# NVlabs/bayes-sim-ig

Hardware: AMD Instinct MI355X
Metric: summary_vectors_per_sec_in_fit (higher is better)
Workload: dtype f32; 1 GPU; cfg5: ShadowHand MDRFF-4096 K=4 D=32, summary_start (I=2310), 100000 pairs/GPU, reference chunk protocol: <=1000-pair chunks, summarizer + 100 Adam updates x minibatch 100 + 6 held-out evals per chunk; pairs_per_gpu=100000, parallelism=dp1, gradient_exchange=none, hip_graph=True

## Files before the change

### bayes_sim_ig_amd/_lib.py

```python
import ctypes as C
import os

import torch

_HERE = os.path.dirname(os.path.abspath(__file__))
LIB_PATH = os.environ.get('BSIG_LIB_PATH') or os.path.join(_HERE, 'lib', 'libbsig_hip.so')

BSIG_OK, BSIG_EINVAL, BSIG_ELAUNCH, BSIG_EUNSUPPORTED, BSIG_ENONFINITE = 0, -1, -2, -3, -4
EPI_NONE, EPI_BIAS, EPI_BIAS_ACT, EPI_COS_SIN, EPI_COS_OFF, EPI_MUL_DACT = range(6)
ACT_TANH, ACT_RELU, ACT_LEAKY_RELU, ACT_SIGMOID, ACT_IDENTITY = range(5)
MAX_HIDDEN = 8
FIT_GRAPH, FIT_SPLIT_ADAM = 1, 2
PLAN_NO_PERSISTENT = 1
X_ROWS, X_CROSSCORR_FACTORS = 0, 1

i64, i32, u64, f32, vp, sz = (C.c_int64, C.c_int32, C.c_uint64, C.c_float,
                              C.c_void_p, C.c_size_t)


class HeadDims(C.Structure):
    _fields_ = [('out_dim', i32), ('n_comp', i32), ('full_cov', i32),
                ('eps_noise', f32), ('min_weight', f32), ('ll_limit', f32)]


class MdnCfg(C.Structure):
    _fields_ = [('input_dim', i32), ('n_hidden', i32),
                ('hidden', i32 * MAX_HIDDEN), ('activation', i32),
                ('rff_feats', i32), ('rff_cos_only', i32),
                ('rff_scale', f32), ('head', HeadDims),
                ('lr', f32), ('beta1', f32), ('beta2', f32), ('adam_eps', f32)]


class FitBuffers(C.Structure):
    _fields_ = [('params', vp), ('grads', vp), ('exp_avg', vp),
                ('exp_avg_sq', vp),
                ('rff_coeff', vp), ('ld_coeff', i64), ('rff_offset', vp),
                ('x_train', vp), ('ldx_train', i64), ('n_train', i64),
                ('y_train', vp), ('ldy_train', i64),
                ('x_test', vp), ('ldx_test', i64), ('n_test', i64),
                ('y_test', vp), ('ldy_test', i64),
                ('ids_table', vp), ('train_loss', vp), ('test_loss', vp),
                ('state', vp), ('workspace', vp), ('workspace_bytes', sz),
                ('x_kind', i32), ('x_s', i32), ('x_a', i32),
                ('x_test_factors', vp), ('ldx_test_factors', i64)]


_PROTOS = {
    'bsig_last_error': (C.c_char_p, []),
    'bsig_version': (C.c_int, []),
    'bsig_abi_info': (u64, [C.c_int]),
    'bsig_device_count': (C.c_int, []),
    'bsig_summary_dim': (i64, [C.c_int] * 5),
    'bsig_summary_start': (C.c_int, [vp, vp, vp, i64] + [C.c_int] * 5 + [i64, vp]),
    'bsig_crosscorr': (C.c_int, [vp, vp, vp, i64] + [C.c_int] * 5 + [i64, vp, vp]),
    'bsig_crosscorr_factor_dims': (C.c_int, [C.c_int] * 3 + [C.POINTER(i32)] * 2),
    'bsig_crosscorr_factors': (C.c_int, [vp, vp, vp, i64] + [C.c_int] * 5 + [i64, vp, vp]),
    'bsig_crosscorr_expand': (C.c_int, [vp, i64, i64, C.c_int, C.c_int, vp, i64, vp]),
    'bsig_signature': (C.c_int, [vp, vp, vp, i64] + [C.c_int] * 4 + [i64, vp]),
    'bsig_gemm_workspace_bytes': (sz, [i64, i64, i64]),
    'bsig_gemm_f32': (C.c_int, [vp, i64, C.c_int, vp, vp, i64, C.c_int, vp, vp,
                                i64, i64, i64, i64, C.c_int, C.c_int, vp, vp,
                                i64, f32, vp, sz, vp]),
    'bsig_rff_coeff': (C.c_int, [vp, vp, vp, i64, i64, i64, vp]),
    'bsig_rff_project': (C.c_int, [vp, i64, vp, vp, i64, vp, vp, i64, i64, i64,
                                   i64, f32, C.c_int, vp, sz, vp]),
    'bsig_head_width': (i64, [C.POINTER(HeadDims)]),
    'bsig_head_workspace_bytes': (sz, [C.POINTER(HeadDims), i64]),
    'bsig_mdn_head_outputs': (C.c_int, [C.POINTER(HeadDims), vp, i64, i64, vp,
                                        u64, u64, vp, vp, vp, vp, vp, vp, sz, vp]),
    'bsig_mdn_nll_from_tuple': (C.c_int, [C.POINTER(HeadDims), vp, vp, vp, vp,
                                          vp, i64, i64, vp, vp, vp, sz, vp]),
    'bsig_mdn_head_nll': (C.c_int, [C.POINTER(HeadDims), vp, i64, vp, i64, vp,
                                    i64, i64, vp, u64, u64, vp, vp, vp, vp, sz,
                                    vp]),
    'bsig_adam_flat': (C.c_int, [vp, vp, vp, vp, i64, f32, f32, f32, f32, i64, vp]),
    'bsig_colsum': (C.c_int, [vp, i64, i64, i64, vp, vp, sz, vp]),
    'bsig_normalize_rows': (C.c_int, [vp, i64, vp, vp, vp, i64, i64, i64, vp]),
    'bsig_copy_rows': (C.c_int, [vp, i64, vp, vp, i64, i64, i64, vp]),
    'bsig_mdn_param_count': (i64, [C.POINTER(MdnCfg)]),
    'bsig_mdn_param_offsets': (C.c_int, [C.POINTER(MdnCfg), C.POINTER(i64), C.c_int]),
    'bsig_mdn_workspace_bytes': (sz, [C.POINTER(MdnCfg), i64]),
    'bsig_mdn_head_forward': (C.c_int, [C.POINTER(MdnCfg), vp, vp, i64, vp, vp,
                                        i64, vp, i64, vp, i64, vp, sz, vp]),
    'bsig_mdn_loss_grad': (C.c_int, [C.POINTER(MdnCfg), vp, vp, i64, vp, vp, i64,
                                     vp, i64, vp, i64, i64, vp, u64, u64, vp, vp,
                                     vp, vp, sz, vp]),
    'bsig_fit_create': (C.c_int, [C.POINTER(MdnCfg), i64, i64, i64, C.POINTER(vp)]),
    'bsig_fit_create_sized': (C.c_int, [C.POINTER(MdnCfg), i64, i64, i64, i64, C.POINTER(vp)]),
    'bsig_fit_create_ex': (C.c_int, [C.POINTER(MdnCfg), i64, i64, i64, i64, C.c_int, C.POINTER(vp)]),
    'bsig_fit_destroy': (None, [vp]),
    'bsig_fit_workspace_bytes': (sz, [vp]),
    'bsig_fit_bind': (C.c_int, [vp, C.POINTER(FitBuffers), C.c_int]),
    'bsig_fit_begin': (C.c_int, [vp, u64, i64, vp]),
    'bsig_fit_set_features': (C.c_int, [vp, vp, i64, i64, vp]),
    'bsig_fit_run': (C.c_int, [vp, i64, vp]),
    'bsig_fit_grad': (C.c_int, [vp, vp]),
    'bsig_fit_apply': (C.c_int, [vp, vp]),
    'bsig_fit_flush': (C.c_int, [vp, vp]),
    'bsig_fit_is_persistent': (C.c_int, [vp]),
    'bsig_fit_accepts_factors': (C.c_int, [vp]),
    'bsig_fit_accepts_factor_rows': (C.c_int, [vp, C.c_int, C.c_int]),
    'bsig_fit_evaluates_from_factors': (C.c_int, [vp, C.c_int, C.c_int, C.c_int]),
    'bsig_fit_takes_features': (C.c_int, [vp, i64]),
    'bsig_fit_eval': (C.c_int, [vp, vp]),
    'bsig_fit_updates': (C.c_int, [vp, i64, vp]),
    'bsig_debug_persist_profile': (None, [vp]),
    'bsig_debug_spin': (C.c_int, [C.c_int, sz, C.c_int, vp]),
    'bsig_debug_persist_geometry': (C.c_int, [C.c_int, C.c_int, C.c_int, C.c_int, C.c_int, C.POINTER(C.c_int32)]),
    'bsig_debug_head_geometry': (C.c_int, [C.POINTER(HeadDims), i64, C.POINTER(C.c_int32)]),
    'bsig_debug_summary_path': (C.c_int, [C.c_int, i64] + [C.c_int] * 6 + [i64, C.c_int, C.c_int,
                                                                         C.POINTER(C.c_int32)]),
    'bsig_debug_mfma_vs_fma': (C.c_int, [vp, vp, C.c_int, vp, vp]),
    'bsig_debug_persist_mdnn_geometry': (C.c_int, [C.c_int, C.c_int, C.c_int, C.c_int, C.c_int, C.c_int, C.POINTER(C.c_int32)]),
    'bsig_comm_unique_id': (C.c_int, [vp]),
    'bsig_comm_init': (C.c_int, [vp, C.c_int, C.c_int, C.c_int, C.POINTER(vp)]),
    'bsig_comm_init_external': (C.c_int, [C.c_int, C.c_int, vp, vp, C.POINTER(vp)]),
    'bsig_comm_transport': (C.c_int, [vp]),
    'bsig_comm_world': (C.c_int, [vp]),
    'bsig_fit_dp_graph_status': (C.c_int, [vp, C.c_char_p, sz]),
    'bsig_comm_rank': (C.c_int, [vp]),
    'bsig_comm_resident_calls': (i64, [vp]),
    'bsig_comm_set_resident': (None, [vp, C.c_int]),
    'bsig_comm_resident_mode': (C.c_int, [vp]),
    'bsig_comm_allreduce': (C.c_int, [vp, vp, i64, vp]),
    'bsig_comm_broadcast': (C.c_int, [vp, vp, i64, C.c_int, vp]),
    'bsig_comm_destroy': (None, [vp]),
    'bsig_fit_pack_logs': (C.c_int, [vp, i64, vp, vp]),
    'bsig_fit_run_dp': (C.c_int, [vp, vp, i64, vp, vp]),
}
COMM_ID_BYTES = 128
EXCHANGE_SUM, EXCHANGE_BROADCAST = 0, 1
EXCHANGE_FN = C.CFUNCTYPE(C.c_int, vp, C.c_int, vp, i64, C.c_int, vp)

_lib = None


def exported_symbols():
    return sorted(_PROTOS)


def load():
    global _lib
    if _lib is None:
        if not os.path.exists(LIB_PATH):
            raise RuntimeError(
                'libbsig_hip.so not built (%s): run ./build.sh or '
                '__graft_entry__.build(); there is no CPU fallback' % LIB_PATH)
        lib = C.CDLL(LIB_PATH)
        for name, (res, args) in _PROTOS.items():
            fn = getattr(lib, name)
            fn.restype, fn.argtypes = res, args
        _check_abi(lib)
        _lib = lib
    return _lib


HEADER_PATH = os.path.join(os.path.dirname(_HERE), 'include', 'bsig.h')


def header_hash(path=HEADER_PATH):
    h = 0xcbf29ce484222325
    with open(path, 'rb') as f:
        for b in f.read():
            h = ((h ^ b) * 0x100000001b3) & 0xFFFFFFFFFFFFFFFF
    return h


def _check_abi(lib):
    want = {1: C.sizeof(HeadDims), 2: C.sizeof(MdnCfg), 3: C.sizeof(FitBuffers),
            4: FitBuffers.x_kind.offset}
    for which, size in want.items():
        got = int(lib.bsig_abi_info(which))
        if got != size:
            raise RuntimeError('libbsig_hip.so was built against another include/bsig.h (layout %d: '
                               'library %d, binding %d): rebuild with ./build.sh' % (which, got, size))
    built = int(lib.bsig_abi_info(0))
    if built and os.path.exists(HEADER_PATH) and built != header_hash():
        raise RuntimeError('libbsig_hip.so was built from another revision of include/bsig.h '
                           '(hash %016x, header %016x): rebuild with ./build.sh'
                           % (built, header_hash()))


def require_gpu():
    lib = load()
    if not torch.cuda.is_available():
        raise RuntimeError('bayes_sim_ig_amd needs a ROCm GPU (MI355X): '
                           'torch.cuda.is_available() is False and there is '
                           'no CPU fallback')
    return lib


def check(rc):
    if rc == BSIG_OK:
        return
    msg = load().bsig_last_error().decode('utf-8', 'replace')
    if rc == BSIG_EINVAL:
        raise AssertionError(msg)
    if rc == BSIG_EUNSUPPORTED:
        raise NotImplementedError(msg)
    raise RuntimeError('libbsig_hip: %s (code %d)' % (msg, rc))


def ptr(t):
    return None if t is None else C.c_void_p(t.data_ptr())


def stream(device=None):
    return C.c_void_p(torch.cuda.current_stream(device).cuda_stream)


# ... 24 lines not shown
```

### bayes_sim_ig_amd/bayes_sim.py

```python
import os

import numpy as np
import torch

from . import pdf
from . import summarizers as _summ
from .mdnn import MDNN
from .mdrff import MDRFF
from .summarizers import (pad_states_actions, summary_start, summary_waypts,
                          summary_corr, summary_corrdiff, summary_signatory,
                          signature_depth, cross_correlation)

_SUMMARIZERS = {
    'summary_start': summary_start, 'summary_waypts': summary_waypts,
    'summary_corr': summary_corr, 'summary_corrdiff': summary_corrdiff,
    'summary_signatory': summary_signatory,
}
_MODELS = {'MDNN': MDNN, 'MDRFF': MDRFF}


class BayesSim(object):
    NUM_TRAIN_TRAJ_PER_BATCH = 1000
    NUM_TRAIN_EPOCHS = 10
    MINIBATCH_SIZE = 100
# ... 2 lines not shown
    FIT_BLOCK_CHUNKS = 32
    REFIT_SAMPLES = int(1e4)
    REFIT_MINIBATCH = 100
    REFIT_EPOCHS = 5

    def __init__(self, model_cfg, obs_dim, act_dim, params_dim, params_lows,
                 params_highs, prior, proposal=None, device='cpu'):
        self.prior = prior
        self.proposal = proposal
        model_class = model_cfg['modelClass']
        name = model_cfg['summarizerFxn']
        if name not in _SUMMARIZERS:
            raise NameError("name '%s' is not defined" % name)
        self.summarizer_name = name
        self.summarizer_fxn = _SUMMARIZERS[name]
        self._sig_depth = model_cfg.get('sigDepth', None)
        traj_summaries_dim = _summ.summary_dim(
            name, model_cfg['trainTrajLen'], obs_dim, act_dim,
            self._sig_depth or 0)
        full_covariance = bool(model_cfg.get('fullCovariance', False))
        kwargs = {'input_dim': traj_summaries_dim, 'output_dim': params_dim,
                  'output_lows': params_lows, 'output_highs': params_highs,
                  'n_gaussians': model_cfg['components'],
                  'hidden_layers': model_cfg['hiddenLayers'],
                  'lr': model_cfg['lr'],
                  'activation': torch.nn.Tanh,
                  'full_covariance': full_covariance,
                  'device': device}
        if model_class.startswith('MDRFF'):
            kernel, sigma = 'RBF', 4.0
            if '_' in model_class:
                parts = model_class.split('_')
                model_class, kernel = parts[0], parts[1]
                if len(parts) > 2:
                    sigma = float(parts[2])
            kwargs.update({'n_feat': int(model_cfg.get('nFeat', 200)),
                           'sigma': sigma, 'kernel': kernel})
        if model_class not in _MODELS:
            raise NameError("name '%s' is not defined" % model_class)
        self.model = _MODELS[model_class](**kwargs)

    @staticmethod
    def get_n_trajs_per_batch(n_train_trajs, n_train_trajs_done):
        n = BayesSim.NUM_TRAIN_TRAJ_PER_BATCH
        if n_train_trajs_done + n > n_train_trajs:
            n = n_train_trajs - n_train_trajs_done
        return n

    def _summarize(self, states, actions, finite_flag=None, lazy=False):
        if self.summarizer_name == 'summary_signatory' and self._sig_depth:
            return self.summarizer_fxn(states, actions, depth=self._sig_depth)
        if self.summarizer_name in ('summary_corr', 'summary_corrdiff'):
            kw = {}
            if finite_flag is not None:
                kw['check_finite'] = finite_flag
            if lazy and self._lazy_summaries():
                kw['lazy'] = True
            return self.summarizer_fxn(states, actions, **kw)
        return self.summarizer_fxn(states, actions)

    def _lazy_summaries(self):
        return (getattr(self.model, 'rff', None) is None and self.model._flat.is_cuda and
                os.environ.get('BSIG_NO_FUSED_SUMMARY') != '1')

    def run_training(self, params, traj_states, traj_actions, _defer=False, _finite_flag=None,
                     _summaries=None, _feats=None):
        traj_summaries = _summaries if _summaries is not None else \
            self._summarize(traj_states, traj_actions, _finite_flag, lazy=True)
        kw = {} if _feats is None else {'_feats': _feats}
        return self.model.run_training(
            x_data=traj_summaries, y_data=params,
            n_updates=BayesSim.NUM_GRAD_UPDATES,
            batch_size=BayesSim.MINIBATCH_SIZE,
            test_frac=BayesSim.TEST_FRACTION, _defer=_defer, **kw)

    FIT_BLOCK_BYTES = 4 << 30

    def fit(self, params, traj_states, traj_actions):
        if self.model._flat.is_cuda and self.model._may_time_out():
            from .mdnn import PersistentTimeout
            snap = self.model._snapshot()
            for _ in range(2):
                calls0 = self.model._resident_calls()
                try:
                    return self._fit_once(params, traj_states, traj_actions)
                except PersistentTimeout:
                    self.model._restore(snap)
                    self.model._give_up_a_level(calls0)
        return self._fit_once(params, traj_states, traj_actions)

    def _fit_once(self, params, traj_states, traj_actions):
        n, done, pending = params.shape[0], 0, []
        dp = getattr(self.model, '_dp', None)
        if dp is not None:
            counts = dp.gather_counts(n, device=self.model._flat.device)
            if len(set(counts)) != 1:
                raise ValueError('data-parallel fit needs the same number of pairs on every rank '
                                 '(got %s); see dp.equal_shards' % (counts,))
        flag = None
        if torch.is_tensor(traj_states) and traj_states.is_cuda:
            flag = torch.zeros(1, dtype=torch.int32, device=traj_states.device)
        block = 0
        is_rff = getattr(self.model, 'rff', None) is not None
        if flag is not None and os.environ.get('BSIG_NO_FIT_PREPROJECT') != '1':
            row_bytes = 4 * (self.model.input_dim + (self.model.rff.n_feat if is_rff else 0))
            chunks = max(min(BayesSim.FIT_BLOCK_CHUNKS,
                             BayesSim.FIT_BLOCK_BYTES // (row_bytes * BayesSim.NUM_TRAIN_TRAJ_PER_BATCH)), 1)
            block = chunks * BayesSim.NUM_TRAIN_TRAJ_PER_BATCH
        lo = hi = 0
        summ = feats = None
        while done < n:
            m = BayesSim.get_n_trajs_per_batch(n, done)
            if block and done + m > hi:
                lo, hi = done, min(n, done + block)
                summ = self._summarize(traj_states[lo:hi], traj_actions[lo:hi], flag, lazy=True)
                feats = self.model.rff.to_features(summ) if is_rff else None
            if block:
                pending.append(self.run_training(
                    params[done:done + m], None, None, _defer=True,
                    _summaries=summ[done - lo:done - lo + m],
                    _feats=None if feats is None else feats[done - lo:done - lo + m]))
            else:
                pending.append(self.run_training(params[done:done + m],
                                                 traj_states[done:done + m],
                                                 traj_actions[done:done + m], _defer=True,
                                                 _finite_flag=flag))
            done += m
        logs = [p.result() for p in pending]
        assert flag is None or int(flag.item()) == 0
        return logs

    def predict(self, states, actions, threshold=0.005):
        summaries = self._summarize(states, actions)
        mixtures = [self._correct_for_proposal(m, threshold) for m in self.model.predict_MoGs(summaries)]
        return mixtures[0] if len(mixtures) == 1 else self._refit(mixtures)

    def _correct_for_proposal(self, mog, threshold):
        if self.proposal is None:
            return mog
        mog.prune_negligible_components(threshold=threshold)
        if isinstance(self.prior, pdf.Uniform):
            return mog / self.proposal
        if isinstance(self.prior, pdf.Gaussian):
            return (mog * self.prior) / self.proposal
        raise NotImplementedError

    def _refit(self, mixtures):
        src = self.model
        refit = MDNN(input_dim=1, output_dim=src.output_dim,
                     output_lows=src.output_lows.detach().cpu().numpy(),
                     output_highs=src.output_highs.detach().cpu().numpy(),
                     n_gaussians=src.n_gaussians, hidden_layers=(128, 128), lr=src.lr,
                     activation=src.activation, full_covariance=src.L_size > 0, device=src.device)
        share = int(BayesSim.REFIT_SAMPLES / len(mixtures))
        draws = torch.from_numpy(np.concatenate([m.gen(n_samples=share) for m in mixtures], axis=0))
        draws = draws.float().to(src.device)
        if MDNN.VERBOSE:
            print(f'Fitting posterior from {len(mixtures):d} mogs')
        const_in = torch.zeros(draws.shape[0], 1, device=draws.device)
        refit.run_training(const_in, draws,
                           BayesSim.REFIT_EPOCHS * BayesSim.REFIT_SAMPLES // BayesSim.REFIT_MINIBATCH,
                           BayesSim.REFIT_MINIBATCH)
        fitted = refit.predict_MoGs(const_in[0:1, :])
        assert len(fitted) == 1
        return fitted[0]
```

### bayes_sim_ig_amd/csrc/estimator.hip

```cpp
#include "comm.h"
#include "gemm.h"
#include "head.h"
#include "persist.h"
#include "persist_mdnn.h"

#include <algorithm>
#include <chrono>
#include <cmath>
#include <cstdlib>
#include <cstring>
#include <new>

namespace bsig {

int adam_launch(float* p, const float* g, float* m, float* v, int64_t n, float lr,
                float beta1, float beta2, float eps, int64_t t, const float* dyn,
                hipStream_t st);
int colsum_launch(const float* x, int64_t ld, int64_t rows, int64_t cols, float* out,
                  void* workspace, size_t workspace_bytes, hipStream_t st);

constexpr int64_t kAlign = 4;

struct Layout {
  int n_layers;
// ... 297 lines not shown
  bsig_mdn_cfg cfg;
  Layout L;
  int64_t batch, max_test, n_updates, n_evals;
  bool hoist;
  bool feat_cache;
  bool feat_unique;
  bool feats_preloaded;
  const float* ext_feats;
  int64_t feat_rows;
  int64_t max_train;
  bsig_fit_buffers buf;
  bool bound;
  int64_t norm_batch;
  size_t train_ws_bytes, test_ws_bytes, feats_bytes, big_gemm_ws_bytes, iota_bytes;
  bool use_graph, split_adam;

  PersistEngine eng;
  UGeom ug; MdnnGeom mg;
  bool eng_off;
  int dp_evals_done;
  bool resident_ran;
  bool adam_pending;
  hipStream_t cap_stream;
  hipGraphExec_t g_step, g_grad, g_apply, g_eval;
  bool graphs_ready;
  const float* graph_feats;
  hipGraphExec_t g_dp; const bsig_comm* g_dp_comm;
  int g_dp_state;
  char g_dp_error[200];
};

namespace bsig {

static size_t plan_ws_bytes(const bsig_fit_plan* p) {
  return p->train_ws_bytes + p->test_ws_bytes + p->feats_bytes + p->big_gemm_ws_bytes +
         p->iota_bytes + p->eng.workspace_bytes;
}

static int engine(const bsig_fit_plan* p) { return p->eng_off ? 0 : p->eng.kind; }

static bool evals_in_launch(const bsig_fit_plan* p, bool dp, bool test_factors) {
  return (dp ? p->eng.eval_dp : p->eng.eval_single) && (!p->eng.streams || test_factors);
}

static bool feat_cache_applies(const bsig_fit_plan* p, int64_t n_train) {
  return p->hoist && p->feat_cache && n_train <= p->n_updates * p->batch;
}

struct PlanMem { Scratch tr, te; float* feats; float* big_ws; int32_t* iota; void* persist_ws; };

static int begin_regions(const bsig_fit_plan* p) {
  const bool pers = engine(p) != 0;
  return (pers ? 2 : 0) + (!(pers && !p->split_adam) ? 2 : 0);
}
static bool tickets_zeroed(const bsig_fit_plan* p) { return begin_regions(p) + 2 <= 4; }

static void plan_mem(const bsig_fit_plan* p, PlanMem* m) {
  char* base = reinterpret_cast<char*>(p->buf.workspace);
  carve(&p->cfg, p->L, p->batch, base, &m->tr);
  base += p->train_ws_bytes;
  carve(&p->cfg, p->L, std::max<int64_t>(p->max_test, 1), base, &m->te);
  base += p->test_ws_bytes;
  m->feats = p->ext_feats ? const_cast<float*>(p->ext_feats) : reinterpret_cast<float*>(base);
  base += p->feats_bytes;
  m->big_ws = reinterpret_cast<float*>(base); base += p->big_gemm_ws_bytes;
  m->iota = reinterpret_cast<int32_t*>(base); base += p->iota_bytes;
  m->persist_ws = base;
  if (!tickets_zeroed(p)) m->tr.tickets = m->te.tickets = nullptr;
}

static PersistShape persist_shape(const bsig_fit_plan* p) {
  return PersistShape{(int)p->batch, (int)p->L.feat_dim, p->cfg.head.out_dim, p->cfg.head.n_comp,
                      (int)std::min<int64_t>(p->max_test, 1 << 20)};
}

static PersistMdnnShape persist_mdnn_shape(const bsig_fit_plan* p) {
  const bsig_mdn_cfg& c = p->cfg;
  return PersistMdnnShape{(int)p->batch, c.input_dim, c.n_hidden > 0 ? c.hidden[0] : 0,
                          c.n_hidden > 1 ? c.hidden[1] : 0, c.activation, c.head.out_dim,
                          c.head.n_comp, c.head.full_cov,
                          (int)std::min<int64_t>(p->max_test, 1 << 20)};
}

static int enqueue_persistent(bsig_fit_plan* p, int n, hipStream_t st, int eval_total = 0,
                              const CommXr* xr = nullptr) {
  PlanMem m; plan_mem(p, &m);
  const bsig_fit_buffers& b = p->buf;
  PersistCommon c;
  c.y = b.y_train; c.ldy = b.ldy_train; c.ids = b.ids_table;
  c.params = b.params; c.exp_avg = b.exp_avg; c.exp_avg_sq = b.exp_avg_sq;
  c.state = b.state; c.train_loss = b.train_loss;
  c.workspace = m.persist_ws; c.workspace_bytes = p->eng.workspace_bytes;
  if (p->split_adam) {
    c.grads = b.grads; c.adam_pending = p->adam_pending ? 1 : 0;
    p->adam_pending = false;
  }
  if (xr) { c.xr_ready = xr->ready; c.xr_done = xr->done; c.xr_base = xr->base; c.n_total = n; }
  if (eval_total > 0) {
    c.do_eval = 1; c.n_total = eval_total; c.eval_every = std::max(eval_total / 5, 1);
    c.n_test = (int)b.n_test;
    c.y_test = b.y_test; c.ldy_test = b.ldy_test; c.test_loss = b.test_loss;
  }
  c.hy.lr = p->cfg.lr; c.hy.beta1 = p->cfg.beta1; c.hy.beta2 = p->cfg.beta2;
  c.hy.adam_eps = p->cfg.adam_eps; c.hy.eps_noise = p->cfg.head.eps_noise;
  c.hy.min_weight = p->cfg.head.min_weight; c.hy.ll_limit = p->cfg.head.ll_limit;
  c.hy.norm_batch = p->norm_batch;
  if (engine(p) == 1) {
    PersistBuffers pb;
    static_cast<PersistCommon&>(pb) = c;
    pb.feats = m.feats; pb.ld_feats = p->cfg.rff_feats;
    pb.feat_ids = p->feat_unique ? b.ids_table : nullptr;
    pb.w_off = p->L.head_w_off; pb.b_off = p->L.head_b_off;
    pb.eval_row0 = p->feat_unique ? b.n_train : p->n_updates * p->batch;
    return persist_run(persist_shape(p), p->ug, pb, n, st);
  }
  PersistMdnnBuffers pb;
  static_cast<PersistCommon&>(pb) = c;
  pb.x = b.x_train; pb.ldx = b.ldx_train;
  pb.x_kind = b.x_kind; pb.x_s = b.x_s; pb.x_a = b.x_a;
  pb.w1_off = p->L.w_off[0]; pb.b1_off = p->L.b_off[0];
  pb.w2_off = p->L.w_off[1]; pb.b2_off = p->L.b_off[1];
  pb.wh_off = p->L.head_w_off; pb.bh_off = p->L.head_b_off;
  pb.x_test = b.x_test; pb.ldx_test = b.ldx_test;
  pb.x_test_fac = b.x_test_factors; pb.ldx_test_fac = b.ldx_test_factors;
  return persist_mdnn_run(persist_mdnn_shape(p), p->mg, pb, n, st);
}

static Inputs train_inputs(const bsig_fit_plan* p, const PlanMem& m) {
  const bsig_fit_buffers& b = p->buf;
  Inputs in;
  in.dyn = b.state + ST_STEP; in.dyn_stride = p->batch;
  in.rff_coeff = b.rff_coeff; in.ld_coeff = b.ld_coeff; in.rff_offset = b.rff_offset;
  if (p->hoist) {
    in.x = m.feats; in.ldx = p->cfg.rff_feats; in.is_feat = true;
    if (p->feat_unique) in.rows = b.ids_table;
  }
  else { in.x = b.x_train; in.ldx = b.ldx_train; in.rows = b.ids_table; }
  return in;
}

static Inputs eval_inputs(const bsig_fit_plan* p, const PlanMem& m) {
  const bsig_fit_buffers& b = p->buf;
  Inputs in;
  in.rff_coeff = b.rff_coeff; in.ld_coeff = b.ld_coeff; in.rff_offset = b.rff_offset;
  if (p->hoist) {
    in.x = m.feats; in.ldx = p->cfg.rff_feats; in.is_feat = true;
    in.dyn = b.state + ST_EVAL; in.dyn_stride = 0;
    in.dyn_base = p->feat_unique ? b.n_train : p->n_updates * p->batch;
  } else {
    in.x = b.x_test; in.ldx = b.ldx_test;
  }
  return in;
}

static int enqueue_grad(bsig_fit_plan* p, hipStream_t st, bool fuse_adam) {
  if (p->buf.x_kind != BSIG_X_ROWS) { set_error("per-phase update on factor rows"); return BSIG_EUNSUPPORTED; }
  PlanMem m; plan_mem(p, &m);
  const bsig_fit_buffers& b = p->buf;
  const Inputs in = train_inputs(p, m);
  HeadDyn hd;
  hd.y_dyn = b.state + ST_STEP; hd.y_dyn_stride = p->batch;
  hd.hook.state = b.state; hd.hook.kind = 1;
  hd.hook.lr = p->cfg.lr; hd.hook.beta1 = p->cfg.beta1; hd.hook.beta2 = p->cfg.beta2;
  AdamFuse fuse{b.exp_avg, b.exp_avg_sq, reinterpret_cast<const float*>(b.state) + ST_ADAM0,
                p->cfg.beta1, p->cfg.beta2, p->cfg.adam_eps};
  const uint64_t* rng = reinterpret_cast<const uint64_t*>(b.state + ST_RNG);
  int n_sig = 0;
  BSIG_TRY(forward_pass(&p->cfg, p->L, b.params, in, p->batch, m.tr, m.tr.o, m.tr.ld_o, st,
                        &n_sig));
  hd.n_sig_ready = n_sig;
  HeadBiasPartials bp;
  const bool partial_bias = fuse_adam && p->L.n_layers == 0 && in.rows != nullptr &&
      gemm_wide_gradient_applies(p->L.nh, p->L.feat_dim, p->batch, m.tr.ld_o, in.ldx, m.tr.d_o, in.x, true);
  BSIG_TRY(head_nll(&p->cfg, p->L, m.tr, b.y_train, b.ldy_train, b.ids_table, p->batch,
                    p->norm_batch, nullptr, 0, 0, rng, b.train_loss, b.state + ST_STEP, true,
                    b.grads + p->L.head_b_off, b.state + ST_NONFINITE, &hd, st,
                    partial_bias ? &bp : nullptr));
  return backward_pass(&p->cfg, p->L, b.params, in, -1, p->batch, m.tr, b.grads,
                       fuse_adam ? &fuse : nullptr, st, partial_bias ? &bp : nullptr);
}

static int enqueue_apply(bsig_fit_plan* p, hipStream_t st) {
  const bsig_fit_buffers& b = p->buf;
  return adam_launch(b.params, b.grads, b.exp_avg, b.exp_avg_sq, p->L.total, p->cfg.lr,
                     p->cfg.beta1, p->cfg.beta2, p->cfg.adam_eps, 1,
                     reinterpret_cast<const float*>(b.state) + ST_ADAM0, st);
}

static int enqueue_eval(bsig_fit_plan* p, hipStream_t st) {
  PlanMem m; plan_mem(p, &m);
  const bsig_fit_buffers& b = p->buf;
  HeadDyn hd;
  hd.hook.state = b.state; hd.hook.kind = 2;
  if (b.n_test <= 0) {
    hipLaunchKernelGGL(iota_mod_kernel, dim3(1), dim3(64), 0, st, b.state + ST_EVAL + 0, 0, 1);
    BSIG_CHECK_LAUNCH("eval_noop");
// ... 121 lines not shown
  carve(cfg, L, batch, workspace, &s);
  s.tickets = nullptr;
  Inputs in;
  in.x = x; in.ldx = ldx; in.rows = x_rows;
  in.rff_coeff = rff_coeff; in.ld_coeff = ld_coeff; in.rff_offset = rff_offset;
  return forward_pass(cfg, L, params, in, batch, s, head_out, ld_head, as_stream(stream));
}

extern "C" int bsig_mdn_loss_grad(const bsig_mdn_cfg* cfg, const float* params,
                                  const float* rff_coeff, int64_t ld_coeff,
                                  const float* rff_offset, const float* x, int64_t ldx,
                                  const float* y, int64_t ldy, const int32_t* rows,
                                  int64_t batch, int64_t norm_batch, const float* noise,
                                  uint64_t seed, uint64_t stream_id, float* grads, float* loss,
                                  int32_t* nonfinite, void* workspace, size_t workspace_bytes,
                                  bsig_stream_t stream) {
  Layout L;
  BSIG_TRY(make_layout(cfg, &L));
  BSIG_REQUIRE(params && x && y && grads && batch >= 1 && norm_batch >= 1,
               "loss_grad: bad args");
  BSIG_REQUIRE(ldx >= cfg->input_dim && ldy >= cfg->head.out_dim, "loss_grad: leading dims");
  Scratch s;
  carve(cfg, L, batch, nullptr, &s);
  BSIG_REQUIRE(workspace && workspace_bytes >= s.total_bytes, "loss_grad: workspace %zu < %zu",
               workspace_bytes, s.total_bytes);
  carve(cfg, L, batch, workspace, &s);
  s.tickets = nullptr;
  hipStream_t st = as_stream(stream);
  Inputs in;
  in.x = x; in.ldx = ldx; in.rows = rows;
  in.rff_coeff = rff_coeff; in.ld_coeff = ld_coeff; in.rff_offset = rff_offset;
  int n_sig = 0;
  BSIG_TRY(forward_pass(cfg, L, params, in, batch, s, s.o, s.ld_o, st, &n_sig));
  HeadDyn hd;
  hd.n_sig_ready = n_sig;
  BSIG_TRY(head_nll(cfg, L, s, y, ldy, rows, batch, norm_batch, noise, seed, stream_id, nullptr,
                    loss, nullptr, true, grads + L.head_b_off, nonfinite, &hd, st));
  return backward_pass(cfg, L, const_cast<float*>(params), in, 0, batch, s, grads, nullptr, st);
}

extern "C" int bsig_fit_create(const bsig_mdn_cfg* cfg, int64_t batch, int64_t max_test_rows,
                               int64_t n_updates, bsig_fit_plan** plan) {
  return bsig_fit_create_sized(cfg, batch, 0, max_test_rows, n_updates, plan);
}

extern "C" int bsig_fit_create_sized(const bsig_mdn_cfg* cfg, int64_t batch,
                                     int64_t max_train_rows, int64_t max_test_rows,
                                     int64_t n_updates, bsig_fit_plan** plan) {
  return bsig_fit_create_ex(cfg, batch, max_train_rows, max_test_rows, n_updates, 0, plan);
}

extern "C" int bsig_fit_create_ex(const bsig_mdn_cfg* cfg, int64_t batch,
                                  int64_t max_train_rows, int64_t max_test_rows,
                                  int64_t n_updates, int plan_flags, bsig_fit_plan** plan) {
  BSIG_REQUIRE(cfg && plan && batch >= 1 && max_train_rows >= 0 && max_test_rows >= 0 &&
               n_updates >= 0, "fit_create: bad args");
  bsig_fit_plan* p = new (std::nothrow) bsig_fit_plan();
  BSIG_REQUIRE(p, "fit_create: out of memory");
  std::memset(p, 0, sizeof(*p));
  p->cfg = *cfg;
  const int rc = make_layout(cfg, &p->L);
  if (rc != BSIG_OK) { delete p; return rc; }
  p->batch = batch; p->max_test = max_test_rows; p->norm_batch = batch;
  p->n_updates = n_updates; p->n_evals = count_evals(n_updates);
  Scratch s;
  carve(cfg, p->L, batch, nullptr, &s); p->train_ws_bytes = s.total_bytes;
  carve(cfg, p->L, std::max<int64_t>(max_test_rows, 1), nullptr, &s);
  p->test_ws_bytes = s.total_bytes;
  p->max_train = max_train_rows;
  const auto set = [](const char* name) { const char* e = getenv(name); return e && e[0] == '1'; };
  p->feat_cache = !set("BSIG_NO_FEAT_CACHE");
  if (!p->feat_cache) max_train_rows = 0;
  p->feat_rows = (max_train_rows > 0 ? std::min(n_updates * batch, max_train_rows)
                                     : n_updates * batch) + max_test_rows;
  const size_t feats = (size_t)p->feat_rows * (size_t)std::max(cfg->rff_feats, 0) * sizeof(float);
  p->hoist = cfg->rff_feats > 0 && n_updates > 0 && feats <= ((size_t)4 << 30) && !set("BSIG_NO_RFF_HOIST");
  if (!((plan_flags & BSIG_PLAN_NO_PERSISTENT) || set("BSIG_NO_PERSISTENT"))) {
    if (p->hoist && p->L.n_layers == 0 && cfg->head.full_cov == 0)
      persist_resolve(persist_shape(p), &p->ug, &p->eng);
    else if (cfg->rff_feats == 0 && p->L.n_layers == 2 && n_updates > 0)
      persist_mdnn_resolve(persist_mdnn_shape(p), &p->mg, &p->eng);
  }
  if (set("BSIG_NO_INKERNEL_EVAL")) p->eng.eval_single = p->eng.eval_dp = false;
  p->eng.workspace_bytes = round_up<size_t>(p->eng.workspace_bytes, 256);
  if (p->hoist) {
    p->feats_bytes = round_up<size_t>(feats, 256);
    const int64_t mf = cfg->rff_cos_only ? cfg->rff_feats : cfg->rff_feats / 2;
    p->big_gemm_ws_bytes = round_up<size_t>(
        std::max(bsig_gemm_workspace_bytes(p->feat_rows - max_test_rows, mf, cfg->input_dim),
                 bsig_gemm_workspace_bytes(std::max<int64_t>(max_test_rows, 1), mf,
                                           cfg->input_dim)) + 256, 256);
  }
  *plan = p;
  return BSIG_OK;
}

extern "C" void bsig_fit_destroy(bsig_fit_plan* p) {
  if (!p) return;
  drop_graphs(p);
  if (p->cap_stream) (void)hipStreamDestroy(p->cap_stream);
  delete p;
}

extern "C" size_t bsig_fit_workspace_bytes(const bsig_fit_plan* p) {
  return p ? plan_ws_bytes(p) : 0;
}

extern "C" int bsig_fit_bind(bsig_fit_plan* p, const bsig_fit_buffers* b, int flags) {
  BSIG_REQUIRE(p && b, "fit_bind: null");
  BSIG_REQUIRE(b->params && b->grads && b->exp_avg && b->exp_avg_sq && b->state &&
               b->workspace && b->x_train && b->y_train && b->ids_table && b->train_loss &&
               b->test_loss, "fit_bind: null buffer");
  BSIG_REQUIRE(b->workspace_bytes >= plan_ws_bytes(p), "fit_bind: workspace %zu < %zu",
               b->workspace_bytes, plan_ws_bytes(p));
  BSIG_REQUIRE(!(p->max_train > 0 && b->n_train > p->max_train),
               "fit_bind: %lld training rows exceed the %lld the plan was sized for",
               (long long)b->n_train, (long long)p->max_train);
  BSIG_REQUIRE(b->n_train >= 1 && b->n_test >= 0 && b->n_test <= std::max<int64_t>(p->max_test, 0),
               "fit_bind: n_train=%lld n_test=%lld (max %lld)", (long long)b->n_train,
               (long long)b->n_test, (long long)p->max_test);
  const bool fac = b->x_kind == BSIG_X_CROSSCORR_FACTORS;
  BSIG_REQUIRE(b->x_kind == BSIG_X_ROWS || fac, "fit_bind: unknown x_kind %d", b->x_kind);
  const bool graph = (flags & BSIG_FIT_GRAPH) != 0, split = (flags & BSIG_FIT_SPLIT_ADAM) != 0;
  const bool eng_off = p->eng.streams && !(fac && bsig_fit_accepts_factor_rows(p, b->x_s, b->x_a));
  if (eng_off != p->eng_off) { drop_graphs(p); p->eng_off = eng_off; p->bound = false; }
  const MdnnGeom& g = p->mg;
  if (engine(p) == 2 && p->eng.streams && !(g.s_S == b->x_s && g.s_A == b->x_a && g.s_dp == (split ? 1 : 0)))
    BSIG_TRY(persist_mdnn_resolve_stream(&p->mg, p->cfg.input_dim, p->cfg.head.full_cov != 0, b->x_s, b->x_a, split));
  if (fac) {
    BSIG_REQUIRE(b->x_s >= 1 && b->x_a >= 1 && (int64_t)b->x_s * b->x_a + 2 == p->cfg.input_dim,
                 "fit_bind: factor rows S=%d A=%d do not give the %d inputs of the first layer",
                 b->x_s, b->x_a, p->cfg.input_dim);
    BSIG_REQUIRE(b->ldx_train >= b->x_s + b->x_a + 3, "fit_bind: factor rows need a pitch >= S + A + 3");
    const bool eval_fac = b->x_test_factors && bsig_fit_evaluates_from_factors(p, b->x_s, b->x_a, flags);
    BSIG_REQUIRE(b->n_test == 0 || (eval_fac && !b->x_test) || b->ldx_test >= p->cfg.input_dim,
                 "fit_bind: the held-out rows are summary rows (ldx_test >= input_dim)");
    if (!bsig_fit_accepts_factor_rows(p, b->x_s, b->x_a)) {
      set_error("fit_bind: this plan runs kernels that read materialised summary rows "
                "(bsig_fit_accepts_factors); expand the factors (bsig_crosscorr_expand)");
      return BSIG_EUNSUPPORTED;
    }
  }
  BSIG_REQUIRE((fac || b->ldx_train >= p->cfg.input_dim) && b->ldy_train >= p->cfg.head.out_dim,
               "fit_bind: leading dims too small");
  BSIG_REQUIRE(!(b->n_test > 0 && !b->y_test), "fit_bind: null test buffers");
  BSIG_REQUIRE(!(b->n_test > 0 && !b->x_test &&
                 !(fac && b->x_test_factors && bsig_fit_evaluates_from_factors(p, b->x_s, b->x_a, flags))),
               "fit_bind: null test buffers");
  const bool same = p->bound && std::memcmp(&p->buf, b, sizeof(*b)) == 0 &&
                    p->use_graph == graph && p->split_adam == split;
  if (!same) {
    drop_graphs(p);
    p->buf = *b;
    p->feat_unique = feat_cache_applies(p, b->n_train);
    if (p->hoist && !p->feat_unique && p->feat_rows - p->max_test < p->n_updates * p->batch) {
      p->bound = false;
      set_error("fit_bind: %lld training rows exceed the %lld the plan was sized for",
                (long long)b->n_train, (long long)p->max_train);
      return BSIG_EINVAL;
    }
    p->bound = true;
    p->use_graph = graph;
    p->split_adam = split;
  }
  if (p->use_graph && !p->cap_stream)
    BSIG_HIP(hipStreamCreateWithFlags(&p->cap_stream, hipStreamNonBlocking));
  return BSIG_OK;
}

static bool graphs_read_feats(const bsig_fit_plan* p) {
  if (!p->use_graph) return false;
  if (engine(p) != 1) return true;
  if (p->buf.n_test < 1) return false;
  return !evals_in_launch(p, p->split_adam, false);
}

extern "C" int bsig_fit_set_features(bsig_fit_plan* p, const float* feats, int64_t ld_feats,
                                     int64_t rows, bsig_stream_t stream) {
  BSIG_REQUIRE(p && p->bound && feats, "fit_set_features: plan not bound / null");
  BSIG_REQUIRE(p->hoist && p->feat_unique, "fit_set_features: the plan keeps no per-row feature cache");
  BSIG_REQUIRE(rows == p->buf.n_train + p->buf.n_test && ld_feats >= p->cfg.rff_feats,
               "fit_set_features: need the %lld training + %lld held-out rows",
               (long long)p->buf.n_train, (long long)p->buf.n_test);
  p->ext_feats = nullptr;
  if (ld_feats == p->cfg.rff_feats && aligned(feats, 16) && !graphs_read_feats(p)) {
    p->ext_feats = feats;
  } else {
    PlanMem m; plan_mem(p, &m);
    const size_t w = (size_t)p->cfg.rff_feats * sizeof(float);
    BSIG_HIP(hipMemcpy2DAsync(m.feats, w, feats, (size_t)ld_feats * sizeof(float), w, (size_t)rows,
                              hipMemcpyDeviceToDevice, as_stream(stream)));
  }
  p->feats_preloaded = true;
  return BSIG_OK;
}

extern "C" int bsig_fit_begin(bsig_fit_plan* p, uint64_t seed, int64_t norm_batch,
                              bsig_stream_t stream) {
  bsig::Range roctx_range("bsig_fit_begin");
  BSIG_REQUIRE(p && p->bound, "fit_begin: plan not bound");
  BSIG_REQUIRE(norm_batch >= 1, "fit_begin: norm_batch must be >= 1");
  if (norm_batch != p->norm_batch) { drop_graphs(p); p->norm_batch = norm_batch; }
  hipStream_t st = as_stream(stream);
  p->adam_pending = false;
  p->resident_ran = false;
  p->dp_evals_done = 0;
  BeginZero bz{};
  int nz = 0;
  int64_t total4 = 0;
  auto add_zero = [&](void* ptr, size_t bytes) {
    bz.ptr[nz] = reinterpret_cast<float4*>(ptr);
    bz.n4[nz] = (int64_t)(bytes / 16);
    total4 += bz.n4[nz];
    ++nz;
  };
  if (engine(p)) {
    PlanMem m; plan_mem(p, &m);
    ZeroRegion zr[2];
    if (engine(p) == 1) BSIG_TRY(persist_reset_regions(p->ug, m.persist_ws, p->eng.workspace_bytes, zr));
    else BSIG_TRY(persist_mdnn_reset_regions(p->mg, m.persist_ws, p->eng.workspace_bytes, zr));
    BSIG_REQUIRE(aligned(zr[0].ptr, 16) && aligned(zr[1].ptr, 16) && zr[0].bytes % 16 == 0 &&
                 zr[1].bytes % 16 == 0, "fit_begin: persistent workspace regions must be 16-byte multiples");
    add_zero(zr[0].ptr, zr[0].bytes);
    add_zero(zr[1].ptr, zr[1].bytes);
  }
  if (!(engine(p) && !p->split_adam)) {
    BSIG_REQUIRE(aligned(p->buf.exp_avg, 16) && aligned(p->buf.exp_avg_sq, 16),
                 "fit_begin: the Adam moment buffers must be 16-byte aligned");
    add_zero(p->buf.exp_avg, (size_t)p->L.total * sizeof(float));
    add_zero(p->buf.exp_avg_sq, (size_t)p->L.total * sizeof(float));
  }
  if (tickets_zeroed(p)) {
    BSIG_REQUIRE(nz == begin_regions(p), "fit_begin: region count out of step with begin_regions()");
    PlanMem tm; plan_mem(p, &tm);
    add_zero(tm.tr.tickets, kWideTickets * sizeof(int32_t));
    add_zero(tm.te.tickets, kWideTickets * sizeof(int32_t));
  }
  const int blocks = (int)std::min<int64_t>(std::max<int64_t>(ceil_div<int64_t>(total4, 256 * 4), 1), 1024);
  hipLaunchKernelGGL(fit_begin_kernel, dim3(blocks), dim3(256), 0, st, p->buf.state, seed, bz);
  BSIG_CHECK_LAUNCH("fit_begin");
  if (p->hoist) {
    if (p->feats_preloaded) p->feats_preloaded = false;
    else { p->ext_feats = nullptr; BSIG_TRY(enqueue_hoisted_rff(p, st)); }
  }
  return ensure_graphs(p);
}

static int dp_eval_total(const bsig_fit_plan* p) {
  return engine(p) && p->split_adam && p->buf.n_test >= 1 && evals_in_launch(p, true, false) ? (int)p->n_updates : 0;
}

extern "C" int bsig_fit_grad(bsig_fit_plan* p, bsig_stream_t stream) {
  BSIG_REQUIRE(p && p->bound && p->split_adam, "fit_grad: plan not bound with SPLIT_ADAM");
  if (engine(p)) return enqueue_persistent(p, 1, as_stream(stream), dp_eval_total(p));
  if (p->use_graph) { BSIG_TRY(ensure_graphs(p)); BSIG_HIP(hipGraphLaunch(p->g_grad, as_stream(stream))); return BSIG_OK; }
  return enqueue_grad(p, as_stream(stream), false);
}

extern "C" int bsig_fit_apply(bsig_fit_plan* p, bsig_stream_t stream) {
  BSIG_REQUIRE(p && p->bound && p->split_adam, "fit_apply: plan not bound with SPLIT_ADAM");
  if (engine(p) && !p->eng.streams) { p->adam_pending = true; return BSIG_OK; }
  if (engine(p)) return enqueue_apply(p, as_stream(stream));
  if (p->use_graph) { BSIG_TRY(ensure_graphs(p)); BSIG_HIP(hipGraphLaunch(p->g_apply, as_stream(stream))); return BSIG_OK; }
  return enqueue_apply(p, as_stream(stream));
}

extern "C" int bsig_fit_takes_features(const bsig_fit_plan* p, int64_t n_train) {
  return p && n_train >= 1 && feat_cache_applies(p, n_train) ? 1 : 0;
}

extern "C" int bsig_fit_accepts_factors(const bsig_fit_plan* p) {
  return p && p->eng.kind == 2 && !p->eng.streams ? 1 : 0;
}

extern "C" int bsig_fit_accepts_factor_rows(const bsig_fit_plan* p, int s_dim, int a_dim) {
  return p && p->eng.kind == 2 && persist_mdnn_factors_fit(p->mg, p->cfg.input_dim, s_dim, a_dim) ? 1 : 0;
}

extern "C" int bsig_fit_evaluates_from_factors(const bsig_fit_plan* p, int s_dim, int a_dim, int bind_flags) {
  return p && p->eng.streams && bsig_fit_accepts_factor_rows(p, s_dim, a_dim) &&
                 evals_in_launch(p, (bind_flags & BSIG_FIT_SPLIT_ADAM) != 0, true) ? 1 : 0;
}

extern "C" int bsig_fit_is_persistent(const bsig_fit_plan* p) {
  return p ? engine(p) : 0;
}

extern "C" int bsig_fit_flush(bsig_fit_plan* p, bsig_stream_t stream) {
  BSIG_REQUIRE(p && p->bound, "fit_flush: plan not bound");
  if (engine(p) && p->split_adam && p->adam_pending)
    return enqueue_persistent(p, 0, as_stream(stream));
  return BSIG_OK;
}

extern "C" int bsig_fit_eval(bsig_fit_plan* p, bsig_stream_t stream) {
  bsig::Range roctx_range("bsig_fit_eval");
  BSIG_REQUIRE(p && p->bound, "fit_eval: plan not bound");
  if (const int total = dp_eval_total(p)) {
    if (++p->dp_evals_done < count_evals(total)) return BSIG_OK;
    return enqueue_persistent(p, 0, as_stream(stream), total);
  }
  BSIG_REQUIRE(p->buf.n_test < 1 || p->buf.x_test,
               "fit_eval: this binding has no held-out summary rows (its evaluations run inside bsig_fit_run)");
  BSIG_TRY(bsig_fit_flush(p, stream));
  if (p->use_graph) { BSIG_TRY(ensure_graphs(p)); BSIG_HIP(hipGraphLaunch(p->g_eval, as_stream(stream))); return BSIG_OK; }
  return enqueue_eval(p, as_stream(stream));
}

static int enqueue_updates(bsig_fit_plan* p, int64_t n, hipStream_t st) {
  if (n <= 0) return BSIG_OK;
  if (engine(p) && !p->split_adam) return enqueue_persistent(p, (int)n, st);
  if (engine(p)) {
    for (int64_t it = 0; it < n; ++it) {
      BSIG_TRY(enqueue_persistent(p, 1, st, dp_eval_total(p)));
      if (p->eng.streams) BSIG_TRY(enqueue_apply(p, st));
      else p->adam_pending = true;
    }
    return BSIG_OK;
  }
  for (int64_t it = 0; it < n; ++it) {
    if (p->use_graph) {
      if (p->split_adam) {
        BSIG_HIP(hipGraphLaunch(p->g_grad, st));
        BSIG_HIP(hipGraphLaunch(p->g_apply, st));
      } else {
        BSIG_HIP(hipGraphLaunch(p->g_step, st));
      }
    } else {
      BSIG_TRY(enqueue_grad(p, st, !p->split_adam));
      if (p->split_adam) BSIG_TRY(enqueue_apply(p, st));
    }
  }
  return BSIG_OK;
}

extern "C" int bsig_fit_updates(bsig_fit_plan* p, int64_t n_updates, bsig_stream_t stream) {
  bsig::Range roctx_range("bsig_fit_updates");
  BSIG_REQUIRE(p && p->bound, "fit_updates: plan not bound");
  BSIG_REQUIRE(n_updates >= 0 && n_updates <= p->n_updates,
               "fit_updates: n_updates %lld exceeds the plan's %lld", (long long)n_updates,
               (long long)p->n_updates);
  if (p->use_graph) BSIG_TRY(ensure_graphs(p));
  return enqueue_updates(p, n_updates, as_stream(stream));
}

extern "C" int bsig_fit_run(bsig_fit_plan* p, int64_t n_updates, bsig_stream_t stream) {
  bsig::Range roctx_range("bsig_fit_run");
  BSIG_REQUIRE(p && p->bound, "fit_run: plan not bound");
  BSIG_REQUIRE(n_updates >= 0 && n_updates <= p->n_updates,
               "fit_run: n_updates %lld exceeds the plan's %lld", (long long)n_updates,
               (long long)p->n_updates);
  hipStream_t st = as_stream(stream);
  if (p->use_graph) BSIG_TRY(ensure_graphs(p));
  if (engine(p) && !p->split_adam && n_updates >= 1 && p->buf.n_test >= 1 &&
      evals_in_launch(p, false, p->buf.x_test_factors != nullptr))
    return enqueue_persistent(p, (int)n_updates, st, (int)n_updates);
  const int64_t every = std::max<int64_t>(n_updates / 5, 1);
  int64_t done = 0;
  for (int64_t it = 0; it < n_updates; ++it) {
    if (it % every == 0 || it + 1 == n_updates) {
      BSIG_TRY(enqueue_updates(p, it + 1 - done, st));
      done = it + 1;
      BSIG_TRY(bsig_fit_eval(p, stream));
    }
  }
  return BSIG_OK;
}

namespace bsig {
__global__ void pack_logs_kernel(const float* train_loss, const float* test_loss,
                                 const int32_t* state, int n_updates, int n_evals, float* out) {
  const int every = n_updates / 5 > 1 ? n_updates / 5 : 1;
  if (threadIdx.x == 0) {
    int e = 0;
    for (int it = 0; it < n_updates; ++it)
      if (it % every == 0 || it + 1 == n_updates) { out[e] = train_loss[it]; ++e; }
    out[2 * n_evals] = (float)state[ST_NONFINITE];
  }
  for (int i = threadIdx.x; i < n_evals; i += blockDim.x) out[n_evals + i] = test_loss[i];
}
}

extern "C" int bsig_fit_pack_logs(bsig_fit_plan* p, int64_t n_updates, float* out,
                                  bsig_stream_t stream) {
  BSIG_REQUIRE(p && p->bound && out, "fit_pack_logs: plan not bound / null");
  BSIG_REQUIRE(n_updates >= 0 && n_updates <= p->n_updates, "fit_pack_logs: bad n_updates");
  hipLaunchKernelGGL(pack_logs_kernel, dim3(1), dim3(64), 0, as_stream(stream), p->buf.train_loss,
                     p->buf.test_loss, p->buf.state, (int)n_updates, (int)count_evals(n_updates), out);
  BSIG_CHECK_LAUNCH("pack_logs");
  return BSIG_OK;
}

namespace bsig {
__global__ void pack_dp_logs_kernel(const float* train_loss, const float* test_loss,
                                    const int32_t* state, int n_updates, int n_evals, float n_test,
                                    float* out) {
  const int n = n_updates + n_evals + 3;
  for (int i = blockIdx.x * blockDim.x + threadIdx.x; i < n; i += gridDim.x * blockDim.x) {
    float v;
    if (i < n_updates) v = train_loss[i];
    else if (i < n_updates + n_evals) v = n_test > 0.f ? test_loss[i - n_updates] * n_test : 0.f;
    else if (i == n_updates + n_evals) v = n_test;
    else v = (state[ST_NONFINITE] >> (i - n_updates - n_evals - 1)) & 1 ? 1.f : 0.f;
    out[i] = v;
  }
}
}

__global__ void debug_scale_kernel(float* buf, int64_t n, float s) {
  for (int64_t i = (int64_t)blockIdx.x * blockDim.x + threadIdx.x; i < n; i += (int64_t)gridDim.x * blockDim.x)
    buf[i] *= s;
}
static int allreduce_grads(bsig_fit_plan* p, bsig_comm* comm, bsig_stream_t stream) {
  BSIG_TRY(bsig_comm_allreduce(comm, p->buf.grads, p->L.total, stream));
  if (const char* e = getenv("BSIG_DEBUG_GRAD_EXCHANGE_SCALE")) {
    const float s = (float)atof(e);
    if (s != 1.0f) {
      const char* ge = getenv("BSIG_DEBUG_GRAD_EXCHANGE_GRID");
      const int grid = ge ? std::max(atoi(ge), 1) : 8;
      hipLaunchKernelGGL(debug_scale_kernel, dim3(grid), dim3(1024), 0, as_stream(stream), p->buf.grads, p->L.total, s);
      BSIG_CHECK_LAUNCH("debug_scale");
    }
  }
  return BSIG_OK;
}

static int ensure_dp_graph(bsig_fit_plan* p, bsig_comm* comm) {
  if (p->g_dp_state == 1 && p->g_dp_comm == comm) return BSIG_OK;
  if (p->g_dp_state < 0 && p->g_dp_comm == comm) return BSIG_OK;
  if (p->g_dp) { (void)hipGraphExecDestroy(p->g_dp); p->g_dp = nullptr; }
  p->g_dp_comm = comm; p->g_dp_error[0] = 0;
  const char* env = getenv("BSIG_DP_GRAPH");
  if (!p->use_graph || engine(p) != 1 || bsig_comm_transport(comm) != 1 || !(env && env[0] == '1')) {
    p->g_dp_state = -2;
    snprintf(p->g_dp_error, sizeof(p->g_dp_error), "%s",
             !(env && env[0] == '1') ? "not requested (BSIG_DP_GRAPH=1)" :
             bsig_comm_transport(comm) != 1 ? "the exchange is not RCCL" : "the plan's updates are not one launch each");
    return BSIG_OK;
  }
  hipGraph_t graph = nullptr;
  hipError_t e = hipStreamBeginCapture(p->cap_stream, hipStreamCaptureModeRelaxed);
  int rc = BSIG_OK;
  if (e == hipSuccess) {
    p->adam_pending = true;
    rc = enqueue_persistent(p, 1, p->cap_stream, dp_eval_total(p));
    if (rc == BSIG_OK) rc = allreduce_grads(p, comm, reinterpret_cast<bsig_stream_t>(p->cap_stream));
    e = hipStreamEndCapture(p->cap_stream, &graph);
  }
  if (e == hipSuccess && rc == BSIG_OK) e = hipGraphInstantiate(&p->g_dp, graph, nullptr, nullptr, 0);
  if (graph) (void)hipGraphDestroy(graph);
  if (e != hipSuccess || rc != BSIG_OK || !p->g_dp) {
    snprintf(p->g_dp_error, sizeof(p->g_dp_error), "capture of launch + ncclAllReduce failed: %s",
             rc != BSIG_OK ? bsig_last_error() : hipGetErrorString(e));
    (void)hipGetLastError();
    p->g_dp = nullptr; p->g_dp_state = -1;
    return BSIG_OK;
  }
  p->g_dp_state = 1;
  return BSIG_OK;
}

extern "C" int bsig_fit_dp_graph_status(const bsig_fit_plan* p, char* msg, size_t msg_bytes) {
  if (!p) return 0;
  if (msg && msg_bytes) snprintf(msg, msg_bytes, "%s", p->g_dp_error);
  return p->g_dp_state;
}

static bool dp_resident_applies(const bsig_fit_plan* p, const bsig_comm* comm, int64_t n_updates) {
  const char* e = getenv("BSIG_DP_RESIDENT");
  const int mode = bsig_comm_resident_mode(comm);
  bool want = mode >= 0 ? mode == 1 : (e && e[0] == '1');
  if (want && !bsig::comm_resident_allowed(comm)) {
// ... 157 lines not shown
```

### bayes_sim_ig_amd/csrc/fit_persistent.hip

```cpp
#include "persist.h"

#include <algorithm>
#include <cstdlib>

#include "head_device.h"
#include "persist_device.h"

namespace bsig {

constexpr int kUT = 512;
constexpr int kUSteps = 18;
constexpr int kUGroup = 6;
constexpr int kUMT = 7;
constexpr int kULds = 160 * 1024;
constexpr int kUProf = 8;
constexpr int kUFP = 116;

struct UArgs {
  int B, Bp, MT;
  int Fdim, KS, ksteps, KB, WP;
  int Nh, NhP, D, K;
  int n_blocks, k_slices, G, T, n_owner, R;
  int n_updates, xs_floats;
  int fast_rows;
  const float* feats; int64_t ld_feats; const int32_t* feat_ids;
  const float* y; int64_t ldy; const int32_t* ids;
  float* params; float* m1; float* m2; int64_t w_off, b_off;
  int32_t* state; float* train_loss;
  double lr, beta1, beta2;
  float adam_eps, eps_noise, min_w, ll_limit, inv_norm;
  float* slabs; float* d_out; float* e_out; unsigned* flag_fwd; unsigned long long* gran;
  unsigned long long* gran_rep;
  float* grads; int adam_pending; int quad_ok;
  unsigned* xr_ready; const unsigned* xr_done; unsigned* xr_count; unsigned xr_base;
  int do_eval, eval_every, n_total, n_test, eval_passes, NE, RE;
  int64_t eval_row0;
  const float* y_test; int64_t ldy_test;
  float* test_loss;
  float* eval_slabs;
  unsigned* flag_eval;
  unsigned long long* gran_eval;
  long long* prof;
  int prof_t0;
};

__device__ __forceinline__ f32x4 umfma(float a, float b, f32x4 c) {
  return __builtin_amdgcn_mfma_f32_16x16x4f32(a, b, c, 0, 0, 0);
}

struct URole { int tile, owner; };
__device__ __forceinline__ URole wg_role(int wg, int T, int G) {
  const int per = T >> 3, rem = T & 7, gq = G >> 3, gr = G & 7;
  const int x = wg & 7, j = wg >> 3;
  const int tiles_x = gq + (x < gr ? 1 : 0);
  URole r;
  if (j < tiles_x) {
    r.tile = x * gq + min(x, gr) + j;
    int rank = 0;
    for (int xx = 0; xx < 8; ++xx) {
      const int cnt = wg > xx ? (wg - xx + 7) >> 3 : 0;
      rank += min(cnt, gq + (xx < gr ? 1 : 0));
    }
    r.owner = (T - G) + rank;
  } else {
    r.tile = -1;
    r.owner = x * (per - gq) + min(x, rem) - min(x, gr) + (j - tiles_x);
  }
  return r;
}

__device__ __forceinline__ int u_rowpos(int b) { return (b & ~15) + ((b & 3) << 2) + ((b >> 2) & 3); }

__device__ __forceinline__ int u_evals_before(int s, int every) { return s == 0 ? 0 : (s - 1) / every + 1; }

#define BSIG_USTAMP(k)                                                           \
  do {                                                                           \
    if (p.prof && threadIdx.x == 0 && t >= p.prof_t0 && t < p.prof_t0 + kUProf)  \
      p.prof[((int64_t)wg * kUProf + t - p.prof_t0) * 16 + (k)] = wall_clock64(); \
  } while (0)

__device__ __forceinline__ int u_fast_kind(const UArgs& p) {
  const int K = p.K;
  if (K > 16 || p.fast_rows == 0) return 0;
  if (p.T - p.G < p.n_owner) return 0;
  const int KP = K <= 4 ? 4 : (K <= 8 ? 8 : 16);
  const int nq = (p.D + 64 / KP - 1) / (64 / KP);
  if (p.R > 4 || nq > 8 || p.R * ((p.Nh + 3) >> 2) > kUT) return 0;
  const int nqh = nq <= 2 ? 1 : (nq <= 4 ? 2 : 4);
  return KP * 8 + nqh;
}

__device__ __forceinline__ unsigned long long* gran_rep(const UArgs& p, int arr, int x) {
  return p.gran_rep + (int64_t)(arr * 8 + x) * kGranArr;
}
__device__ __forceinline__ void granule_publish8(const UArgs& p, int arr, int slot, uint32_t tag, float v, int lane) {
  if (lane < 8) granule_publish(gran_rep(p, arr, lane), slot, tag, v);
}

template <typename RowOff, typename F>
__device__ __forceinline__ void u_rows_sum(const float* slabs, RowOff&& rowoff, int k_slices, int zs, int nrows,
                                           int n_cols, float* out, int out_pitch, int tid, F&& fn) {
  const __amdgpu_buffer_rsrc_t sr = xwg_buffer(slabs);
  for (int idx = tid; idx < nrows * n_cols; idx += kUT) {
    const int r = idx / n_cols, col = idx - r * n_cols;
    const int voff = (rowoff(r) + col) * 4;
    float v = 0.f;
    for (int z = 0; z < k_slices; z += 16) {
      float q[16];
#pragma unroll
      for (int u = 0; u < 16; ++u)
        q[u] = __uint_as_float(__builtin_amdgcn_raw_buffer_load_b32(sr, voff, min(z + u, k_slices - 1) * zs * 4, kXwgPolicy));
#pragma unroll
      for (int u = 0; u < 16; ++u)
        if (z + u < k_slices) v += q[u];
    }
    out[r * out_pitch + col] = v;
    fn(col, v);
  }
}

template <typename RowOff, typename F>
__device__ __forceinline__ void u_rows_sum4(const float* slabs, RowOff&& rowoff, int k_slices, int zs, int nrows,
                                            int n_cols, int ld, float* out, int out_pitch, float* part, int tid,
                                            F&& fn) {
  const __amdgpu_buffer_rsrc_t sr = xwg_buffer(slabs);
  const int ncq = (n_cols + 3) >> 2, Q = nrows * ncq;
  const int SG = max(1, min(min(k_slices, kUT / Q), 8));
  const int qc = tid % Q, sg = tid / Q;
  if (sg < SG) {
    const int r = qc / ncq, c4 = (qc - r * ncq) * 4;
    const int voff = rowoff(r) + c4;
    f32x4 v = {0.f, 0.f, 0.f, 0.f};
    for (int z0 = sg; z0 < k_slices; z0 += 8 * SG) {
      f32x4 q[8];
#pragma unroll
      for (int u = 0; u < 8; ++u) q[u] = xwg_load4(sr, voff + min(z0 + u * SG, k_slices - 1) * zs);
#pragma unroll
      for (int u = 0; u < 8; ++u)
        if (z0 + u * SG < k_slices) v += q[u];
    }
    *reinterpret_cast<f32x4*>(part + 4 * (sg * Q + qc)) = v;
  }
  __syncthreads();
  if (tid < Q) {
    const int r = tid / ncq, c4 = (tid - r * ncq) * 4;
    f32x4 v = *reinterpret_cast<const f32x4*>(part + 4 * tid);
    for (int g = 1; g < SG; ++g) v += *reinterpret_cast<const f32x4*>(part + 4 * (g * Q + tid));
#pragma unroll
    for (int j = 0; j < 4; ++j)
      if (c4 + j < n_cols) {
        out[r * out_pitch + c4 + j] = v[j];
        fn(c4 + j, v[j]);
      }
  }
}

template <int NT>
__device__ __forceinline__ void u_tile_eval(const UArgs& p, const float* Wl, const float* biasl, int slot,
                                            int ks, int n0, int k0, int eidx) {
  int tid = threadIdx.x;
  asm volatile("" : "+v"(tid));
  const int lane = tid & 63, w = tid >> 6, c16 = lane & 15, g4 = lane >> 4;
  const int B = p.B, NhP = p.NhP;
  for (int pass = 0; pass < p.eval_passes; ++pass) {
    const int rows = min(B, p.n_test - pass * B);
    if (rows <= 0) break;
    if (w < p.MT) {
      f32x4 acc[NT];
#pragma unroll
      for (int nt = 0; nt < NT; ++nt) {
        const f32x4 zero = {0.f, 0.f, 0.f, 0.f};
        acc[nt] = ks == 0 ? *reinterpret_cast<const f32x4*>(biasl + 16 * nt + 4 * g4) : zero;
      }
      const int64_t r = p.eval_row0 + pass * B + min(16 * w + c16, rows - 1);
      const float* src = p.feats + r * p.ld_feats;
      const float* ap = Wl + c16 * p.WP + 4 * g4;
#pragma unroll 1
      for (int s0 = 0; s0 < p.ksteps; s0 += kUGroup) {
        f32x4 breg[kUGroup];
#pragma unroll
        for (int q = 0; q < kUGroup; ++q) {
          const int col = k0 + 16 * (s0 + q) + 4 * g4;
          const f32x4 v = *reinterpret_cast<const f32x4*>(src + min((int64_t)col, p.ld_feats - 4));
          const f32x4 zero = {0.f, 0.f, 0.f, 0.f};
          breg[q] = col < p.Fdim ? v : zero;
        }
#pragma unroll
        for (int q = 0; q < kUGroup; ++q) {
#pragma unroll
          for (int nt = 0; nt < NT; ++nt) {
            const f32x4 a4 = *reinterpret_cast<const f32x4*>(ap + nt * 16 * p.WP + 16 * (s0 + q));
            acc[nt] = umfma(a4[0], breg[q][0], acc[nt]);
            acc[nt] = umfma(a4[1], breg[q][1], acc[nt]);
            acc[nt] = umfma(a4[2], breg[q][2], acc[nt]);
            acc[nt] = umfma(a4[3], breg[q][3], acc[nt]);
          }
        }
      }
      if (16 * w + c16 < rows) {
        const __amdgpu_buffer_rsrc_t sr = xwg_buffer(
            p.eval_slabs + ((((int64_t)(eidx % 3) * p.eval_passes + pass) * p.k_slices + ks) * B) * NhP + n0);
#pragma unroll
        for (int nt = 0; nt < NT; ++nt)
          xwg_store4(sr, (16 * w + c16) * NhP + 16 * nt + 4 * g4, acc[nt][0], acc[nt][1], acc[nt][2], acc[nt][3]);
      }
    }
  }
  __builtin_amdgcn_s_waitcnt(0);
  __syncthreads();
  if (tid == 0) flag_raise(p.flag_eval, slot, (unsigned)eidx + 1u);
}

__device__ __forceinline__ void u_owner_eval(const UArgs& p, float* XS, float* red, int eo, int eidx,
                                             uint64_t stream, const HeadArgs& a) {
  int tid = threadIdx.x;
  asm volatile("" : "+v"(tid));
  const int lane = tid & 63, w = tid >> 6;
  const int B = p.B, Nh = p.Nh, NhP = p.NhP, D = p.D, K = p.K, DK = D * K;
  const int per_wave = Nh + D + 3 * K;
  int32_t* flagp = p.state + 2;
  const unsigned etag = (unsigned)eidx + 1u;
  if (w == 0) flags_wait(p.flag_eval, p.G, etag, lane, flagp);
  __syncthreads();
  const int nr = eo < p.n_test ? min(p.RE, (p.n_test - eo + p.NE - 1) / p.NE) : 0;
  const float* ebase = p.eval_slabs + (int64_t)(eidx % 3) * p.eval_passes * p.k_slices * B * NhP;
  float eacc = 0.f;
  u_rows_sum(ebase,
             [&](int r) {
               const int erow = eo + p.NE * r, pass = erow / B, rb = erow - pass * B;
               return (pass * p.k_slices * B + rb) * NhP;
             },
             p.k_slices, B * NhP, nr, Nh, XS, per_wave, tid,
             [&](int col, float v) { if (col >= K + DK && col < K + 2 * DK) eacc += expf(v); });
  eacc = wave_sum_dpp(eacc);
  if (lane == 0) red[w] = eacc;
  __syncthreads();
  if (tid == 0) {
    float sx = 0.f;
    for (int q = 0; q < kUT / 64; ++q) sx += red[q];
    granule_publish(p.gran_eval, eo, etag, sx);
  }
  const int erow = eo + p.NE * w;
  const bool act = w < nr;
  float* tile = XS + w * per_wave;
  float* yv = tile + Nh;
  float* rk = yv + D;
  float* lpk = rk + K;
  float* dlg = lpk + K;
  if (act)
    for (int j = lane; j < D; j += 64) yv[j] = p.y_test[(int64_t)erow * p.ldy_test + j];
  RowOut ro;
  ro.lse = 0.f; ro.uds = 0.f; ro.bad = false;
#pragma unroll
  for (int q = 0; q < kElemsPerLane; ++q) ro.esg0[q] = 0.f;
  if (w < p.RE) {
    HeadArgs ae = a;
    ae.d_out = nullptr;
    ae.batch = p.n_test;
    ae.stream_id = stream;
    diag_row(ae, erow, act, lane, tile, yv, rk, lpk, dlg,
             [&] {
               return p.eps_noise != 0.f
                          ? p.eps_noise * (granule_gather(p.gran_eval, p.NE, etag, lane, flagp) /
                                           ((float)p.n_test * (float)DK))
                          : 0.f;
             },
             ro);
  }
  if (lane == 0) red[16 + w] = act ? ro.lse : 0.f;
  __syncthreads();
  if (tid == 0) {
    float sl = 0.f;
    for (int q = 0; q < kUT / 64; ++q) sl += red[16 + q];
    granule_publish(p.gran_eval + kGranArr, eo, etag, sl);
  }
  if (eo == 0 && w == 0) {
    const float sum = granule_gather(p.gran_eval + kGranArr, p.NE, etag, lane, flagp);
    if (lane == 0) {
      const float l = -sum / (float)p.n_test;
      p.test_loss[p.state[1]] = l;
      p.state[1] = p.state[1] + 1;
      if (!isfinite(l)) atomicOr(flagp, 1);
    }
  }
  if (ro.bad) atomicOr(flagp, 1);
  __syncthreads();
}

struct UOwn {
  int own, r0, per_wave;
  bool has_tile;
  float *XS, *red, *part;
  HeadArgs a; RowGeom rg;
  uint64_t rng_ctr0; int step0, ev0; float norm; int32_t* flagp;
};
__device__ __forceinline__ void u_own_init(const UArgs& p, UOwn& o, int own, bool has_tile, float* XS,
                                           float* red, float* part, int lane0) {
  o.own = own; o.r0 = own * p.R; o.per_wave = p.Nh + p.D + 3 * p.K; o.has_tile = has_tile;
  o.XS = XS; o.red = red; o.part = part;
  o.a = HeadArgs{};
  o.a.D = p.D; o.a.K = p.K; o.a.Nh = p.Nh; o.a.batch = p.B; o.a.from_tuple = 0;
  o.a.min_w = p.min_w; o.a.ll_limit = p.ll_limit; o.a.inv_norm = p.inv_norm;
  o.a.eps_noise = p.eps_noise; o.a.seed = reinterpret_cast<const uint64_t*>(p.state + 8)[0]; o.a.d_out = p.d_out;
  o.rg = row_geom(p.D, p.K, lane0);
  o.rng_ctr0 = reinterpret_cast<const uint64_t*>(p.state + 8)[1];
  o.step0 = p.state[0];
  o.ev0 = p.do_eval ? u_evals_before(o.step0, p.eval_every) : 0;
  o.norm = (float)p.B * (float)(p.D * p.K);
  o.flagp = p.state + 2;
}
__device__ __forceinline__ uint64_t u_eval_stream(const UArgs& p, const UOwn& o, int e, bool last) {
  const int at = last ? p.n_total : e * p.eval_every + 1;
  return o.rng_ctr0 + (uint64_t)(at - o.step0) + (uint64_t)(e - o.ev0);
}

__device__ __forceinline__ void u_own_update(const UArgs& p, UOwn& o, int t, int w, int lane0, int wg) {
  const int B = p.B, Nh = p.Nh, NhP = p.NhP, D = p.D, K = p.K, DK = D * K;
  const int step = o.step0 + t;
  const unsigned epoch = (unsigned)step + 1u;
  const uint32_t tag = epoch * 4u;
  const int own = o.own, r0 = o.r0, per_wave = o.per_wave;
  const bool has_tile = o.has_tile;
  float* XS = o.XS; float* red = o.red; float* Ft = o.part;
  int32_t* flagp = o.flagp;
  HeadArgs& a = o.a;
  const RowGeom& rg = o.rg;
  const uint64_t rng_ctr0 = o.rng_ctr0;
  const int ev0 = o.ev0;
  const float norm = o.norm;
  const int tid = threadIdx.x;
  float* tile = XS + w * per_wave;
  float* yv = tile + Nh;
  float* rk = yv + D;
  float* lpk = rk + K;
  float* dlg = lpk + K;
  const int row = r0 + w;
  const bool owner_wave = w < p.R;
  const bool active = owner_wave && row < B;
    int lane = lane0;
    asm volatile("" : "+v"(lane));
    const int tid_l = 64 * w + lane;
    if (active) {
      const int64_t yrow = p.ids[(int64_t)step * B + row];
      for (int j = lane; j < D; j += 64) yv[j] = p.y[yrow * p.ldy + j];
    }
    float eu_pre[kElemsPerLane];
    a.stream_id = rng_ctr0 + (uint64_t)t + (uint64_t)(p.do_eval ? u_evals_before(step, p.eval_every) - ev0 : 0);
    if (owner_wave) diag_row_noise(a, rg.groups, rg.k, rg.d0, row, active, lane, eu_pre);
    if (w == 0) {
      flag_wait_one(p.flag_fwd, (int)(((int64_t)own * p.G) / p.n_owner), epoch, flagp);
      flags_wait(p.flag_fwd, p.G, epoch, lane, flagp);
    }
    __syncthreads();
    BSIG_USTAMP(4);
    float eacc = 0.f;
    if (!has_tile && p.R * NhP <= 4 * kUT)
      u_rows_sum4(p.slabs, [&](int r) { return (r0 + r) * NhP; }, p.k_slices, B * NhP, min(p.R, B - r0), Nh,
                  NhP, XS, per_wave, Ft, tid_l,
                  [&](int col, float v) { if (col >= K + DK && col < K + 2 * DK) eacc += expf(v); });
    else
      u_rows_sum(p.slabs, [&](int r) { return (r0 + r) * NhP; }, p.k_slices, B * NhP,
                 min(p.R, B - r0), Nh, XS, per_wave, tid_l,
                 [&](int col, float v) { if (col >= K + DK && col < K + 2 * DK) eacc += expf(v); });
    eacc = wave_sum_dpp(eacc);
    if (lane == 0) red[w] = eacc;
    __syncthreads();
    if (tid_l < 8) {
      float sx = 0.f;
      for (int q = 0; q < kUT / 64; ++q) sx += red[q];
      granule_publish8(p, 0, own, tag + 1, sx, tid_l);
    }
    BSIG_USTAMP(5);
    RowOut ro;
    ro.lse = 0.f; ro.uds = 0.f; ro.bad = false;
#pragma unroll
    for (int q = 0; q < kElemsPerLane; ++q) ro.esg0[q] = 0.f;
    if (owner_wave) {
      GranuleEps ge{gran_rep(p, 0, wg & 7), p.n_owner, tag + 1, lane, flagp, p.eps_noise, norm, {0ull, 0ull, 0ull, 0ull}};
      diag_row_impl(a, rg, row, active, lane, tile, yv, rk, lpk, dlg, ge, ro, eu_pre);
#ifdef BSIG_ROW_PROF
      if (p.prof && tid == 0 && t >= p.prof_t0 && t < p.prof_t0 + kUProf)
        for (int i = 0; i < 9; ++i)
          p.prof[(int64_t)256 * kUProf * 16 + ((int64_t)wg * kUProf + t - p.prof_t0) * 16 + i] = ro.ts[i];
#endif
      const float uds_w = wave_sum_dpp(ro.uds);
      if (lane == 0) { red[16 + w] = active ? ro.lse : 0.f; red[32 + w] = uds_w; }
      BSIG_USTAMP(7);
      if (active) {
        for (int j = lane; j < K; j += 64) tile[j] = dlg[j];
        __builtin_amdgcn_wave_barrier();
        float* dst = p.d_out + (int64_t)row * NhP;
        for (int j = lane; j < Nh; j += 64) xwg_store(dst + j, tile[j]);
        if (p.eps_noise != 0.f) {
          const int TPR = (64 / K) * K;
          float* est = p.e_out + (int64_t)row * NhP + K + DK;
#pragma unroll
          for (int q = 0; q < kElemsPerLane; ++q)
            if (lane < TPR && lane + q * TPR < DK) xwg_store(est + lane + q * TPR, ro.esg0[q]);
        }
      }
    }
    __builtin_amdgcn_s_waitcnt(0);
    __syncthreads();
    if (tid_l < 8) {
      float sl = 0.f, su = 0.f;
      for (int q = 0; q < p.R; ++q) { sl += red[16 + q]; su += red[32 + q]; }
      granule_publish8(p, 1, own, tag + 2, su, tid_l);
      if (tid_l == 0) granule_publish(loss_granules(p.gran, epoch), own, tag + 3, sl);
    }
    BSIG_USTAMP(9);
    if (own == 0 && w == 0) {
      const float s = granule_gather(loss_granules(p.gran, epoch), p.n_owner, tag + 3, lane, flagp);
      if (lane == 0) {
        const float l = -s / (float)B;
        p.train_loss[step] = l;
        if (!isfinite(l)) atomicOr(flagp, 1);
      }
    }
    if (ro.bad) atomicOr(flagp, 1);
}


#ifdef BSIG_ROW_PROF
#define BSIG_FSTAMP(i) do { if (p.prof && threadIdx.x == 0 && t >= p.prof_t0 && t < p.prof_t0 + kUProf) \
    p.prof[(int64_t)256 * kUProf * 16 + ((int64_t)wg * kUProf + t - p.prof_t0) * 16 + (i)] = wall_clock64(); } while (0)
#else
#define BSIG_FSTAMP(i)
#endif
template <int KP, int NQH>
__device__ __forceinline__ void u_own_update_fast(const UArgs& p, UOwn& o, int t, int w, int lane0, int wg) {
#pragma clang fp contract(off)
  constexpr int GR = 64 / KP;
  const int K = p.K;
  const bool exact = K == KP;
  const int B = p.B, Nh = p.Nh, NhP = p.NhP, D = p.D, DK = D * K, R = p.R;
  const int step = o.step0 + t;
  const unsigned epoch = (unsigned)step + 1u;
  const uint32_t tag = epoch * 4u;
  const int own = o.own, r0 = o.r0;
  float* red = o.red; float* part = o.part; float* XS = o.XS;
  int32_t* flagp = o.flagp;
  int lane = lane0;
  asm volatile("" : "+v"(lane));
  const int tid_l = 64 * w + lane;
  const int rr = w >> 1, h = w & 1;
  const int row = r0 + rr;
  const bool row_wave = rr < R;
  const bool active = row_wave && row < B;
  const int k = lane & (KP - 1), d0 = lane / KP;
  const bool kok = k < K;
  const bool jitter = p.eps_noise != 0.f;

  float yd[NQH], eu[NQH];
  bool valid[NQH];
  int ecol[NQH];
#pragma unroll
  for (int i = 0; i < NQH; ++i) {
    const int d = d0 + (h + 2 * i) * GR;
    valid[i] = active && kok && d < D;
    ecol[i] = min(d, D - 1) * K + min(k, K - 1);
    yd[i] = 0.f; eu[i] = 0.f;
  }
  if (active) {
    const int64_t yrow = p.ids[(int64_t)step * B + row];
#pragma unroll
    for (int i = 0; i < NQH; ++i)
      if (valid[i]) yd[i] = p.y[yrow * p.ldy + d0 + (h + 2 * i) * GR];
    if (jitter) {
      const uint64_t sid = o.rng_ctr0 + (uint64_t)t + (uint64_t)(p.do_eval ? u_evals_before(step, p.eval_every) - o.ev0 : 0);
      if (exact && NQH <= 2) {
        const Philox4 ph = philox4x32_10(o.a.seed, sid, ((uint64_t)row * 64 + lane) * 2);
#pragma unroll
        for (int i = 0; i < NQH; ++i)
          if (valid[i]) eu[i] = u01(h ? ph.v[(2 * i + 1) & 3] : ph.v[(2 * i) & 3]);
      } else {
        const int G = 64 / K;
#pragma unroll
        for (int i = 0; i < NQH; ++i) {
          if (valid[i]) {
            const int d = d0 + (h + 2 * i) * GR, q = d / G, gl = (d - q * G) * K + k;
            const Philox4 ph = philox4x32_10(o.a.seed, sid, ((uint64_t)row * 64 + gl) * 2 + (q >> 2));
            const int oi = q & 3;
            eu[i] = u01(oi == 0 ? ph.v[0] : (oi == 1 ? ph.v[1] : (oi == 2 ? ph.v[2] : ph.v[3])));
          }
        }
      }
    }
  }
  if (w == 0) {
    flag_wait_one(p.flag_fwd, (int)(((int64_t)own * p.G) / p.n_owner), epoch, flagp);
    flags_wait(p.flag_fwd, p.G, epoch, lane, flagp);
  }
  __syncthreads();
  BSIG_USTAMP(4);

  const int nrows = min(R, B - r0);
  const int ncq = (Nh + 3) >> 2, Q = nrows * ncq;
  const int SG = max(1, min(min(p.k_slices, kUT / Q), 8));
  {
    const __amdgpu_buffer_rsrc_t sr = xwg_buffer(p.slabs);
    const int qc = tid_l % Q, sg = tid_l / Q;
    if (sg < SG) {
      const int r = qc / ncq, c4 = (qc - r * ncq) * 4;
      const int voff = (r0 + r) * NhP + c4, zs = B * NhP;
      f32x4 v = {0.f, 0.f, 0.f, 0.f};
      for (int z0 = sg; z0 < p.k_slices; z0 += 8 * SG) {
        f32x4 q[8];
#pragma unroll
        for (int u = 0; u < 8; ++u) q[u] = xwg_load4(sr, voff + min(z0 + u * SG, p.k_slices - 1) * zs);
#pragma unroll
        for (int u = 0; u < 8; ++u)
          if (z0 + u * SG < p.k_slices) v += q[u];
      }
      *reinterpret_cast<f32x4*>(part + 4 * (sg * Q + qc)) = v;
    }
  }
  BSIG_FSTAMP(0);
  __syncthreads();
  BSIG_FSTAMP(1);

  const float* pb = part + 4 * (active ? rr : 0) * ncq;
  const int gs = 4 * Q;
  auto slice_sum = [&](int col) {
    const float* b = pb + col;
    const float v0 = b[0], v1 = b[gs * min(1, SG - 1)], v2 = b[gs * min(2, SG - 1)], v3 = b[gs * min(3, SG - 1)];
    float sacc = v0;
    if (SG > 1) sacc += v1;
    if (SG > 2) sacc += v2;
    if (SG > 3) sacc += v3;
    if (SG > 4) {
      const float v4 = b[gs * 4], v5 = b[gs * min(5, SG - 1)], v6 = b[gs * min(6, SG - 1)], v7 = b[gs * min(7, SG - 1)];
      sacc += v4;
      if (SG > 5) sacc += v5;
      if (SG > 6) sacc += v6;
      if (SG > 7) sacc += v7;
    }
    return sacc;
  };
  const int pq = DK >> 2, npq = nrows * pq;
  const bool one_wave_exp = exact && npq <= 64;
  if (one_wave_exp && w == kUT / 64 - 1) {
    const int r = lane / pq, c4 = K + DK + 4 * (lane - r * pq);
    const float* b = part + 4 * min(r, nrows - 1) * ncq + c4;
    f32x4 v = *reinterpret_cast<const f32x4*>(b);
    for (int g = 1; g < SG; ++g) v += *reinterpret_cast<const f32x4*>(b + gs * g);
    float es = lane < npq ? (expf(v[0]) + expf(v[1])) + (expf(v[2]) + expf(v[3])) : 0.f;
    es = wave_sum_dpp(es);
// ... 1 lines not shown
  }
  float ev[NQH], muv[NQH], pre[NQH];
#pragma unroll
  for (int i = 0; i < NQH; ++i) pre[i] = slice_sum(K + DK + ecol[i]);
#pragma unroll
  for (int i = 0; i < NQH; ++i) muv[i] = slice_sum(K + ecol[i]);
  const float lg_own = slice_sum(min(k, K - 1));
#pragma unroll
  for (int i = 0; i < NQH; ++i) ev[i] = valid[i] ? expf(pre[i]) : 0.f;
  if (jitter && row_wave) {
    const __amdgpu_buffer_rsrc_t er = xwg_buffer(p.e_out + (int64_t)(active ? row : 0) * NhP);
#pragma unroll
    for (int i = 0; i < NQH; ++i) {
      const f32x4 qe = quad_gather(ev[i]);
      if (exact) {
        if (valid[i] && (lane & 3) == 0) xwg_store4(er, K + DK + ecol[i], qe[0], qe[1], qe[2], qe[3]);
      } else if (valid[i]) {
        xwg_store(p.e_out + (int64_t)row * NhP + K + DK + ecol[i], ev[i]);
      }
    }
  }
  if (!one_wave_exp) {
    float esum = 0.f;
#pragma unroll
    for (int i = 0; i < NQH; ++i) esum += ev[i];
    esum = wave_sum_dpp(esum);
    if (lane == 0) red[w] = esum;
    __syncthreads();
    if (tid_l < 8) {
      float sx = 0.f;
      for (int q = 0; q < 2 * R; ++q) sx += red[q];
      granule_publish8(p, 0, own, tag + 1, sx, tid_l);
    }
  }
  BSIG_USTAMP(5);
  GranuleEps ge{gran_rep(p, 0, wg & 7), p.n_owner, tag + 1, lane, flagp, p.eps_noise, o.norm, {0ull, 0ull, 0ull, 0ull}};
  float uds = 0.f, lse = 0.f;
  bool bad = false;
  if (row_wave) {
    ge.issue();
    float dmu[NQH], dpre[NQH], dlogit;
    float* xq = XS + ((active ? rr : 0) * KP + k) * 8;
    diag_row_fast_core<KP, NQH>(K, D, active, kok, valid, muv, yd, eu, ev, lg_own, p.min_w, p.ll_limit, p.inv_norm,
                                xq, xq + 4 * KP * 8, h, lane, ge, [] { lds_barrier(); }, dmu, dpre, dlogit, lse, uds, bad);
  BSIG_FSTAMP(6);
    BSIG_USTAMP(7);
    const __amdgpu_buffer_rsrc_t dr = xwg_buffer(p.d_out + (int64_t)(active ? row : 0) * NhP);
    float* drow = p.d_out + (int64_t)(active ? row : 0) * NhP;
#pragma unroll
    for (int i = 0; i < NQH; ++i) {
      const f32x4 qm = quad_gather(dmu[i]), qp = quad_gather(dpre[i]);
      if (exact) {
        if (valid[i] && (lane & 3) == 0) {
          xwg_store4(dr, K + ecol[i], qm[0], qm[1], qm[2], qm[3]);
          xwg_store4(dr, K + DK + ecol[i], qp[0], qp[1], qp[2], qp[3]);
        }
      } else if (valid[i]) {
        xwg_store(drow + K + ecol[i], dmu[i]);
        xwg_store(drow + K + DK + ecol[i], dpre[i]);
      }
    }
    {
      const f32x4 ql = quad_gather(dlogit);
      if (exact) {
        if (active && h == 0 && lane < K && (lane & 3) == 0) xwg_store4(dr, lane, ql[0], ql[1], ql[2], ql[3]);
      } else if (active && h == 0 && lane < KP && kok) {
        xwg_store(drow + k, dlogit);
      }
    }
    uds = wave_sum_dpp(uds);
    BSIG_FSTAMP(7);
    __builtin_amdgcn_s_waitcnt(0);
    BSIG_FSTAMP(8);
    granule_publish8(p, 1, own * 2 * R + w, tag + 2, uds, lane);
    if (h == 0 && lane == 0) granule_publish(loss_granules(p.gran, epoch), own * R + rr, tag + 3, active ? lse : 0.f);
  } else {
    lds_barrier();
  }
  BSIG_USTAMP(9);
  if (own == 0 && w == 0) {
    const float s = granule_gather(loss_granules(p.gran, epoch), p.n_owner * R, tag + 3, lane, flagp);
    if (lane == 0) {
      const float l = -s / (float)B;
      p.train_loss[step] = l;
      if (!isfinite(l)) atomicOr(flagp, 1);
    }
  }
  if (bad) atomicOr(flagp, 1);
}

#define BSIG_U_ROWID(step_)                                                                  \
  if (has_tile && w < p.MT) {                                                                \
    const int64_t r = (int64_t)(step_) * B + min(16 * w + c16_l, B - 1);                     \
    pf_row = p.feat_ids ? (int64_t)p.feat_ids[r] : r;                                        \
  }
#define BSIG_U_PREFETCH()                                                                    \
  if (has_tile && w < p.MT) {                                                                \
    const float* src = p.feats + pf_row * p.ld_feats + k0 + 4 * g4_l;                        \
    if (k0 + p.KS <= p.ld_feats) {          \
      _Pragma("unroll") for (int G6 = 0; G6 < kUSteps / kUGroup; ++G6)                       \
        if (kUGroup * G6 < p.ksteps) {                                                       \
          _Pragma("unroll") for (int S = kUGroup * G6; S < kUGroup * (G6 + 1); ++S)          \
            Freg[S] = *reinterpret_cast<const f32x4*>(src + 16 * S);                         \
        }                                                                                    \
    } else {                                                                                 \
      const int cmax = (int)p.ld_feats - 4 - k0 - 4 * g4_l;                                  \
      _Pragma("unroll") for (int G6 = 0; G6 < kUSteps / kUGroup; ++G6)                       \
        if (kUGroup * G6 < p.ksteps) {                                                       \
          _Pragma("unroll") for (int S = kUGroup * G6; S < kUGroup * (G6 + 1); ++S)          \
            Freg[S] = *reinterpret_cast<const f32x4*>(src + min(16 * S, cmax));              \
        }                                                                                    \
    }                                                                                        \
  }

template <bool DP, int NT, bool XR = false>
__device__ __forceinline__ void unified_workgroup(const UArgs& p, float* smem, const URole& role) {
  static_assert(!(DP && XR), "XR is the resident kernel with the exchange inside, not the per-update launch");
  constexpr int NBW = 16 * NT;
  constexpr int MAXBLK = NT == 1 ? 3 : 2;
  float* Ft = smem;
  float* Wl = Ft + p.KS * kUFP;
  float* XS = Wl + NBW * p.WP;
  float* red = XS + p.xs_floats;
  float* biasl = red + 64;
  const int tid = threadIdx.x, lane0 = tid & 63;
  const int w = __builtin_amdgcn_readfirstlane(tid >> 6);
  const int c16 = lane0 & 15, g4 = lane0 >> 4;
  const int wg = blockIdx.x;
  const int slot = role.tile, own = role.owner;
  constexpr bool has_tile = true;
  const bool has_row = own < p.n_owner;
  const int ks = slot / p.n_blocks, nb = slot - ks * p.n_blocks;
  const int n0 = nb * NBW, k0 = ks * p.KS;
  const int B = p.B, Nh = p.Nh, NhP = p.NhP, D = p.D, K = p.K, DK = D * K;
  constexpr int FP = kUFP;
  const int WP = p.WP;
  int32_t* flagp = p.state + 2;
  const int step0 = p.state[0];
  if (p.prof && p.n_updates > 0 && tid == 0) p.prof[((int64_t)wg * kUProf) * 16 + 14] = wall_clock64();
  double b1t = reinterpret_cast<const double*>(p.state + 12)[0];
  double b2t = reinterpret_cast<const double*>(p.state + 12)[1];
  float a0 = 0.f, a1 = 0.f;
  const AdamK ak{1.0f - (float)p.beta1, (float)p.beta2, 1.0f - (float)p.beta2, p.adam_eps};
  const bool pend = DP && p.adam_pending != 0;
  const bool fresh = !DP && step0 == 0;
  const float pa0 = pend ? reinterpret_cast<const float*>(p.state)[4] : 0.f;
  const float pa1 = pend ? reinterpret_cast<const float*>(p.state)[5] : 0.f;

  float Mr[MAXBLK][NT][4], Vr[MAXBLK][NT][4];
#pragma unroll
  for (int jj = 0; jj < MAXBLK; ++jj)
#pragma unroll
    for (int nt = 0; nt < NT; ++nt)
#pragma unroll
      for (int v = 0; v < 4; ++v) { Mr[jj][nt][v] = 0.f; Vr[jj][nt][v] = 0.f; }
  float bw[NT], bm[NT], bv[NT];
#pragma unroll
  for (int nt = 0; nt < NT; ++nt) { bw[nt] = 0.f; bm[nt] = 0.f; bv[nt] = 0.f; }
  if (has_tile) {
    if (DP && p.quad_ok) {
      const int qpr = p.KS >> 2, total = NBW * qpr;
      for (int base = 0; base < total; base += 3 * kUT) {
        f32x4 Wq[3], Mq[3], Vq[3], Gq[3];
        const f32x4 zero = {0.f, 0.f, 0.f, 0.f};
#pragma unroll
        for (int q = 0; q < 3; ++q) {
          const int idx = base + q * kUT + tid, r = idx / qpr, c = (idx - r * qpr) * 4;
          Wq[q] = zero; Mq[q] = zero; Vq[q] = zero; Gq[q] = zero;
          if (idx < total && n0 + r < Nh && k0 + c < p.Fdim) {
            const int64_t off = p.w_off + (int64_t)(n0 + r) * p.Fdim + k0 + c;
            Wq[q] = *reinterpret_cast<const f32x4*>(p.params + off);
            if (pend) {
              Mq[q] = *reinterpret_cast<const f32x4*>(p.m1 + off);
              Vq[q] = *reinterpret_cast<const f32x4*>(p.m2 + off);
              Gq[q] = *reinterpret_cast<const f32x4*>(p.grads + off);
            }
          }
        }
        if (pend) {
#pragma unroll
          for (int q = 0; q < 3; ++q)
#pragma unroll
            for (int j = 0; j < 4; ++j) {
              float m = Mq[q][j], v = Vq[q][j];
              Wq[q][j] = adam_weight(Gq[q][j], m, v, Wq[q][j], pa0, pa1, ak);
              Mq[q][j] = m; Vq[q][j] = v;
            }
#pragma unroll
          for (int q = 0; q < 3; ++q) {
            const int idx = base + q * kUT + tid, r = idx / qpr, c = (idx - r * qpr) * 4;
            if (idx < total && n0 + r < Nh && k0 + c < p.Fdim) {
              const int64_t off = p.w_off + (int64_t)(n0 + r) * p.Fdim + k0 + c;
              *reinterpret_cast<f32x4*>(p.params + off) = Wq[q];
              *reinterpret_cast<f32x4*>(p.m1 + off) = Mq[q];
              *reinterpret_cast<f32x4*>(p.m2 + off) = Vq[q];
            }
          }
        }
#pragma unroll
        for (int q = 0; q < 3; ++q) {
          const int idx = base + q * kUT + tid, r = idx / qpr, c = (idx - r * qpr) * 4;
          if (idx < total) *reinterpret_cast<f32x4*>(Wl + r * WP + c) = Wq[q];
        }
      }
    } else {
      float Wv[MAXBLK][NT][4], Gv[MAXBLK][NT][4];
#pragma unroll
      for (int jj = 0; jj < MAXBLK; ++jj)
#pragma unroll
        for (int nt = 0; nt < NT; ++nt)
#pragma unroll
          for (int v = 0; v < 4; ++v) {
            const int n = n0 + 16 * nt + 4 * g4 + v, kc = 16 * (w + 8 * jj) + c16;
            Wv[jj][nt][v] = 0.f; Gv[jj][nt][v] = 0.f;
            if (w + 8 * jj < p.KB && n < Nh && k0 + kc < p.Fdim) {
              const int64_t off = p.w_off + (int64_t)n * p.Fdim + k0 + kc;
              Wv[jj][nt][v] = p.params[off];
              if (!fresh) { Mr[jj][nt][v] = p.m1[off]; Vr[jj][nt][v] = p.m2[off]; }
              if (pend) Gv[jj][nt][v] = p.grads[off];
            }
          }
      if (pend) {
#pragma unroll
        for (int jj = 0; jj < MAXBLK; ++jj)
#pragma unroll
          for (int nt = 0; nt < NT; ++nt)
#pragma unroll
            for (int v = 0; v < 4; ++v)
              Wv[jj][nt][v] = adam_weight(Gv[jj][nt][v], Mr[jj][nt][v], Vr[jj][nt][v], Wv[jj][nt][v], pa0, pa1, ak);
#pragma unroll
        for (int jj = 0; jj < MAXBLK; ++jj)
#pragma unroll
          for (int nt = 0; nt < NT; ++nt)
#pragma unroll
            for (int v = 0; v < 4; ++v) {
              const int n = n0 + 16 * nt + 4 * g4 + v, kc = 16 * (w + 8 * jj) + c16;
              if (w + 8 * jj < p.KB && n < Nh && k0 + kc < p.Fdim) {
                const int64_t off = p.w_off + (int64_t)n * p.Fdim + k0 + kc;
                p.params[off] = Wv[jj][nt][v]; p.m1[off] = Mr[jj][nt][v]; p.m2[off] = Vr[jj][nt][v];
              }
            }
      }
#pragma unroll
      for (int jj = 0; jj < MAXBLK; ++jj)
#pragma unroll
        for (int nt = 0; nt < NT; ++nt)
#pragma unroll
          for (int v = 0; v < 4; ++v)
            if (w + 8 * jj < p.KB) Wl[(16 * nt + 4 * g4 + v) * WP + 16 * (w + 8 * jj) + c16] = Wv[jj][nt][v];
    }
    if (ks == 0 && w >= 8 - NT && g4 == 0) {
#pragma unroll
      for (int nt = 0; nt < NT; ++nt) {
        if (w != 8 - NT + nt) continue;
        const int n = n0 + 16 * nt + c16;
        if (n < Nh) {
          bw[nt] = p.params[p.b_off + n];
          if (!fresh) { bm[nt] = p.m1[p.b_off + n]; bv[nt] = p.m2[p.b_off + n]; }
          if (pend) {
            bw[nt] = adam_bias(p.grads[p.b_off + n], bm[nt], bv[nt], bw[nt], pa0, pa1, ak);
            p.params[p.b_off + n] = bw[nt]; p.m1[p.b_off + n] = bm[nt]; p.m2[p.b_off + n] = bv[nt];
          }
        }
        biasl[16 * nt + c16] = bw[nt];
      }
    }
  }
  if (tid == 0)
    red[63] = (__hip_atomic_load(flagp, __ATOMIC_RELAXED, __HIP_MEMORY_SCOPE_AGENT) & 2) ? 1.f : 0.f;
  if (has_tile && p.MT < kUMT)
    for (int idx = tid; idx < p.KS * (kUFP / 4); idx += kUT) {
      const f32x4 zero = {0.f, 0.f, 0.f, 0.f};
      *reinterpret_cast<f32x4*>(Ft + 4 * idx) = zero;
    }

  UOwn o;
  u_own_init(p, o, own, true, XS, red, Ft, lane0);
  const int eo = (own - p.n_owner + p.T) % p.T;
  const bool has_erow = p.do_eval && eo < p.NE;
  int pending_eval = -1;

  f32x4 Freg[kUSteps];
  {
    const f32x4 zero = {0.f, 0.f, 0.f, 0.f};
#pragma unroll
    for (int S = 0; S < kUSteps; ++S) Freg[S] = zero;
  }
  int64_t pf_row = 0;
  {
    const int c16_l = c16, g4_l = g4;
    if (p.n_updates > 0) { BSIG_U_ROWID(step0) BSIG_U_PREFETCH() }
  }
  __syncthreads();

  for (int t = 0; t < p.n_updates; ++t) {
    int tid_l = tid, c16_l = c16, g4_l = g4;
    asm volatile("" : "+v"(tid_l), "+v"(c16_l), "+v"(g4_l));
    const int step = step0 + t;
    const unsigned epoch = (unsigned)step + 1u;
    const uint32_t tag = epoch * 4u;
    if (red[63] != 0.f) break;
    BSIG_USTAMP(0);
    {
      if (w < p.MT) {
        const bool rok = 16 * w + c16_l < B;
        if (16 * (w + 1) > B || k0 + p.KS > p.Fdim) {
          const f32x4 zero = {0.f, 0.f, 0.f, 0.f};
#pragma unroll
          for (int S = 0; S < kUSteps; ++S)
            if (!(rok && k0 + 16 * S + 4 * g4_l < p.Fdim)) Freg[S] = zero;
        }
        f32x4 acc[NT];
#pragma unroll
        for (int nt = 0; nt < NT; ++nt) {
          const f32x4 zero = {0.f, 0.f, 0.f, 0.f};
          acc[nt] = ks == 0 ? *reinterpret_cast<const f32x4*>(biasl + 16 * nt + 4 * g4_l) : zero;
        }
        const float* ap = Wl + c16_l * WP + 4 * g4_l;
        float* ftp = Ft + (4 * g4_l) * FP + 16 * w + u_rowpos(c16_l);
#pragma unroll
        for (int G6 = 0; G6 < kUSteps / kUGroup; ++G6) {
          if (kUGroup * G6 < p.ksteps) {
#pragma unroll
            for (int S = kUGroup * G6; S < kUGroup * (G6 + 1); ++S) {
              const f32x4 b4 = Freg[S];
#pragma unroll
              for (int nt = 0; nt < NT; ++nt) {
                const f32x4 a4 = *reinterpret_cast<const f32x4*>(ap + nt * 16 * WP + 16 * S);
                acc[nt] = umfma(a4[0], b4[0], acc[nt]);
                acc[nt] = umfma(a4[1], b4[1], acc[nt]);
                acc[nt] = umfma(a4[2], b4[2], acc[nt]);
                acc[nt] = umfma(a4[3], b4[3], acc[nt]);
              }
              ftp[(16 * S + 0) * FP] = b4[0];
              ftp[(16 * S + 1) * FP] = b4[1];
              ftp[(16 * S + 2) * FP] = b4[2];
              ftp[(16 * S + 3) * FP] = b4[3];
            }
          }
        }
        BSIG_USTAMP(1);
        if (rok) {
          const __amdgpu_buffer_rsrc_t sr = xwg_buffer(p.slabs + (int64_t)ks * B * NhP + n0);
#pragma unroll
          for (int nt = 0; nt < NT; ++nt)
            xwg_store4(sr, (16 * w + c16_l) * NhP + 16 * nt + 4 * g4_l, acc[nt][0], acc[nt][1], acc[nt][2], acc[nt][3]);
        }
      }
      __builtin_amdgcn_s_waitcnt(0);
      __syncthreads();
      if (tid_l == 0) flag_raise(p.flag_fwd, slot, epoch);
      BSIG_USTAMP(3);
      if (t + 1 < p.n_updates) { BSIG_U_ROWID(step + 1) }
    }
    if (tid_l == 0)
      red[63] = (__hip_atomic_load(flagp, __ATOMIC_RELAXED, __HIP_MEMORY_SCOPE_AGENT) & 2) ? 1.f : 0.f;
    b1t *= p.beta1; b2t *= p.beta2;
    a0 = (float)(p.lr / (1.0 - b1t));
    a1 = (float)(1.0 / sqrt(1.0 - b2t));

    if (has_row) u_own_update(p, o, t, w, lane0, wg);
    if (__builtin_expect(pending_eval >= 0, 0)) {
      __syncthreads();
      if (has_erow) u_owner_eval(p, XS, red, eo, pending_eval, u_eval_stream(p, o, pending_eval, false), o.a);
      pending_eval = -1;
    }
    if (__builtin_expect(p.do_eval && step > 0 && (step - 1) % p.eval_every == 0, 0)) {
      const int e = u_evals_before(step, p.eval_every) - 1;
      u_tile_eval<NT>(p, Wl, biasl, slot, ks, n0, k0, e);
      pending_eval = e;
    }

    {
      int tid_l = tid, c16_l = c16, g4_l = g4;
      asm volatile("" : "+v"(tid_l), "+v"(c16_l), "+v"(g4_l));
      const int lane = tid_l & 63;
      if (t + 1 < p.n_updates) { BSIG_U_PREFETCH() }
      BSIG_USTAMP(2);
      if (w == 0) {
        unsigned long long* sug = gran_rep(p, 1, wg & 7);
        const int n_su = (p.T - p.G >= p.n_owner && u_fast_kind(p) != 0) ? p.n_owner * 2 * p.R : p.n_owner;
        granule_wait_one(sug, slot % n_su, tag + 2, flagp);
        const float su = granule_gather(sug, n_su, tag + 2, lane, flagp);
        if (lane == 0) red[62] = p.eps_noise != 0.f ? p.eps_noise / ((float)B * (float)DK) * su : 0.f;
      }
      __syncthreads();
      BSIG_USTAMP(10);
      {
        const float c = red[62];
        const int sg_lo = K + DK, sg_hi = K + 2 * DK;
        const bool any_e = c != 0.f && n0 + NBW > sg_lo && n0 < sg_hi;
        const __amdgpu_buffer_rsrc_t dr = xwg_buffer(p.d_out + n0), er = xwg_buffer(p.e_out + n0);
        constexpr int QN = NBW / 4;
        constexpr int total = 16 * kUMT * QN;
        for (int base = 0; base < total; base += 2 * kUT) {
          f32x4 q[2], e[2];
#pragma unroll
          for (int u = 0; u < 2; ++u) {
            const int idx = base + u * kUT + tid_l;
            const int b = idx / QN, c4 = (idx - b * QN) * 4;
            const bool ok = idx < total && b < B;
            const f32x4 zero = {0.f, 0.f, 0.f, 0.f};
            q[u] = ok ? xwg_load4(dr, b * NhP + c4) : zero;
            e[u] = ok && any_e ? xwg_load4(er, b * NhP + c4) : zero;
          }
#pragma unroll
          for (int u = 0; u < 2; ++u) {
            const int idx = base + u * kUT + tid_l;
            const int b = idx / QN, c4 = (idx - b * QN) * 4;
            if (idx < total) {
#pragma unroll
              for (int j = 0; j < 4; ++j) {
                const int n = n0 + c4 + j;
                const float ev = (n >= sg_lo && n < sg_hi) ? e[u][j] : 0.f;
                XS[(c4 + j) * FP + u_rowpos(b)] = q[u][j] + c * ev;
              }
            }
          }
        }
      }
      __syncthreads();
      BSIG_USTAMP(11);
      const int n4 = (B + 3) >> 2;
      [[maybe_unused]] const int xr_cols = p.Fdim - k0, xr_kb = min(p.KB, (xr_cols + 15) >> 4), xr_nt = 64 * p.Fdim;
      [[maybe_unused]] const int xr_col = 16 * w + (c16_l & ~3);
      [[maybe_unused]] const int xr_lane = 4 * ((n0 + 4 * g4_l + (c16_l & 3)) * p.Fdim + k0 + 16 * w + (c16_l & ~3));
      [[maybe_unused]] __amdgpu_buffer_rsrc_t xr_rsrc;
      if constexpr (XR) xr_rsrc = xwg_buffer_n(p.grads + p.w_off, 4 * Nh * p.Fdim);
      const float* ap = XS + c16_l * FP + 4 * g4_l;
#pragma unroll
      for (int jj = 0; jj < MAXBLK; ++jj) {
        const int j = w + 8 * jj;
        if (j < p.KB) {
          f32x4 acc[NT];
          [[maybe_unused]] float wv[NT][4];
          if constexpr (!DP && !XR) {
#pragma unroll
            for (int nt = 0; nt < NT; ++nt)
#pragma unroll
              for (int v = 0; v < 4; ++v) wv[nt][v] = Wl[(16 * nt + 4 * g4_l + v) * WP + 16 * j + c16_l];
          }
          const float* bp = Ft + (16 * j + c16_l) * FP + 4 * g4_l;
          const f32x4 zero = {0.f, 0.f, 0.f, 0.f};
#pragma unroll
          for (int nt = 0; nt < NT; ++nt) acc[nt] = zero;
          f32x4 qa[2][NT], qb[2];
          qb[0] = *reinterpret_cast<const f32x4*>(bp);
#pragma unroll
          for (int nt = 0; nt < NT; ++nt) qa[0][nt] = *reinterpret_cast<const f32x4*>(ap + nt * 16 * FP);
#pragma unroll
          for (int S = 0; S < kUMT; ++S) {
            if (S + 1 < kUMT) {
              qb[(S + 1) & 1] = *reinterpret_cast<const f32x4*>(bp + 16 * (S + 1));
#pragma unroll
              for (int nt = 0; nt < NT; ++nt)
                qa[(S + 1) & 1][nt] = *reinterpret_cast<const f32x4*>(ap + nt * 16 * FP + 16 * (S + 1));
            }
            __builtin_amdgcn_sched_barrier(0);
            const f32x4 b = qb[S & 1];
            if (S < kUMT - 1) {
// ... 44 lines not shown
#pragma unroll
            for (int nt = 0; nt < NT; ++nt)
#pragma unroll
              for (int v = 0; v < 4; ++v) Wl[(16 * nt + 4 * g4_l + v) * WP + 16 * j + c16_l] = wv[nt][v];
          }
        }
      }
      if (ks == 0 && w >= 8 - NT) {
#pragma unroll
        for (int nt = 0; nt < NT; ++nt) {
          if (w != 8 - NT + nt) continue;
          const float* xp = XS + (16 * nt + c16_l) * FP + 4 * g4_l;
          f32x4 x4[kUMT];
#pragma unroll
          for (int S = 0; S < kUMT; ++S) x4[S] = *reinterpret_cast<const f32x4*>(xp + 16 * S);
          __builtin_amdgcn_sched_barrier(0);
          float g = 0.f;
#pragma unroll
          for (int S = 0; S < kUMT; ++S) g += (x4[S][0] + x4[S][1]) + (x4[S][2] + x4[S][3]);
          g += __shfl_xor(g, 16, 64);
          g += __shfl_xor(g, 32, 64);
          if (g4_l == 0) {
            const int n = n0 + 16 * nt + c16_l;
            if (DP) {
              if (n < Nh) p.grads[p.b_off + n] = g;
            } else if constexpr (XR) {
              if (n < Nh) xwg_store(p.grads + p.b_off + n, g);
            } else {
              bw[nt] = adam_bias(g, bm[nt], bv[nt], bw[nt], a0, a1, ak);
              biasl[16 * nt + c16_l] = bw[nt];
            }
          }
        }
      }
      if constexpr (XR) {
        __builtin_amdgcn_s_waitcnt(0);
        __syncthreads();
        BSIG_USTAMP(13);
        if (tid_l == 0)
          xr_hand_off(p.xr_count, p.xr_ready, p.xr_done, p.xr_base, (unsigned)t + 1u, (unsigned)p.G, flagp);
        (void)run_aborted(flagp, red, tid);
        BSIG_USTAMP(14);
        if (ks == 0 && w >= 8 - NT && g4_l == 0) {
#pragma unroll
          for (int nt = 0; nt < NT; ++nt) {
            if (w != 8 - NT + nt) continue;
            const int n = n0 + 16 * nt + c16_l;
            const float g = n < Nh ? xwg_load(p.grads + p.b_off + n) : 0.f;
            bw[nt] = adam_bias(g, bm[nt], bv[nt], bw[nt], a0, a1, ak);
            biasl[16 * nt + c16_l] = bw[nt];
          }
        }
#pragma unroll
        for (int jj = 0; jj < MAXBLK; ++jj) {
          const int j = w + 8 * jj;
          if (j < p.KB) {
            float gr[NT][4];
            f32x4 gq[NT];
            const f32x4 zero = {0.f, 0.f, 0.f, 0.f};
#pragma unroll
            for (int nt = 0; nt < NT; ++nt)
              gq[nt] = j < xr_kb ? xwg_load4s(xr_rsrc, xr_col + 128 * jj < xr_cols ? xr_lane + jj * 512 + nt * xr_nt : -1, 0) : zero;
#pragma unroll
            for (int nt = 0; nt < NT; ++nt) {
              const f32x4 c = quad_transpose4(gq[nt][0], gq[nt][1], gq[nt][2], gq[nt][3], c16_l & 3);
#pragma unroll
              for (int v = 0; v < 4; ++v) gr[nt][v] = c[v];
            }
#pragma unroll
            for (int nt = 0; nt < NT; ++nt)
#pragma unroll
              for (int v = 0; v < 4; ++v) {
                float* wp = Wl + (16 * nt + 4 * g4_l + v) * WP + 16 * j + c16_l;
                *wp = adam_weight(gr[nt][v], Mr[jj][nt][v], Vr[jj][nt][v], *wp, a0, a1, ak);
              }
          }
        }
      }
      BSIG_USTAMP(8);
      lds_barrier();
      BSIG_USTAMP(12);
    }
  }
  if constexpr (XR) {
    if (slot == 0 && tid == 0 &&
        (__hip_atomic_load(flagp, __ATOMIC_RELAXED, __HIP_MEMORY_SCOPE_AGENT) & 2))
      __hip_atomic_store(p.xr_ready, p.xr_base + (unsigned)p.n_total, __ATOMIC_RELAXED, __HIP_MEMORY_SCOPE_SYSTEM);
  }

  if (p.do_eval && !run_aborted(flagp, red, tid)) {
    if (pending_eval >= 0) {
      if (has_erow) u_owner_eval(p, XS, red, eo, pending_eval, u_eval_stream(p, o, pending_eval, false), o.a);
      pending_eval = -1;
    }
    if (step0 + p.n_updates == p.n_total && (!DP || p.n_updates == 0)) {
      const int e = u_evals_before(p.n_total - 1, p.eval_every);
      __syncthreads();
      u_tile_eval<NT>(p, Wl, biasl, slot, ks, n0, k0, e);
      if (has_erow) u_owner_eval(p, XS, red, eo, e, u_eval_stream(p, o, e, true), o.a);
    }
  }
  if (!DP && has_tile) {
#pragma unroll
    for (int jj = 0; jj < MAXBLK; ++jj)
#pragma unroll
      for (int nt = 0; nt < NT; ++nt)
#pragma unroll
        for (int v = 0; v < 4; ++v) {
          const int n = n0 + 16 * nt + 4 * g4 + v, kc = 16 * (w + 8 * jj) + c16;
          if (w + 8 * jj < p.KB && n < Nh && k0 + kc < p.Fdim) {
            const int64_t off = p.w_off + (int64_t)n * p.Fdim + k0 + kc;
            p.params[off] = Wl[(16 * nt + 4 * g4 + v) * WP + kc];
            p.m1[off] = Mr[jj][nt][v]; p.m2[off] = Vr[jj][nt][v];
          }
        }
    if (ks == 0 && w >= 8 - NT && g4 == 0) {
#pragma unroll
      for (int nt = 0; nt < NT; ++nt) {
        if (w != 8 - NT + nt) continue;
        const int n = n0 + 16 * nt + c16;
        if (n < Nh) { p.params[p.b_off + n] = bw[nt]; p.m1[p.b_off + n] = bm[nt]; p.m2[p.b_off + n] = bv[nt]; }
      }
    }
  }
  if (p.prof && p.n_updates > 0 && tid == 0) {
    __builtin_amdgcn_s_waitcnt(0);
    p.prof[((int64_t)wg * kUProf) * 16 + 13] = wall_clock64();
  }
  if (wg == 0 && tid == 0 && p.n_updates > 0) {
    int32_t* st = p.state;
    reinterpret_cast<double*>(st + 12)[0] = b1t;
    reinterpret_cast<double*>(st + 12)[1] = b2t;
    reinterpret_cast<float*>(st)[4] = a0;
    reinterpret_cast<float*>(st)[5] = a1;
    int n_ev = 0;
    if (p.do_eval) {
      n_ev = u_evals_before(step0 + p.n_updates, p.eval_every) - u_evals_before(step0, p.eval_every);
      if (!DP && step0 + p.n_updates == p.n_total && (p.n_total - 1) % p.eval_every != 0) ++n_ev;
    }
    reinterpret_cast<uint64_t*>(st + 8)[1] += (uint64_t)(p.n_updates + n_ev);
    st[0] = step0 + p.n_updates;
  }
}

__device__ __forceinline__ void owner_only_workgroup(const UArgs& p, float* smem, const URole& role, int NBW, bool dp) {
  float* XS = smem + p.KS * kUFP + NBW * p.WP;
  float* red = XS + p.xs_floats;
  const int tid = threadIdx.x, lane0 = tid & 63;
  const int w = __builtin_amdgcn_readfirstlane(tid >> 6);
  const int wg = blockIdx.x;
  int32_t* flagp = p.state + 2;
  UOwn o;
  u_own_init(p, o, role.owner, false, XS, red, smem, lane0);
  const bool has_row = role.owner < p.n_owner;
  const int eo = (role.owner - p.n_owner + p.T) % p.T;
  const bool has_erow = p.do_eval && eo < p.NE;
  const int fk = u_fast_kind(p);
  int pending_eval = -1;
  for (int t = 0; t < p.n_updates; ++t) {
    const int step = o.step0 + t;
    if (run_aborted(flagp, red, tid)) break;
    BSIG_USTAMP(0);
    if (has_row) {
      switch (fk) {
        case 4 * 8 + 1: u_own_update_fast<4, 1>(p, o, t, w, lane0, wg); break;
        case 4 * 8 + 2: u_own_update_fast<4, 2>(p, o, t, w, lane0, wg); break;
        case 4 * 8 + 4: u_own_update_fast<4, 4>(p, o, t, w, lane0, wg); break;
        case 8 * 8 + 1: u_own_update_fast<8, 1>(p, o, t, w, lane0, wg); break;
        case 8 * 8 + 2: u_own_update_fast<8, 2>(p, o, t, w, lane0, wg); break;
        case 8 * 8 + 4: u_own_update_fast<8, 4>(p, o, t, w, lane0, wg); break;
        case 16 * 8 + 1: u_own_update_fast<16, 1>(p, o, t, w, lane0, wg); break;
        case 16 * 8 + 2: u_own_update_fast<16, 2>(p, o, t, w, lane0, wg); break;
        case 16 * 8 + 4: u_own_update_fast<16, 4>(p, o, t, w, lane0, wg); break;
        default: u_own_update(p, o, t, w, lane0, wg); break;
      }
    }
    if (__builtin_expect(pending_eval >= 0, 0)) {
      __syncthreads();
      if (has_erow) u_owner_eval(p, XS, red, eo, pending_eval, u_eval_stream(p, o, pending_eval, false), o.a);
      pending_eval = -1;
    }
    if (__builtin_expect(p.do_eval && step > 0 && (step - 1) % p.eval_every == 0, 0))
      pending_eval = u_evals_before(step, p.eval_every) - 1;
    __syncthreads();
  }
  if (p.do_eval && !run_aborted(flagp, red, tid)) {
    if (pending_eval >= 0 && has_erow)
      u_owner_eval(p, XS, red, eo, pending_eval, u_eval_stream(p, o, pending_eval, false), o.a);
    if (o.step0 + p.n_updates == p.n_total && (!dp || p.n_updates == 0)) {
      const int e = u_evals_before(p.n_total - 1, p.eval_every);
      __syncthreads();
      if (has_erow) u_owner_eval(p, XS, red, eo, e, u_eval_stream(p, o, e, true), o.a);
    }
  }
}

template <bool DP, int NT, bool XR = false>
__global__ __launch_bounds__(kUT) void linear_head_updates_kernel(UArgs p) {
  extern __shared__ __attribute__((aligned(16))) float smem[];
#ifndef BSIG_HOST_SAN_BUILD
  const URole role = wg_role(blockIdx.x, p.T, p.G);
  if (role.tile < 0) owner_only_workgroup(p, smem, role, 16 * NT, DP);
  else unified_workgroup<DP, NT, XR>(p, smem, role);
#endif
}

__global__ void spin_kernel(long long ticks, int* sink) {
  extern __shared__ float spin_lds[];
  spin_lds[threadIdx.x] = 1.f;
  const long long t0 = wall_clock64();
  while (wall_clock64() - t0 < ticks) __builtin_amdgcn_s_sleep(64);
  if (spin_lds[threadIdx.x] == 2.f) sink[0] = 1;
}
int debug_spin(int blocks, size_t lds_bytes, int ms, hipStream_t st) {
  BSIG_REQUIRE(blocks >= 1 && ms >= 0 && lds_bytes <= (size_t)kULds, "debug_spin: bad args");
  BSIG_HIP(hipFuncSetAttribute(reinterpret_cast<const void*>(spin_kernel),
                               hipFuncAttributeMaxDynamicSharedMemorySize, kULds));
  hipLaunchKernelGGL(spin_kernel, dim3(blocks), dim3(256), std::max<size_t>(lds_bytes, 1024), st,
                     (long long)ms * 100000LL , (int*)nullptr);
  BSIG_CHECK_LAUNCH("debug_spin");
  return BSIG_OK;
}

static long long* g_prof = nullptr;
void persist_set_profile_buffer(void* buf) { g_prof = reinterpret_cast<long long*>(buf); }
void* persist_profile_buffer() { return g_prof; }

static bool u_geom_try(const PersistShape& s, int NT, int KS, UGeom* g, double* cost) {
  const int NBW = 16 * NT, max_blk = NT == 1 ? 3 : 2;
  g->Bp = (int)round_up(s.batch, 16);
  g->MT = g->Bp / 16;
  g->FP = kUFP;
  g->Nh = s.n_comp + 2 * s.out_dim * s.n_comp;
  g->per_wave = g->Nh + s.out_dim + 3 * s.n_comp;
  g->NT = NT;
  g->n_blocks = ceil_div(g->Nh, NBW);
  g->NhP = g->n_blocks * NBW;
  g->KS = KS;
  g->ksteps = g->KB = KS / 16;
  if (g->ksteps > kUSteps || g->KB > 8 * max_blk) return false;
  g->WP = KS + 4;
  g->k_slices = ceil_div(s.feat_dim, KS);
  g->G = g->n_blocks * g->k_slices;
  if (g->G > kXwgMax) return false;
  const int spare = kXwgMax - g->G;
  bool mixed = false;
  static const bool force_mixed = [] { const char* e = getenv("BSIG_PERSIST_MIXED"); return e && e[0] == '1'; }();
  if (!force_mixed && spare >= s.batch) { g->R = 1; g->T = g->G + s.batch; }
  else if (!force_mixed && spare >= ceil_div(s.batch, 2)) { g->R = 2; g->T = g->G + ceil_div(s.batch, 2); }
  else {
    mixed = true;
    g->T = std::max(g->G, std::min(s.batch, kXwgMax));
    g->R = ceil_div(s.batch, std::min(g->T, s.batch));
    if (g->R > kUT / 64) return false;
  }
  g->n_owner = ceil_div(s.batch, g->R);
  g->eval_passes = s.max_test > 0 ? ceil_div(s.max_test, s.batch) : 0;
  g->NE = 1; g->RE = 1;
  if (g->eval_passes > 0) {
    const int idle = g->T - g->n_owner;
    const int re_all = ceil_div(s.max_test, g->T);
    const int re_idle = idle > 0 ? ceil_div(s.max_test, idle) : 1 << 20;
    if (re_idle <= kUT / 64 && re_idle <= 2 * re_all) { g->NE = idle; g->RE = re_idle; }
    else { g->NE = g->T; g->RE = re_all; }
    if (g->RE > kUT / 64) { g->eval_passes = 0; g->NE = 1; g->RE = 1; }
    else g->NE = std::min(g->NE, ceil_div(s.max_test, g->RE));
  }
  auto lds_of = [&] {
    g->xs_floats = (int)round_up(std::max(NBW * g->FP, std::max(g->R, g->RE) * g->per_wave), 4);
    g->lds = ((size_t)g->KS * g->FP + (size_t)NBW * g->WP + g->xs_floats + 64 + NBW) * sizeof(float);
  };
  lds_of();
  if (g->lds > (size_t)kULds && g->eval_passes > 0 && g->RE > g->R) {
    g->eval_passes = 0; g->NE = 1; g->RE = 1;
    lds_of();
  }
  if (g->lds > (size_t)kULds) return false;
  g->slab_floats = (size_t)g->k_slices * s.batch * g->NhP;
  g->dout_floats = (size_t)s.batch * g->NhP;
  g->eval_floats = (size_t)3 * g->eval_passes * g->slab_floats;
  const double mfma_us = 32.0 * (2.0 * 4 * g->ksteps * NT + 4.0 * kUMT * NT * ceil_div(g->KB, 4)) / 2200.0;
  const double tile_us = mixed ? (double)s.batch * KS * 4 / 20000.0 : 0.0;
  const double sum_us = 0.035 * g->k_slices * g->R;
  *cost = mfma_us + tile_us + sum_us;
  return true;
}

static bool u_geom(const PersistShape& s, UGeom* g) {
  if (s.batch < 1 || s.batch > 16 * kUMT || s.feat_dim < 4 || s.feat_dim % 4 != 0 || s.out_dim < 1 ||
      s.n_comp < 1 || s.n_comp > 64)
    return false;
  const int groups = 64 / s.n_comp;
  if (ceil_div(s.out_dim, groups) > kElemsPerLane) return false;
  bool found = false;
  double best = 0.0;
  static const int force_nt = [] { const char* e = getenv("BSIG_PERSIST_NT"); return e ? atoi(e) : 0; }();
  static const int force_ks = [] { const char* e = getenv("BSIG_PERSIST_KS"); return e ? atoi(e) : 0; }();
  for (int NT = 1; NT <= 2; ++NT)
    for (int groups6 = 1; groups6 <= kUSteps / kUGroup; ++groups6) {
      UGeom c;
      double cost = 0.0;
      if ((force_nt && NT != force_nt) || (force_ks && 16 * kUGroup * groups6 != force_ks)) continue;
      if (!u_geom_try(s, NT, 16 * kUGroup * groups6, &c, &cost)) continue;
      if (!found || cost < best) { *g = c; best = cost; found = true; }
    }
  return found;
}

int persist_geometry(const PersistShape& s, int32_t* out) {
  UGeom g;
  for (int i = 0; i < 16; ++i) out[i] = 0;
  if (!u_geom(s, &g)) return 0;
  const int32_t v[13] = {g.NT, g.KS, g.n_blocks, g.k_slices, g.G, g.T, g.n_owner, g.R, g.NE, g.RE,
                         g.eval_passes, (int32_t)g.lds, std::max(0, g.n_owner - (g.T - g.G))};
  for (int i = 0; i < 13; ++i) out[i] = v[i];
  return 1;
}

static int u_allow_dynamic_lds() {
  static bool done[64] = {};
  const void* kernels[6] = {reinterpret_cast<const void*>(linear_head_updates_kernel<false, 1>),
                            reinterpret_cast<const void*>(linear_head_updates_kernel<false, 2>),
                            reinterpret_cast<const void*>(linear_head_updates_kernel<true, 1>),
                            reinterpret_cast<const void*>(linear_head_updates_kernel<false, 1, true>),
                            reinterpret_cast<const void*>(linear_head_updates_kernel<true, 2>),
                            reinterpret_cast<const void*>(linear_head_updates_kernel<false, 2, true>)};
  return allow_dynamic_lds(done, kernels, 6, kULds);
}

template <int NT>
static bool u_can_host(const UGeom& g) {
  int dev = 0;
  hipDeviceProp_t prop;
  if (hipGetDevice(&dev) != hipSuccess || hipGetDeviceProperties(&prop, dev) != hipSuccess) return false;
  if (prop.multiProcessorCount < g.T || (size_t)prop.maxSharedMemoryPerMultiProcessor < g.lds) return false;
  int per_cu = 0;
  if (u_allow_dynamic_lds() != BSIG_OK ||
      hipOccupancyMaxActiveBlocksPerMultiprocessor(&per_cu, linear_head_updates_kernel<false, NT>, kUT, g.lds) != hipSuccess)
    return false;
  return per_cu >= 1;
}

static size_t u_data_bytes(const UGeom& g) {
  return round_up<size_t>((g.slab_floats + 2 * g.dout_floats + g.eval_floats) * sizeof(float), 256);
}
static size_t u_sync_bytes() { return 2 * kFlagArr * sizeof(unsigned) + (6 + 16) * kGranArr * 8 + 256; }

bool persist_resolve(const PersistShape& s, UGeom* g, PersistEngine* e) {
  UGeom c;
  if (!u_geom(s, &c) || !(c.NT == 1 ? u_can_host<1>(c) : u_can_host<2>(c))) return false;
  *g = c;
  e->kind = 1; e->streams = false;
  e->eval_single = e->eval_dp = c.eval_passes > 0;
  e->workspace_bytes = u_data_bytes(c) + u_sync_bytes();
  return true;
}

int persist_reset_regions(const UGeom& g, void* workspace, size_t workspace_bytes, ZeroRegion* regions) {
  BSIG_REQUIRE(workspace && workspace_bytes >= u_data_bytes(g) + u_sync_bytes(),
               "persistent updates: workspace too small");
  char* base = reinterpret_cast<char*>(workspace);
  const size_t slab_bytes = g.slab_floats * sizeof(float);
  regions[0] = ZeroRegion{base + slab_bytes, 2 * g.dout_floats * sizeof(float)};
  regions[1] = ZeroRegion{base + u_data_bytes(g), u_sync_bytes()};
  return BSIG_OK;
}

template <int NT>
static int u_launch(const UGeom& g, const UArgs& p, bool dp, int n, bool do_eval, hipStream_t st) {
  if (p.xr_ready)
    hipLaunchKernelGGL((linear_head_updates_kernel<false, NT, true>), dim3(g.T), dim3(kUT), g.lds, st, p);
  else if (dp)
    hipLaunchKernelGGL((linear_head_updates_kernel<true, NT>), dim3(g.T), dim3(kUT), g.lds, st, p);
  else
    hipLaunchKernelGGL((linear_head_updates_kernel<false, NT>), dim3(g.T), dim3(kUT), g.lds, st, p);
  BSIG_CHECK_LAUNCH("linear_head_updates");
  return BSIG_OK;
}

int persist_run(const PersistShape& s, const UGeom& g, const PersistBuffers& b, int n, hipStream_t st) {
  BSIG_REQUIRE(b.feats && b.y && b.ids && b.params && b.exp_avg && b.exp_avg_sq && b.state &&
                   b.train_loss && b.workspace, "persistent updates: null buffer");
  BSIG_REQUIRE(b.workspace_bytes >= u_data_bytes(g) + u_sync_bytes(), "persistent updates: workspace too small");
  BSIG_REQUIRE(b.ld_feats % 4 == 0 && aligned(b.feats, 16) && b.ld_feats >= s.feat_dim,
               "persistent updates: features must be 16-byte aligned rows");
  BSIG_REQUIRE(!(b.adam_pending && !b.grads), "persistent updates: pending Adam step without gradients");
  BSIG_REQUIRE(!(b.grads && n > 1 && !b.xr_ready), "persistent updates: data-parallel launches take one update");
  BSIG_REQUIRE(!(b.xr_ready && !(b.grads && b.xr_done && !b.adam_pending && b.n_total == n)),
               "persistent updates: a resident data-parallel launch takes the whole call");
  BSIG_REQUIRE(!(b.xr_ready && !(b.w_off % 4 == 0 && s.feat_dim % 4 == 0 && aligned(b.grads, 16) &&
                                 (int64_t)g.Nh * s.feat_dim < ((int64_t)1 << 29))),
               "persistent updates: a resident data-parallel launch moves 16-byte gradient quads");
  if (n <= 0 && !b.adam_pending && !b.do_eval) return BSIG_OK;
  UArgs p{};
  p.B = s.batch; p.Bp = g.Bp; p.MT = g.MT;
  p.Fdim = s.feat_dim; p.KS = g.KS; p.ksteps = g.ksteps; p.KB = g.KB; p.WP = g.WP;
  p.Nh = g.Nh; p.NhP = g.NhP; p.D = s.out_dim; p.K = s.n_comp;
  p.n_blocks = g.n_blocks; p.k_slices = g.k_slices; p.G = g.G; p.T = g.T; p.n_owner = g.n_owner; p.R = g.R;
  p.n_updates = std::max(n, 0); p.xs_floats = g.xs_floats;
  {
    const char* e = getenv("BSIG_PERSIST_FAST_ROWS");
    p.fast_rows = (e && e[0] == '0') ? 0 : 1;
  }
  p.grads = b.grads; p.adam_pending = b.adam_pending;
  p.xr_ready = b.xr_ready; p.xr_done = b.xr_done; p.xr_base = b.xr_base;
  p.xr_count = reinterpret_cast<unsigned*>(reinterpret_cast<char*>(b.workspace) + u_data_bytes(g) + u_sync_bytes() - 256);
  p.feats = b.feats; p.ld_feats = b.ld_feats; p.feat_ids = b.feat_ids; p.y = b.y; p.ldy = b.ldy; p.ids = b.ids;
  p.params = b.params; p.m1 = b.exp_avg; p.m2 = b.exp_avg_sq; p.w_off = b.w_off; p.b_off = b.b_off;
  p.quad_ok = (p.w_off % 4 == 0 && p.Fdim % 4 == 0 &&
               ((reinterpret_cast<uintptr_t>(b.params) | reinterpret_cast<uintptr_t>(b.exp_avg) |
                 reinterpret_cast<uintptr_t>(b.exp_avg_sq) | reinterpret_cast<uintptr_t>(b.grads)) & 15) == 0) ? 1 : 0;
  p.state = b.state; p.train_loss = b.train_loss;
  const PersistHyper& hy = b.hy;
  p.lr = hy.lr; p.beta1 = hy.beta1; p.beta2 = hy.beta2;
  p.adam_eps = hy.adam_eps; p.eps_noise = hy.eps_noise; p.min_w = hy.min_weight;
  p.ll_limit = hy.ll_limit; p.inv_norm = 1.0f / (float)hy.norm_batch;
  char* base = reinterpret_cast<char*>(b.workspace);
  p.slabs = reinterpret_cast<float*>(base);
  p.d_out = p.slabs + g.slab_floats;
  p.e_out = p.d_out + g.dout_floats;
  p.eval_slabs = p.e_out + g.dout_floats;
  char* sync = base + u_data_bytes(g);
  p.flag_fwd = reinterpret_cast<unsigned*>(sync);
  p.flag_eval = p.flag_fwd + kFlagArr;
  p.gran = reinterpret_cast<unsigned long long*>(sync + 2 * kFlagArr * sizeof(unsigned));
  p.gran_eval = p.gran + 3 * kGranArr;
  p.gran_rep = p.gran + 6 * kGranArr;
  p.NE = g.NE; p.RE = g.RE;
  if (b.do_eval) {
    BSIG_REQUIRE(g.eval_passes > 0 && b.n_test >= 1 && b.n_test <= g.eval_passes * s.batch &&
                     b.n_test <= g.NE * g.RE && b.y_test && b.test_loss && b.eval_every >= 1 && b.n_total >= 1,
                 "persistent updates: in-launch evaluation not covered");
    p.do_eval = 1; p.eval_every = b.eval_every; p.n_total = b.n_total; p.n_test = b.n_test;
    p.eval_passes = ceil_div(b.n_test, s.batch); p.eval_row0 = b.eval_row0;
    p.y_test = b.y_test; p.ldy_test = b.ldy_test; p.test_loss = b.test_loss;
  }
  p.prof = reinterpret_cast<long long*>(persist_profile_buffer());
  if (p.prof) {
    const char* t0 = getenv("BSIG_PROF_T0");
    p.prof_t0 = t0 ? atoi(t0) : 0;
  }
  if (b.xr_ready && !p.n_total) p.n_total = n;
  return g.NT == 1 ? u_launch<1>(g, p, b.grads != nullptr, n, b.do_eval != 0, st)
                   : u_launch<2>(g, p, b.grads != nullptr, n, b.do_eval != 0, st);
}

}
```

### bayes_sim_ig_amd/csrc/persist.h

```cpp
#pragma once
#include "common.h"

namespace bsig {

struct PersistEngine {
  int kind = 0;
  bool streams = false;
  bool eval_single = false;
  bool eval_dp = false;
  size_t workspace_bytes = 0;
};

struct PersistShape {
  int batch, feat_dim, out_dim, n_comp;
  int max_test = 0;
};

struct UGeom {
  int NT, Bp, MT, FP, KS, ksteps, KB, WP, Nh, NhP, n_blocks, k_slices, G, T, n_owner, R;
  int per_wave, xs_floats;
  int eval_passes, NE, RE;
  size_t lds, slab_floats, dout_floats, eval_floats;
};

struct PersistHyper {
  double lr, beta1, beta2; float adam_eps, eps_noise, min_weight, ll_limit;
  int64_t norm_batch;
};

struct PersistCommon {
  const float* y; int64_t ldy;
  const int32_t* ids;
  float* params; float* exp_avg; float* exp_avg_sq;
  int32_t* state;
  float* train_loss;
  void* workspace; size_t workspace_bytes;
  float* grads = nullptr; int adam_pending = 0;
  unsigned* xr_ready = nullptr; const unsigned* xr_done = nullptr; unsigned xr_base = 0;
  int do_eval = 0; int eval_every = 1; int n_total = 0; int n_test = 0;
  const float* y_test = nullptr; int64_t ldy_test = 0;
  float* test_loss = nullptr;
  PersistHyper hy;
};

struct PersistBuffers : PersistCommon {
  const float* feats; int64_t ld_feats;
  const int32_t* feat_ids;
  int64_t w_off, b_off;
  int64_t eval_row0 = 0;
};

bool persist_resolve(const PersistShape& s, UGeom* g, PersistEngine* e);
struct ZeroRegion { void* ptr; size_t bytes; };
int persist_reset_regions(const UGeom& g, void* workspace, size_t workspace_bytes, ZeroRegion* regions);
int persist_run(const PersistShape& s, const UGeom& g, const PersistBuffers& b, int n, hipStream_t st);

int persist_geometry(const PersistShape& s, int32_t* out);

inline int allow_dynamic_lds(bool (&done)[64], const void* const* kernels, int n, int bytes) {
  int dev = 0;
  BSIG_HIP(hipGetDevice(&dev));
  if (done[dev & 63]) return BSIG_OK;
  for (int i = 0; i < n; ++i)
    BSIG_HIP(hipFuncSetAttribute(kernels[i], hipFuncAttributeMaxDynamicSharedMemorySize, bytes));
  done[dev & 63] = true;
  return BSIG_OK;
}

void persist_set_profile_buffer(void* buf);
int debug_spin(int blocks, size_t lds_bytes, int ms, hipStream_t st);
void* persist_profile_buffer();

}
```

### bayes_sim_ig_amd/mdnn.py

```python
import ctypes as C
import os
from collections import OrderedDict

import numpy as np
import torch
import torch.nn as nn

from . import _lib
from . import pdf
from . import dp as _dp
from .summarizers import CrossCorrFactors

_ACT_CODES = {nn.Tanh: _lib.ACT_TANH, nn.ReLU: _lib.ACT_RELU,
              nn.LeakyReLU: _lib.ACT_LEAKY_RELU, nn.Sigmoid: _lib.ACT_SIGMOID,
              nn.Identity: _lib.ACT_IDENTITY}


def _on_model_device(fn):
    import functools

    @functools.wraps(fn)
    def wrapped(self, *args, **kwargs):
        flat = getattr(self, '_flat', None)
        if flat is None or not flat.is_cuda or flat.device.index == torch.cuda.current_device():
# ... 125 lines not shown
        cfg.rff_scale = self._rff_scale
        cfg.head.out_dim = int(self.output_dim)
        cfg.head.n_comp = int(self.n_gaussians)
        cfg.head.full_cov = 1 if self.Lower is not None else 0
        cfg.head.eps_noise = float(type(self).EPS_NOISE)
        cfg.head.min_weight = float(type(self).MIN_WEIGHT)
        cfg.head.ll_limit = float(type(self).LL_LIMIT)
        cfg.lr, cfg.beta1, cfg.beta2, cfg.adam_eps = float(self.lr), 0.9, 0.999, 1e-8
        return cfg

    def _linears(self):
        mods = [self.net[2 * l] for l in range(len(self._hidden))]
        mods += [self.pi, self.mu, self.Diag[0]]
        if self.Lower is not None:
            mods.append(self.Lower)
        return mods

    def _flatten(self, device):
        lib = _lib.load()
        cfg = self._cfg()
        total = int(lib.bsig_mdn_param_count(C.byref(cfg)))
        assert total > 0, lib.bsig_last_error().decode()
        n_off = 2 * (len(self._hidden) + 4)
        offs = (C.c_int64 * n_off)()
        _lib.check(lib.bsig_mdn_param_offsets(C.byref(cfg), offs, n_off))
        flat = torch.zeros(total, dtype=torch.float32, device=device)
        grads = torch.zeros(total, dtype=torch.float32, device=device)
        self._param_slices = []
        widths = [self.input_dim if self._rff_feats == 0 else self._rff_feats] + self._hidden_stored
        with torch.no_grad():
            for i, mod in enumerate(self._linears()):
                l = min(i, len(self._hidden))
                rows = self._hidden_stored[i] if i < len(self._hidden) else mod.weight.shape[0]
                for j, prm in enumerate((mod.weight, mod.bias)):
                    o = int(offs[2 * i + j])
                    full = (rows, widths[l]) if j == 0 else (rows,)
                    real = tuple(prm.shape)
                    sub = tuple(slice(0, d) for d in real)
                    self._param_slices.append((o, full, real))
                    view = flat[o:o + int(np.prod(full))].view(full)[sub]
                    view.copy_(prm.detach().to(dtype=torch.float32))
                    prm.data = view
                    prm.grad = grads[o:o + int(np.prod(full))].view(full)[sub]
        self._flat, self._flat_grad = flat, grads
        self._exp_avg = torch.zeros_like(flat)
        self._exp_avg_sq = torch.zeros_like(flat)
        if self.output_lows is not None:
            self.output_lows = self.output_lows.to(device)
            self.output_highs = self.output_highs.to(device)
        self.device = str(device) if not isinstance(device, str) else device
        self._drop_plan()

    def _apply(self, fn, *args, **kwargs):
        super()._apply(fn, *args, **kwargs)
        prm = next(self.parameters())
        if prm.dtype != torch.float32:
            raise NotImplementedError('the HIP estimator computes in fp32 only')
        self._flatten(prm.device)
        return self

    def _drop_plan(self):
        if getattr(self, '_plan', None):
            _lib.load().bsig_fit_destroy(self._plan)
        self._plan, self._plan_key = None, None
        self._bufs = {}

    def __del__(self):
        try:
            self._drop_plan()
        except Exception:
            pass

    def _snapshot(self):
        return (self._flat.clone(), self._exp_avg.clone(), self._exp_avg_sq.clone(),
                np.random.get_state(), torch.get_rng_state())

    def _restore(self, snap):
        self._flat.copy_(snap[0]); self._exp_avg.copy_(snap[1]); self._exp_avg_sq.copy_(snap[2])
        np.random.set_state(snap[3]); torch.set_rng_state(snap[4])

    def _resident_calls(self):
        return self._dp.resident_calls() if self._dp is not None else 0

    def _give_up_a_level(self, resident_calls_before):
        if self._dp is not None and self._dp.resident_calls() > resident_calls_before:
            import warnings
            warnings.warn('bayes_sim_ig_amd: a data-parallel launch that stays resident across the gradient '
                          'exchange timed out waiting for the exchange; this model continues with one launch '
                          'per update', RuntimeWarning, stacklevel=3)
            self._dp.set_resident(False)
            return
        self._disable_persistent()

    def _disable_persistent(self):
        import warnings
        warnings.warn('bayes_sim_ig_amd: a persistent update launch timed out waiting for another workgroup '
                      '(GPU shared with another process?); this model continues on the per-phase kernels, '
                      'which are slower', RuntimeWarning, stacklevel=3)
        self._no_persistent = True
        self._drop_plan()

    def _gpu(self):
        lib = _lib.require_gpu()
        if not self._flat.is_cuda:
            raise RuntimeError("MDNN was built with device=%r: the estimator runs on "
                               "MI355X only, construct it with device='cuda:N' "
                               "(no CPU fallback)" % (self.device,))
        return lib

    def _buf(self, name, numel, dtype=torch.float32):
        t = self._bufs.get(name)
        if t is None or t.numel() < numel or t.dtype != dtype:
            t = torch.empty(max(int(numel), 1), dtype=dtype, device=self._flat.device)
            self._bufs[name] = t
        return t

    def _rff_args(self):
        return None, 0, None

    def _seed(self):
        if type(self).EPS_NOISE == 0.0:
            return 0
        return int(torch.randint(0, 2 ** 62, (1,)).item())

    @_on_model_device
    def _head_forward(self, x):
        lib = self._gpu()
        cfg = self._cfg()
        xs, ldx = _lib.as_f32_rows(x, self._flat.device)
        assert xs.shape[1] == self.input_dim
        b = xs.shape[0]
        nh = int(lib.bsig_head_width(C.byref(cfg.head)))
        out = torch.empty((b, nh), dtype=torch.float32, device=xs.device)
        ws_bytes = int(lib.bsig_mdn_workspace_bytes(C.byref(cfg), b))
        ws = self._buf('fwd_ws', ws_bytes // 4 + 1)
        coeff, ldc, off = self._rff_args()
        _lib.check(lib.bsig_mdn_head_forward(
            C.byref(cfg), _lib.ptr(self._flat), _lib.ptr(coeff), ldc, _lib.ptr(off),
            _lib.ptr(xs), ldx, None, b, _lib.ptr(out), nh, _lib.ptr(ws),
            ws.numel() * 4, _lib.stream()))
        return cfg, out

    @_on_model_device
    def forward(self, x, noise=None):
        lib = self._gpu()
        cfg, out = self._head_forward(x)
        b, d, k = out.shape[0], self.output_dim, self.n_gaussians
        dev = out.device
        weights = torch.empty((b, k), dtype=torch.float32, device=dev)
        mu = torch.empty((b, d, k), dtype=torch.float32, device=dev)
        l_d = torch.empty((b, d, k), dtype=torch.float32, device=dev)
        low = None
        if self.Lower is not None:
            low = torch.empty((b, self.L_size, k), dtype=torch.float32, device=dev)
        flag = torch.zeros(1, dtype=torch.int32, device=dev)
        ws = self._buf('head_ws', 64 + int(lib.bsig_head_workspace_bytes(C.byref(cfg.head), b)) // 4)
        nz = None if noise is None else noise.to(dev, torch.float32).contiguous()
        seed = self._seed()
        _lib.check(lib.bsig_mdn_head_outputs(
            C.byref(cfg.head), _lib.ptr(out), out.stride(0), b, _lib.ptr(nz),
            seed, 0, _lib.ptr(weights), _lib.ptr(mu), _lib.ptr(l_d),
            _lib.ptr(low), _lib.ptr(flag), _lib.ptr(ws), ws.numel() * 4, _lib.stream()))
        assert int(flag.item()) == 0
        self._fwd_ctx = (weights, x, nz, seed) if torch.is_grad_enabled() else None
        return weights, mu, l_d, low

    @_on_model_device
# ... 8 lines not shown
        s = L_d.to(dev, torch.float32).contiguous()
        lo = None if L is None else L.to(dev, torch.float32).contiguous()
        head = cfg.head
        head.full_cov = 0 if lo is None else 1
        loss = torch.zeros(1, dtype=torch.float32, device=dev)
        flag = torch.zeros(1, dtype=torch.int32, device=dev)
        ws = self._buf('head_ws', 64 + int(lib.bsig_head_workspace_bytes(C.byref(head), b)) // 4)
        _lib.check(lib.bsig_mdn_nll_from_tuple(
            C.byref(head), _lib.ptr(w), _lib.ptr(m), _lib.ptr(s), _lib.ptr(lo),
            _lib.ptr(ys), ldy, b, _lib.ptr(loss), _lib.ptr(flag), _lib.ptr(ws),
            ws.numel() * 4, _lib.stream()))
        assert int(flag.item()) == 0
        ctx = getattr(self, '_fwd_ctx', None)
        if torch.is_grad_enabled() and ctx is not None and ctx[0] is weights:
            return _FusedNLL.apply(loss[0], self, ctx[1], ys, ctx[2], ctx[3], *self.parameters())
        return loss[0]

    @_on_model_device
    def loss_and_grad(self, x, y, rows=None, noise=None, norm_batch=None, seed=None,
                      grads_out=None):
        lib = self._gpu()
        cfg = self._cfg()
        dev = self._flat.device
        xs, ldx = _lib.as_f32_rows(x, dev)
        ys, ldy = _lib.as_f32_rows(y, dev)
        ridx = None
        b = xs.shape[0]
        if rows is not None:
            ridx = torch.as_tensor(rows, dtype=torch.int32, device=dev).contiguous()
            b = ridx.numel()
        ws_bytes = int(lib.bsig_mdn_workspace_bytes(C.byref(cfg), b))
        ws = self._buf('grad_ws', ws_bytes // 4 + 1)
        loss = torch.zeros(1, dtype=torch.float32, device=dev)
        flag = torch.zeros(1, dtype=torch.int32, device=dev)
        nz = None if noise is None else noise.to(dev, torch.float32).contiguous()
        coeff, ldc, off = self._rff_args()
        _lib.check(lib.bsig_mdn_loss_grad(
            C.byref(cfg), _lib.ptr(self._flat), _lib.ptr(coeff), ldc, _lib.ptr(off),
            _lib.ptr(xs), ldx, _lib.ptr(ys), ldy, _lib.ptr(ridx), b,
            int(norm_batch or b), _lib.ptr(nz), self._seed() if seed is None else int(seed), 0,
            _lib.ptr(self._flat_grad if grads_out is None else grads_out), _lib.ptr(loss),
            _lib.ptr(flag), _lib.ptr(ws),
            ws.numel() * 4, _lib.stream()))
        assert int(flag.item()) == 0
        return loss[0]

    @_on_model_device
    def adam_step(self, t):
        lib = self._gpu()
        _lib.check(lib.bsig_adam_flat(
            _lib.ptr(self._flat), _lib.ptr(self._flat_grad), _lib.ptr(self._exp_avg),
            _lib.ptr(self._exp_avg_sq), self._flat.numel(), float(self.lr), 0.9, 0.999,
            1e-8, int(t), _lib.stream()))

    def enable_data_parallel(self, group=None, transport=None):
        self._dp = _dp.DataParallel(group)
        if self._flat.is_cuda:
            with _lib.on_device(self._flat.device):
                self._dp.init_comm(self._flat.device, transport)
        self._dp.broadcast(self._flat)
        self._dp_sync_extra()
        return self

    def _dp_sync_extra(self):
        """Replica state outside the flat parameter buffer (MDRFF: the RFF frequencies)."""

    def run_training(self, x_data, y_data, n_updates, batch_size, test_frac=0.2,
                     ids_table=None, _defer=False, _feats=None):
        if _defer or not self._flat.is_cuda:
            return self._run_training_once(x_data, y_data, n_updates, batch_size, test_frac,
                                           ids_table, _defer, _feats)
        snap = self._snapshot() if self._may_time_out() else None
        for attempt in range(3):
            calls0 = self._resident_calls()
            try:
                return self._run_training_once(x_data, y_data, n_updates, batch_size, test_frac,
                                               ids_table, False, _feats)
            except PersistentTimeout:
                if snap is None or attempt == 2:
                    raise
                self._restore(snap)
                self._give_up_a_level(calls0)

    def _may_time_out(self):
        if getattr(self, '_no_persistent', False) or os.environ.get('BSIG_NO_PERSISTENT') == '1':
            return False
        return self._plan is None or bool(_lib.load().bsig_fit_is_persistent(self._plan))

    @_on_model_device
    def _run_training_once(self, x_data, y_data, n_updates, batch_size, test_frac=0.2,
                           ids_table=None, _defer=False, _feats=None):
        assert x_data.shape[0] == y_data.shape[0]
        lib = self._gpu()
        self.train()
        cfg = self._cfg()
        dev = self._flat.device
        d, n_tot = self.output_dim, x_data.shape[0]
        n_train = max(int(n_tot * (1.0 - test_frac)), 1)
        n_test = n_tot - n_train
        st = _lib.stream()
        key = (batch_size, max(n_test, self._bufs.get('cap_test', 0)), n_updates,
               cfg.head.eps_noise, cfg.lr, cfg.head.min_weight, cfg.head.ll_limit,
               max(n_train, self._bufs.get('cap_train', 0)))
        if self._plan is None or self._plan_key != key:
            if self._plan:
                lib.bsig_fit_destroy(self._plan)
            handle = C.c_void_p()
            flags = _lib.PLAN_NO_PERSISTENT if getattr(self, '_no_persistent', False) else 0
            _lib.check(lib.bsig_fit_create_ex(C.byref(cfg), batch_size, key[7], key[1],
                                              n_updates, flags, C.byref(handle)))
            self._plan, self._plan_key = handle, key
            self._bufs['cap_test'], self._bufs['cap_train'] = key[1], key[7]
        factored = isinstance(x_data, CrossCorrFactors)
        if factored and not lib.bsig_fit_accepts_factor_rows(self._plan, x_data.s_dim, x_data.a_dim):
            x_data, factored = x_data.materialize(), False
        ldy = _lib.round_up(d, 4)
        ys, ldy_src = _lib.as_f32_rows(y_data, dev)
        assert x_data.shape[1] == self.input_dim and ys.shape[1] == d
        cap = self._bufs.get('cap_rows', 0)
        if n_tot > cap:
            self._bufs.pop('x_stage', None), self._bufs.pop('y_stage', None)
            self._bufs['cap_rows'] = n_tot
        if factored:
            x_stage, _ = _lib.as_f32_rows(x_data.factors, dev)
            ldx = x_stage.stride(0) if n_tot > 1 else x_stage.shape[1]
            bind_flags = (_lib.FIT_GRAPH if type(self).USE_GRAPH else 0) | \
                (_lib.FIT_SPLIT_ADAM if self._dp is not None else 0)
            eval_fac = bool(lib.bsig_fit_evaluates_from_factors(self._plan, x_data.s_dim, x_data.a_dim, bind_flags))
            x_held = x_data[n_train:].materialize() if n_test > 0 and not eval_fac else None
            self._bufs['x_keepalive'] = (x_stage, x_held)
        else:
            xs, ldx_src = _lib.as_f32_rows(x_data, dev)
            ldx = _lib.round_up(self.input_dim, 4)
            x_stage = self._buf('x_stage', self._bufs['cap_rows'] * ldx)
            if _feats is None or not lib.bsig_fit_takes_features(self._plan, n_train):
                _lib.check(lib.bsig_copy_rows(_lib.ptr(xs), ldx_src, None, _lib.ptr(x_stage), ldx,
                                              n_tot, self.input_dim, st))
        y_stage = self._buf('y_stage', self._bufs['cap_rows'] * ldy)
        if self.output_lows is not None:
            _lib.check(lib.bsig_normalize_rows(
                _lib.ptr(ys), ldy_src, _lib.ptr(self.output_lows),
                _lib.ptr(self.output_highs), _lib.ptr(y_stage), ldy, n_tot, d, st))
        else:
            _lib.check(lib.bsig_copy_rows(_lib.ptr(ys), ldy_src, None, _lib.ptr(y_stage),
                                          ldy, n_tot, d, st))
        n_ids = n_updates * batch_size
        ids_dev = self._buf('ids', max(n_ids, 1), torch.int32)
        def upload_ids():
            if ids_table is None:
                ids_np = np.random.randint(0, n_train, (n_updates, batch_size), dtype=np.int32)
            else:
                ids_np = np.asarray(ids_table)
                assert ids_np.shape == (n_updates, batch_size)
            ring = self._bufs.setdefault('ids_ring', {'slots': [], 'next': 0})
            if not ring['slots'] or ring['slots'][0][0].numel() < n_ids:
                ring['slots'] = [[torch.empty(max(n_ids, 1), dtype=torch.int32, pin_memory=True), None]
                                 for _ in range(4)]
            slot = ring['slots'][ring['next'] % 4]
            ring['next'] += 1
            if slot[1] is not None:
                slot[1].synchronize()
            slot[0][:n_ids].copy_(torch.from_numpy(np.ascontiguousarray(ids_np, dtype=np.int32)).reshape(-1))
            ids_dev[:n_ids].copy_(slot[0][:n_ids], non_blocking=True)
            slot[1] = torch.cuda.Event()
            slot[1].record()

        late_ids = n_ids >= (1 << 16) and (cfg.rff_feats == 0 or
                                           bool(lib.bsig_fit_takes_features(self._plan, n_train)))
        if not late_ids:
            upload_ids()
        every = max(n_updates // 5, 1)
        eval_its = [it for it in range(n_updates)
                    if it % every == 0 or it + 1 == n_updates]
        train_loss = self._buf('train_loss', n_updates)
        test_loss = self._buf('test_loss', len(eval_its))
        state = self._buf('state', 16, torch.int32)
        ws = self._buf('fit_ws', int(lib.bsig_fit_workspace_bytes(self._plan)) // 4 + 1)
        coeff, ldc, off = self._rff_args()
        fb = _lib.FitBuffers()
        fb.params, fb.grads = self._flat.data_ptr(), self._flat_grad.data_ptr()
        fb.exp_avg, fb.exp_avg_sq = self._exp_avg.data_ptr(), self._exp_avg_sq.data_ptr()
        fb.rff_coeff = None if coeff is None else coeff.data_ptr()
        fb.ld_coeff = ldc
        fb.rff_offset = None if off is None else off.data_ptr()
        fb.x_train, fb.ldx_train, fb.n_train = x_stage.data_ptr(), ldx, n_train
        fb.y_train, fb.ldy_train = y_stage.data_ptr(), ldy
        fb.x_test, fb.ldx_test, fb.n_test = x_stage.data_ptr() + 4 * n_train * ldx, ldx, n_test
        if factored and n_test > 0:
            if x_held is not None:
                fb.x_test, fb.ldx_test = x_held.data_ptr(), x_held.stride(0)
            else:
                fb.x_test, fb.ldx_test = None, 0
        fb.y_test, fb.ldy_test = y_stage.data_ptr() + 4 * n_train * ldy, ldy
        fb.ids_table = ids_dev.data_ptr()
        fb.train_loss, fb.test_loss = train_loss.data_ptr(), test_loss.data_ptr()
# ... 71 lines not shown
```

### include/bsig.h

```cpp
#ifndef BSIG_H
#define BSIG_H

#include <stddef.h>
#include <stdint.h>

#ifdef __cplusplus
extern "C" {
#endif

typedef void* bsig_stream_t;

#define BSIG_OK 0
#define BSIG_EINVAL (-1)
#define BSIG_ELAUNCH (-2)
#define BSIG_EUNSUPPORTED (-3)
#define BSIG_ENONFINITE (-4)

const char* bsig_last_error(void);
int bsig_version(void);
uint64_t bsig_abi_info(int which);
int bsig_device_count(void);


int64_t bsig_summary_dim(int kind, int traj_len, int sd, int ad, int depth);
// ... 92 lines not shown
int bsig_colsum(const float* x, int64_t ld, int64_t rows, int64_t cols, float* out,
                void* workspace, size_t workspace_bytes, bsig_stream_t stream);
int bsig_normalize_rows(const float* theta, int64_t ld_in, const float* lows,
                        const float* highs, float* out, int64_t ld_out, int64_t rows,
                        int64_t cols, bsig_stream_t stream);
int bsig_copy_rows(const float* src, int64_t ld_src, const int32_t* rows, float* dst,
                   int64_t ld_dst, int64_t n_rows, int64_t cols, bsig_stream_t stream);

#define BSIG_MAX_HIDDEN 8

typedef struct bsig_mdn_cfg {
  int32_t input_dim;
  int32_t n_hidden;
  int32_t hidden[BSIG_MAX_HIDDEN];
  int32_t activation;
  int32_t rff_feats;
  int32_t rff_cos_only;
  float rff_scale;
  bsig_head_dims head;
  float lr, beta1, beta2, adam_eps;
} bsig_mdn_cfg;

int64_t bsig_mdn_param_count(const bsig_mdn_cfg* cfg);
int bsig_mdn_param_offsets(const bsig_mdn_cfg* cfg, int64_t* offsets, int n_offsets);
size_t bsig_mdn_workspace_bytes(const bsig_mdn_cfg* cfg, int64_t max_batch);

int bsig_mdn_head_forward(const bsig_mdn_cfg* cfg, const float* params,
                          const float* rff_coeff, int64_t ld_coeff,
                          const float* rff_offset, const float* x, int64_t ldx,
                          const int32_t* x_rows, int64_t batch, float* head_out,
                          int64_t ld_head, void* workspace, size_t workspace_bytes,
                          bsig_stream_t stream);

int bsig_mdn_loss_grad(const bsig_mdn_cfg* cfg, const float* params,
                       const float* rff_coeff, int64_t ld_coeff,
                       const float* rff_offset, const float* x, int64_t ldx,
                       const float* y, int64_t ldy, const int32_t* rows,
                       int64_t batch, int64_t norm_batch, const float* noise,
                       uint64_t seed, uint64_t stream_id, float* grads, float* loss,
                       int32_t* nonfinite, void* workspace, size_t workspace_bytes,
                       bsig_stream_t stream);

typedef struct bsig_fit_buffers {
  float* params; float* grads; float* exp_avg; float* exp_avg_sq;
  const float* rff_coeff; int64_t ld_coeff; const float* rff_offset;
  const float* x_train; int64_t ldx_train; int64_t n_train;
  const float* y_train; int64_t ldy_train;
  const float* x_test; int64_t ldx_test; int64_t n_test;
  const float* y_test; int64_t ldy_test;
  const int32_t* ids_table;
  float* train_loss;
  float* test_loss;
  int32_t* state;
  void* workspace; size_t workspace_bytes;
  int32_t x_kind; int32_t x_s; int32_t x_a;
  const float* x_test_factors; int64_t ldx_test_factors;
} bsig_fit_buffers;
#define BSIG_X_ROWS 0
#define BSIG_X_CROSSCORR_FACTORS 1

typedef struct bsig_fit_plan bsig_fit_plan;

int bsig_fit_create(const bsig_mdn_cfg* cfg, int64_t batch, int64_t max_test_rows,
                    int64_t n_updates, bsig_fit_plan** plan);
int bsig_fit_create_sized(const bsig_mdn_cfg* cfg, int64_t batch, int64_t max_train_rows,
                          int64_t max_test_rows, int64_t n_updates, bsig_fit_plan** plan);
#define BSIG_PLAN_NO_PERSISTENT 1
int bsig_fit_create_ex(const bsig_mdn_cfg* cfg, int64_t batch, int64_t max_train_rows,
                       int64_t max_test_rows, int64_t n_updates, int plan_flags, bsig_fit_plan** plan);
void bsig_fit_destroy(bsig_fit_plan* plan);
size_t bsig_fit_workspace_bytes(const bsig_fit_plan* plan);
#define BSIG_FIT_GRAPH 1
#define BSIG_FIT_SPLIT_ADAM 2
int bsig_fit_bind(bsig_fit_plan* plan, const bsig_fit_buffers* buffers, int flags);
int bsig_fit_set_features(bsig_fit_plan* plan, const float* feats, int64_t ld_feats,
                          int64_t rows, bsig_stream_t stream);
int bsig_fit_takes_features(const bsig_fit_plan* plan, int64_t n_train);
int bsig_fit_begin(bsig_fit_plan* plan, uint64_t seed, int64_t norm_batch,
                   bsig_stream_t stream);
int bsig_fit_run(bsig_fit_plan* plan, int64_t n_updates, bsig_stream_t stream);
int bsig_fit_updates(bsig_fit_plan* plan, int64_t n_updates, bsig_stream_t stream);
int bsig_fit_pack_logs(bsig_fit_plan* plan, int64_t n_updates, float* out,
                       bsig_stream_t stream);
int bsig_fit_grad(bsig_fit_plan* plan, bsig_stream_t stream);
int bsig_fit_apply(bsig_fit_plan* plan, bsig_stream_t stream);
int bsig_fit_flush(bsig_fit_plan* plan, bsig_stream_t stream);
int bsig_fit_accepts_factors(const bsig_fit_plan* plan);
int bsig_fit_accepts_factor_rows(const bsig_fit_plan* plan, int s_dim, int a_dim);
int bsig_fit_evaluates_from_factors(const bsig_fit_plan* plan, int s_dim, int a_dim, int bind_flags);
int bsig_fit_is_persistent(const bsig_fit_plan* plan);
int bsig_fit_eval(bsig_fit_plan* plan, bsig_stream_t stream);

typedef struct bsig_comm bsig_comm;
#define BSIG_COMM_ID_BYTES 128
int bsig_comm_unique_id(void* id_out);
int bsig_comm_init(const void* unique_id, int world, int rank, int device,
                   bsig_comm** comm);
enum { BSIG_EXCHANGE_SUM = 0, BSIG_EXCHANGE_BROADCAST = 1 };
typedef int (*bsig_exchange_fn)(void* ctx, int op, float* buf, int64_t n, int root,
                                bsig_stream_t stream);
int bsig_comm_init_external(int world, int rank, bsig_exchange_fn exchange, void* ctx,
                            bsig_comm** comm);
int bsig_comm_transport(const bsig_comm* comm);
int bsig_comm_world(const bsig_comm* comm);
int bsig_comm_rank(const bsig_comm* comm);
int64_t bsig_comm_resident_calls(const bsig_comm* comm);
void bsig_comm_set_resident(bsig_comm* comm, int mode);
int bsig_comm_resident_mode(const bsig_comm* comm);
int bsig_comm_allreduce(bsig_comm* comm, float* buf, int64_t n, bsig_stream_t stream);
int bsig_comm_broadcast(bsig_comm* comm, float* buf, int64_t n, int root,
                        bsig_stream_t stream);
void bsig_comm_destroy(bsig_comm* comm);

int bsig_fit_run_dp(bsig_fit_plan* plan, bsig_comm* comm, int64_t n_updates,
                    float* reduced_logs, bsig_stream_t stream);
int bsig_fit_dp_graph_status(const bsig_fit_plan* plan, char* msg, size_t msg_bytes);

void bsig_debug_persist_profile(void* device_buffer);
int bsig_debug_spin(int blocks, size_t lds_bytes, int ms, bsig_stream_t stream);
int bsig_debug_persist_geometry(int batch, int feat_dim, int out_dim, int n_comp, int max_test,
                                int32_t* out);
int bsig_debug_persist_mdnn_geometry(int batch, int input_dim, int out_dim, int n_comp, int full_cov,
                                     int max_test, int32_t* out);

int bsig_debug_mfma_vs_fma(const float* a, const float* b, int k, int32_t* mismatches, bsig_stream_t stream);

#ifdef __cplusplus
}
#endif
#endif
```

Measured before the change: 544,600 pairs/s.

## Run many fit chunks in one persistent-kernel launch via a device chunk table

Adds a block launch path in which one persistent kernel trains and evaluates many sequential chunks, driven by a device-side chunk descriptor table (rows, seeds, ids offsets, loss slots). Logs are packed per chunk by a single follow-up kernel. This is meant to remove the per-chunk host round trips, binds, begins and graph launches that add up over 100 chunks. In exchange it adds a large new code path with chunk validation, a pinned ring of index buffers, and fallback to the old per-chunk path when the plan cannot run in block mode.

New measurement: 566,600 pairs/s (median of 6 runs). 1.04x the previous value.

```diff
diff --git a/bayes_sim_ig_amd/_lib.py b/bayes_sim_ig_amd/_lib.py
--- a/bayes_sim_ig_amd/_lib.py
+++ b/bayes_sim_ig_amd/_lib.py
@@ -1,6 +1,7 @@
 import ctypes as C
 import os
 
+import numpy as np
 import torch
 
 _HERE = os.path.dirname(os.path.abspath(__file__))
@@ -43,6 +44,24 @@
                 ('state', vp), ('workspace', vp), ('workspace_bytes', sz),
                 ('x_kind', i32), ('x_s', i32), ('x_a', i32),
                 ('x_test_factors', vp), ('ldx_test_factors', i64)]
+
+
+FIT_CHUNK = np.dtype([('row0', '<i8'), ('n_train', '<i4'), ('n_test', '<i4'), ('ids_off', '<i8'),
+                      ('seed', '<u8'), ('rng_ctr0', '<u8'), ('n_updates', '<i4'), ('eval_every', '<i4'),
+                      ('train_slot', '<i4'), ('test_slot', '<i4'), ('upd_base', '<i4'), ('eval_base', '<i4')])
+
+
+def fit_chunk_table(sizes, seeds, n_updates, batch_size, test_frac):
+    every = max(n_updates // 5, 1)
+    n_evals = len([it for it in range(n_updates) if it % every == 0 or it + 1 == n_updates])
+    table = np.zeros(len(sizes), dtype=FIT_CHUNK)
+    row0 = 0
+    for c, (n_tot, seed) in enumerate(zip(sizes, seeds)):
+        n_train = max(int(n_tot * (1.0 - test_frac)), 1)
+        table[c] = (row0, n_train, n_tot - n_train, c * n_updates * batch_size, seed, 1, n_updates, every,
+                    c * n_updates, c * n_evals, c * n_updates, c * n_evals)
+        row0 += n_tot
+    return table
 
 
 _PROTOS = {
@@ -126,6 +145,9 @@
     'bsig_comm_broadcast': (C.c_int, [vp, vp, i64, C.c_int, vp]),
     'bsig_comm_destroy': (None, [vp]),
     'bsig_fit_pack_logs': (C.c_int, [vp, i64, vp, vp]),
+    'bsig_fit_block_chunks': (C.c_int, [vp, i64]),
+    'bsig_fit_run_block': (C.c_int, [vp, vp, i64, i64, vp, i64, vp, i64, vp, vp, C.c_int, vp, vp, vp, i64, vp]),
+    'bsig_debug_block_launch': (C.c_int, [C.c_int, C.c_int, C.c_int]),
     'bsig_fit_run_dp': (C.c_int, [vp, vp, i64, vp, vp]),
 }
 COMM_ID_BYTES = 128
diff --git a/bayes_sim_ig_amd/bayes_sim.py b/bayes_sim_ig_amd/bayes_sim.py
--- a/bayes_sim_ig_amd/bayes_sim.py
+++ b/bayes_sim_ig_amd/bayes_sim.py
@@ -108,11 +108,12 @@
             snap = self.model._snapshot()
             for _ in range(2):
                 calls0 = self.model._resident_calls()
+                blocks0 = getattr(self.model, '_block_launches', 0)
                 try:
                     return self._fit_once(params, traj_states, traj_actions)
                 except PersistentTimeout:
                     self.model._restore(snap)
-                    self.model._give_up_a_level(calls0)
+                    self.model._give_up_a_level(calls0, blocks0)
         return self._fit_once(params, traj_states, traj_actions)
 
     def _fit_once(self, params, traj_states, traj_actions):
@@ -141,6 +142,20 @@
                 lo, hi = done, min(n, done + block)
                 summ = self._summarize(traj_states[lo:hi], traj_actions[lo:hi], flag, lazy=True)
                 feats = self.model.rff.to_features(summ) if is_rff else None
+                if feats is not None and dp is None:
+                    sizes, at = [], lo
+                    while at < hi:
+                        sizes.append(BayesSim.get_n_trajs_per_batch(n, at))
+                        at += sizes[-1]
+                    sizes = sizes[:self.model.block_prefix(sizes, BayesSim.TEST_FRACTION)]
+                    rows = sum(sizes)
+                    logs = self.model.run_training_block(
+                        feats[:rows], params[lo:lo + rows], sizes, BayesSim.NUM_GRAD_UPDATES,
+                        BayesSim.MINIBATCH_SIZE, BayesSim.TEST_FRACTION) if sizes else None
+                    if logs is not None:
+                        pending.extend(logs)
+                        done += rows
+                        continue
             if block:
                 pending.append(self.run_training(
                     params[done:done + m], None, None, _defer=True,
diff --git a/bayes_sim_ig_amd/csrc/estimator.hip b/bayes_sim_ig_amd/csrc/estimator.hip
--- a/bayes_sim_ig_amd/csrc/estimator.hip
+++ b/bayes_sim_ig_amd/csrc/estimator.hip
@@ -403,8 +403,12 @@
                           (int)std::min<int64_t>(p->max_test, 1 << 20)};
 }
 
+struct BlockRun {
+  const float* feats; int64_t ld_feats; const float* y; int64_t ldy; const int32_t* ids;
+  const bsig_fit_chunk* chunks; int n_chunks, max_test, total_updates; float* train_loss; float* test_loss;
+};
 static int enqueue_persistent(bsig_fit_plan* p, int n, hipStream_t st, int eval_total = 0,
-                              const CommXr* xr = nullptr) {
+                              const CommXr* xr = nullptr, const BlockRun* blk = nullptr) {
   PlanMem m; plan_mem(p, &m);
   const bsig_fit_buffers& b = p->buf;
   PersistCommon c;
@@ -433,6 +437,13 @@
     pb.feat_ids = p->feat_unique ? b.ids_table : nullptr;
     pb.w_off = p->L.head_w_off; pb.b_off = p->L.head_b_off;
     pb.eval_row0 = p->feat_unique ? b.n_train : p->n_updates * p->batch;
+    if (blk) {
+      pb.feats = blk->feats; pb.ld_feats = blk->ld_feats; pb.feat_ids = blk->ids; pb.eval_row0 = 0;
+      pb.y = blk->y; pb.ldy = blk->ldy; pb.ids = blk->ids;
+      pb.train_loss = blk->train_loss; pb.test_loss = blk->test_loss;
+      pb.y_test = blk->y; pb.ldy_test = blk->ldy; pb.n_test = blk->max_test;
+      pb.chunks = blk->chunks; pb.n_chunks = blk->n_chunks;
+    }
     return persist_run(persist_shape(p), p->ug, pb, n, st);
   }
   PersistMdnnBuffers pb;
@@ -720,6 +731,7 @@
       persist_mdnn_resolve(persist_mdnn_shape(p), &p->mg, &p->eng);
   }
   if (set("BSIG_NO_INKERNEL_EVAL")) p->eng.eval_single = p->eng.eval_dp = false;
+  p->eng.block_launch = block_launch_resolved(p->eng.kind, p->eng.eval_single, set("BSIG_FIT_CHUNK_PER_LAUNCH"));
   p->eng.workspace_bytes = round_up<size_t>(p->eng.workspace_bytes, 256);
   if (p->hoist) {
     p->feats_bytes = round_up<size_t>(feats, 256);
@@ -833,9 +845,7 @@
   return BSIG_OK;
 }
 
-extern "C" int bsig_fit_begin(bsig_fit_plan* p, uint64_t seed, int64_t norm_batch,
-                              bsig_stream_t stream) {
-  bsig::Range roctx_range("bsig_fit_begin");
+static int fit_begin(bsig_fit_plan* p, uint64_t seed, int64_t norm_batch, bsig_stream_t stream, bool project) {
   BSIG_REQUIRE(p && p->bound, "fit_begin: plan not bound");
   BSIG_REQUIRE(norm_batch >= 1, "fit_begin: norm_batch must be >= 1");
   if (norm_batch != p->norm_batch) { drop_graphs(p); p->norm_batch = norm_batch; }
@@ -877,11 +887,17 @@
   const int blocks = (int)std::min<int64_t>(std::max<int64_t>(ceil_div<int64_t>(total4, 256 * 4), 1), 1024);
   hipLaunchKernelGGL(fit_begin_kernel, dim3(blocks), dim3(256), 0, st, p->buf.state, seed, bz);
   BSIG_CHECK_LAUNCH("fit_begin");
-  if (p->hoist) {
+  if (p->hoist && project) {
     if (p->feats_preloaded) p->feats_preloaded = false;
     else { p->ext_feats = nullptr; BSIG_TRY(enqueue_hoisted_rff(p, st)); }
   }
   return ensure_graphs(p);
+}
+
+extern "C" int bsig_fit_begin(bsig_fit_plan* p, uint64_t seed, int64_t norm_batch,
+                              bsig_stream_t stream) {
+  bsig::Range roctx_range("bsig_fit_begin");
+  return fit_begin(p, seed, norm_batch, stream, true);
 }
 
 static int dp_eval_total(const bsig_fit_plan* p) {
@@ -1026,6 +1042,68 @@
   hipLaunchKernelGGL(pack_logs_kernel, dim3(1), dim3(64), 0, as_stream(stream), p->buf.train_loss,
                      p->buf.test_loss, p->buf.state, (int)n_updates, (int)count_evals(n_updates), out);
   BSIG_CHECK_LAUNCH("pack_logs");
+  return BSIG_OK;
+}
+
+namespace bsig {
+__global__ void pack_block_logs_kernel(const float* train_loss, const float* test_loss, const int32_t* state,
+                                       const bsig_fit_chunk* chunks, int n_evals, float* out) {
+  const bsig_fit_chunk ch = chunks[blockIdx.x];
+  float* o = out + (int64_t)blockIdx.x * (2 * n_evals + 1);
+  if (threadIdx.x == 0) {
+    int e = 0;
+    for (int it = 0; it < ch.n_updates; ++it)
+      if (it % ch.eval_every == 0 || it + 1 == ch.n_updates) { o[e] = train_loss[ch.train_slot + it]; ++e; }
+    o[2 * n_evals] = (float)state[ST_NONFINITE];
+  }
+  for (int i = threadIdx.x; i < n_evals; i += blockDim.x) o[n_evals + i] = test_loss[ch.test_slot + i];
+}
+}
+
+extern "C" int bsig_debug_block_launch(int engine_kind, int eval_in_launch, int forced_single) {
+  return block_launch_resolved(engine_kind, eval_in_launch != 0, forced_single != 0) ? 1 : 0;
+}
+
+extern "C" int bsig_fit_block_chunks(const bsig_fit_plan* p, int64_t n_train) {
+  if (!p || !p->bound || p->split_adam || engine(p) != 1 || !p->eng.block_launch) return 0;
+  if (n_train < 1 || !feat_cache_applies(p, n_train) || p->n_updates < 1) return 0;
+  return (int)std::min<int64_t>(((int64_t)1 << 30) / (p->n_updates + 1), 1 << 16);
+}
+
+extern "C" int bsig_fit_run_block(bsig_fit_plan* p, const float* feats, int64_t ld_feats, int64_t rows,
+                                  const float* y, int64_t ldy, const int32_t* ids, int64_t n_ids,
+                                  const bsig_fit_chunk* chunks_host, const bsig_fit_chunk* chunks_dev, int n_chunks,
+                                  float* train_loss, float* test_loss, float* packed_logs, int64_t norm_batch,
+                                  bsig_stream_t stream) {
+  bsig::Range roctx_range("bsig_fit_run_block");
+  BSIG_REQUIRE(p && p->bound && feats && y && ids && chunks_host && chunks_dev && train_loss && test_loss &&
+               packed_logs, "fit_run_block: plan not bound / null");
+  BSIG_REQUIRE(n_chunks >= 1 && n_chunks <= bsig_fit_block_chunks(p, 1),
+               "fit_run_block: this plan runs one chunk per launch (bsig_fit_block_chunks)");
+  BSIG_REQUIRE(rows >= 1 && ld_feats >= p->cfg.rff_feats && ld_feats % 4 == 0 && aligned(feats, 16) &&
+               ldy >= p->cfg.head.out_dim && n_ids >= 0, "fit_run_block: bad block");
+  const int n_upd = (int)p->n_updates, every = std::max(n_upd / 5, 1), n_ev = (int)p->n_evals;
+  int max_test = 0;
+  for (int c = 0; c < n_chunks; ++c) {
+    const bsig_fit_chunk& k = chunks_host[c];
+    BSIG_REQUIRE(k.n_updates == n_upd && k.eval_every == every && k.upd_base == c * n_upd && k.eval_base == c * n_ev &&
+                 k.train_slot == k.upd_base && k.test_slot == k.eval_base,
+                 "fit_run_block: chunk %d: updates, evaluation schedule or slots out of step with the plan", c);
+    BSIG_REQUIRE(k.n_train >= 1 && k.n_test >= 1 && k.n_test <= p->max_test && feat_cache_applies(p, k.n_train) &&
+                 k.row0 >= 0 && k.row0 + k.n_train + k.n_test <= rows,
+                 "fit_run_block: chunk %d: rows %lld + %d + %d outside the block's %lld (or more than the plan covers)",
+                 c, (long long)k.row0, k.n_train, k.n_test, (long long)rows);
+    BSIG_REQUIRE(k.ids_off == (int64_t)k.upd_base * p->batch && k.ids_off + (int64_t)n_upd * p->batch <= n_ids,
+                 "fit_run_block: chunk %d: ids outside the table", c);
+    max_test = std::max(max_test, k.n_test);
+  }
+  BSIG_TRY(fit_begin(p, chunks_host[0].seed, norm_batch, stream, false));
+  hipStream_t st = as_stream(stream);
+  const BlockRun blk{feats, ld_feats, y, ldy, ids, chunks_dev, n_chunks, max_test, n_chunks * n_upd, train_loss, test_loss};
+  BSIG_TRY(enqueue_persistent(p, n_upd, st, n_upd, nullptr, &blk));
+  hipLaunchKernelGGL(pack_block_logs_kernel, dim3(n_chunks), dim3(64), 0, st, train_loss, test_loss, p->buf.state,
+                     chunks_dev, n_ev, packed_logs);
+  BSIG_CHECK_LAUNCH("pack_block_logs");
   return BSIG_OK;
 }
 
diff --git a/bayes_sim_ig_amd/csrc/fit_persistent.hip b/bayes_sim_ig_amd/csrc/fit_persistent.hip
--- a/bayes_sim_ig_amd/csrc/fit_persistent.hip
+++ b/bayes_sim_ig_amd/csrc/fit_persistent.hip
@@ -42,7 +42,63 @@
   unsigned long long* gran_eval;
   long long* prof;
   int prof_t0;
+  const bsig_fit_chunk* chunks; int n_chunks;
 };
+
+struct UCk {
+  int step0, n_updates, n_total, eval_every, do_eval;
+  unsigned ubase, evbase;
+  uint64_t seed, rng_ctr0;
+};
+__device__ __forceinline__ int u_uniform(int v) { return __builtin_amdgcn_readfirstlane(v); }
+__device__ __forceinline__ int64_t u_uniform(int64_t v) {
+  return (int64_t)(((uint64_t)(uint32_t)u_uniform((int)((uint64_t)v >> 32)) << 32) | (uint32_t)u_uniform((int)(uint64_t)v));
+}
+__device__ __forceinline__ void u_chunk_load(const UArgs& p, int c, UCk& k) {
+  if (p.chunks == nullptr) {
+    k.step0 = p.state[0]; k.n_updates = p.n_updates; k.n_total = p.n_total; k.eval_every = p.eval_every;
+    k.do_eval = p.do_eval; k.ubase = 0u; k.evbase = 0u;
+    k.seed = reinterpret_cast<const uint64_t*>(p.state + 8)[0];
+    k.rng_ctr0 = reinterpret_cast<const uint64_t*>(p.state + 8)[1];
+    return;
+  }
+  const bsig_fit_chunk& e = p.chunks[c];
+  k.step0 = 0; k.n_updates = u_uniform(e.n_updates); k.n_total = k.n_updates; k.eval_every = u_uniform(e.eval_every);
+  k.do_eval = 1; k.ubase = (unsigned)u_uniform(e.upd_base); k.evbase = (unsigned)u_uniform(e.eval_base);
+  k.seed = (uint64_t)u_uniform((int64_t)e.seed); k.rng_ctr0 = (uint64_t)u_uniform((int64_t)e.rng_ctr0);
+}
+
+struct UEval {
+  int n_test, passes; int64_t row0;
+  const float* y_test; int64_t ldy_test;
+  float* out;
+  unsigned gidx;
+  uint64_t seed, stream;
+};
+__device__ __forceinline__ UEval u_eval_of(const UArgs& p, int c, int e) {
+  UEval v;
+  int every, n_total, step0;
+  uint64_t ctr0;
+  if (p.chunks == nullptr) {
+    v.n_test = p.n_test; v.row0 = p.eval_row0; v.y_test = p.y_test; v.ldy_test = p.ldy_test; v.out = nullptr;
+    v.gidx = (unsigned)e; every = p.eval_every; n_total = p.n_total; step0 = p.state[0];
+    v.seed = reinterpret_cast<const uint64_t*>(p.state + 8)[0];
+    ctr0 = reinterpret_cast<const uint64_t*>(p.state + 8)[1];
+  } else {
+    const bsig_fit_chunk& k = p.chunks[c];
+    v.n_test = u_uniform(k.n_test); v.row0 = u_uniform(k.row0) + u_uniform(k.n_train);
+    v.y_test = p.y + v.row0 * p.ldy; v.ldy_test = p.ldy; v.out = p.test_loss + u_uniform(k.test_slot) + e;
+    v.gidx = (unsigned)u_uniform(k.eval_base) + (unsigned)e; every = u_uniform(k.eval_every);
+    n_total = u_uniform(k.n_updates); step0 = 0;
+    v.seed = (uint64_t)u_uniform((int64_t)k.seed); ctr0 = (uint64_t)u_uniform((int64_t)k.rng_ctr0);
+  }
+  v.passes = (v.n_test + p.B - 1) / p.B;
+  const int at = min(e * every + 1, n_total);
+  const int ev0 = p.do_eval || p.chunks ? (step0 == 0 ? 0 : (step0 - 1) / every + 1) : 0;
+  v.stream = ctr0 + (uint64_t)(at - step0) + (uint64_t)(e - ev0);
+  return v;
+}
+__device__ __forceinline__ int u_last_eval(int n_total, int every) { return n_total <= 1 ? 0 : (n_total - 2) / every + 1; }
 
 __device__ __forceinline__ f32x4 umfma(float a, float b, f32x4 c) {
   return __builtin_amdgcn_mfma_f32_16x16x4f32(a, b, c, 0, 0, 0);
@@ -75,8 +131,8 @@
 
 #define BSIG_USTAMP(k)                                                           \
   do {                                                                           \
-    if (p.prof && threadIdx.x == 0 && t >= p.prof_t0 && t < p.prof_t0 + kUProf)  \
-      p.prof[((int64_t)wg * kUProf + t - p.prof_t0) * 16 + (k)] = wall_clock64(); \
+    if (p.prof && threadIdx.x == 0 && pt >= p.prof_t0 && pt < p.prof_t0 + kUProf)  \
+      p.prof[((int64_t)wg * kUProf + pt - p.prof_t0) * 16 + (k)] = wall_clock64(); \
   } while (0)
 
 __device__ __forceinline__ int u_fast_kind(const UArgs& p) {
@@ -157,13 +213,13 @@
 
 template <int NT>
 __device__ __forceinline__ void u_tile_eval(const UArgs& p, const float* Wl, const float* biasl, int slot,
-                                            int ks, int n0, int k0, int eidx) {
+                                            int ks, int n0, int k0, const UEval& ev) {
   int tid = threadIdx.x;
   asm volatile("" : "+v"(tid));
   const int lane = tid & 63, w = tid >> 6, c16 = lane & 15, g4 = lane >> 4;
   const int B = p.B, NhP = p.NhP;
-  for (int pass = 0; pass < p.eval_passes; ++pass) {
-    const int rows = min(B, p.n_test - pass * B);
+  for (int pass = 0; pass < ev.passes; ++pass) {
+    const int rows = min(B, ev.n_test - pass * B);
     if (rows <= 0) break;
     if (w < p.MT) {
       f32x4 acc[NT];
@@ -172,7 +228,7 @@
         const f32x4 zero = {0.f, 0.f, 0.f, 0.f};
         acc[nt] = ks == 0 ? *reinterpret_cast<const f32x4*>(biasl + 16 * nt + 4 * g4) : zero;
       }
-      const int64_t r = p.eval_row0 + pass * B + min(16 * w + c16, rows - 1);
+      const int64_t r = ev.row0 + pass * B + min(16 * w + c16, rows - 1);
       const float* src = p.feats + r * p.ld_feats;
       const float* ap = Wl + c16 * p.WP + 4 * g4;
 #pragma unroll 1
@@ -199,7 +255,7 @@
       }
       if (16 * w + c16 < rows) {
         const __amdgpu_buffer_rsrc_t sr = xwg_buffer(
-            p.eval_slabs + ((((int64_t)(eidx % 3) * p.eval_passes + pass) * p.k_slices + ks) * B) * NhP + n0);
+            p.eval_slabs + ((((int64_t)(ev.gidx % 3u) * p.eval_passes + pass) * p.k_slices + ks) * B) * NhP + n0);
 #pragma unroll
         for (int nt = 0; nt < NT; ++nt)
           xwg_store4(sr, (16 * w + c16) * NhP + 16 * nt + 4 * g4, acc[nt][0], acc[nt][1], acc[nt][2], acc[nt][3]);
@@ -208,22 +264,22 @@
   }
   __builtin_amdgcn_s_waitcnt(0);
   __syncthreads();
-  if (tid == 0) flag_raise(p.flag_eval, slot, (unsigned)eidx + 1u);
-}
-
-__device__ __forceinline__ void u_owner_eval(const UArgs& p, float* XS, float* red, int eo, int eidx,
-                                             uint64_t stream, const HeadArgs& a) {
+  if (tid == 0) flag_raise(p.flag_eval, slot, ev.gidx + 1u);
+}
+
+__device__ __forceinline__ void u_owner_eval(const UArgs& p, float* XS, float* red, int eo, const UEval& ev,
+                                             const HeadArgs& a) {
   int tid = threadIdx.x;
   asm volatile("" : "+v"(tid));
   const int lane = tid & 63, w = tid >> 6;
   const int B = p.B, Nh = p.Nh, NhP = p.NhP, D = p.D, K = p.K, DK = D * K;
   const int per_wave = Nh + D + 3 * K;
   int32_t* flagp = p.state + 2;
-  const unsigned etag = (unsigned)eidx + 1u;
+  const unsigned etag = ev.gidx + 1u;
   if (w == 0) flags_wait(p.flag_eval, p.G, etag, lane, flagp);
   __syncthreads();
-  const int nr = eo < p.n_test ? min(p.RE, (p.n_test - eo + p.NE - 1) / p.NE) : 0;
-  const float* ebase = p.eval_slabs + (int64_t)(eidx % 3) * p.eval_passes * p.k_slices * B * NhP;
+  const int nr = eo < ev.n_test ? min(p.RE, (ev.n_test - eo + p.NE - 1) / p.NE) : 0;
+  const float* ebase = p.eval_slabs + (int64_t)(ev.gidx % 3u) * p.eval_passes * p.k_slices * B * NhP;
   float eacc = 0.f;
   u_rows_sum(ebase,
              [&](int r) {
@@ -248,7 +304,7 @@
   float* lpk = rk + K;
   float* dlg = lpk + K;
   if (act)
-    for (int j = lane; j < D; j += 64) yv[j] = p.y_test[(int64_t)erow * p.ldy_test + j];
+    for (int j = lane; j < D; j += 64) yv[j] = ev.y_test[(int64_t)erow * ev.ldy_test + j];
   RowOut ro;
   ro.lse = 0.f; ro.uds = 0.f; ro.bad = false;
 #pragma unroll
@@ -256,13 +312,14 @@
   if (w < p.RE) {
     HeadArgs ae = a;
     ae.d_out = nullptr;
-    ae.batch = p.n_test;
-    ae.stream_id = stream;
+    ae.batch = ev.n_test;
+    ae.seed = ev.seed;
+    ae.stream_id = ev.stream;
     diag_row(ae, erow, act, lane, tile, yv, rk, lpk, dlg,
              [&] {
                return p.eps_noise != 0.f
                           ? p.eps_noise * (granule_gather(p.gran_eval, p.NE, etag, lane, flagp) /
-                                           ((float)p.n_test * (float)DK))
+                                           ((float)ev.n_test * (float)DK))
                           : 0.f;
              },
              ro);
@@ -277,8 +334,9 @@
   if (eo == 0 && w == 0) {
     const float sum = granule_gather(p.gran_eval + kGranArr, p.NE, etag, lane, flagp);
     if (lane == 0) {
-      const float l = -sum / (float)p.n_test;
-      p.test_loss[p.state[1]] = l;
+      const float l = -sum / (float)ev.n_test;
+      if (ev.out) *ev.out = l;
+      else p.test_loss[p.state[1]] = l;
       p.state[1] = p.state[1] + 1;
       if (!isfinite(l)) atomicOr(flagp, 1);
     }
@@ -293,6 +351,7 @@
   float *XS, *red, *part;
   HeadArgs a; RowGeom rg;
   uint64_t rng_ctr0; int step0, ev0; float norm; int32_t* flagp;
+  unsigned ubase;
 };
 __device__ __forceinline__ void u_own_init(const UArgs& p, UOwn& o, int own, bool has_tile, float* XS,
                                            float* red, float* part, int lane0) {
@@ -301,24 +360,25 @@
   o.a = HeadArgs{};
   o.a.D = p.D; o.a.K = p.K; o.a.Nh = p.Nh; o.a.batch = p.B; o.a.from_tuple = 0;
   o.a.min_w = p.min_w; o.a.ll_limit = p.ll_limit; o.a.inv_norm = p.inv_norm;
-  o.a.eps_noise = p.eps_noise; o.a.seed = reinterpret_cast<const uint64_t*>(p.state + 8)[0]; o.a.d_out = p.d_out;
+  o.a.eps_noise = p.eps_noise; o.a.d_out = p.d_out;
   o.rg = row_geom(p.D, p.K, lane0);
-  o.rng_ctr0 = reinterpret_cast<const uint64_t*>(p.state + 8)[1];
-  o.step0 = p.state[0];
-  o.ev0 = p.do_eval ? u_evals_before(o.step0, p.eval_every) : 0;
   o.norm = (float)p.B * (float)(p.D * p.K);
   o.flagp = p.state + 2;
 }
-__device__ __forceinline__ uint64_t u_eval_stream(const UArgs& p, const UOwn& o, int e, bool last) {
-  const int at = last ? p.n_total : e * p.eval_every + 1;
-  return o.rng_ctr0 + (uint64_t)(at - o.step0) + (uint64_t)(e - o.ev0);
+__device__ __forceinline__ void u_own_chunk(UOwn& o, const UCk& k) {
+  o.a.seed = k.seed;
+  o.rng_ctr0 = k.rng_ctr0;
+  o.step0 = k.step0;
+  o.ev0 = k.do_eval ? u_evals_before(k.step0, k.eval_every) : 0;
+  o.ubase = k.ubase;
 }
 
 __device__ __forceinline__ void u_own_update(const UArgs& p, UOwn& o, int t, int w, int lane0, int wg) {
   const int B = p.B, Nh = p.Nh, NhP = p.NhP, D = p.D, K = p.K, DK = D * K;
   const int step = o.step0 + t;
-  const unsigned epoch = (unsigned)step + 1u;
+  const unsigned epoch = o.ubase + (unsigned)step + 1u;
   const uint32_t tag = epoch * 4u;
+  [[maybe_unused]] const int pt = t + (int)o.ubase;
   const int own = o.own, r0 = o.r0, per_wave = o.per_wave;
   const bool has_tile = o.has_tile;
   float* XS = o.XS; float* red = o.red; float* Ft = o.part;
@@ -341,7 +401,7 @@
     asm volatile("" : "+v"(lane));
     const int tid_l = 64 * w + lane;
     if (active) {
-      const int64_t yrow = p.ids[(int64_t)step * B + row];
+      const int64_t yrow = p.ids[(int64_t)(epoch - 1u) * B + row];
       for (int j = lane; j < D; j += 64) yv[j] = p.y[yrow * p.ldy + j];
     }
     float eu_pre[kElemsPerLane];
@@ -379,9 +439,9 @@
       GranuleEps ge{gran_rep(p, 0, wg & 7), p.n_owner, tag + 1, lane, flagp, p.eps_noise, norm, {0ull, 0ull, 0ull, 0ull}};
       diag_row_impl(a, rg, row, active, lane, tile, yv, rk, lpk, dlg, ge, ro, eu_pre);
 #ifdef BSIG_ROW_PROF
-      if (p.prof && tid == 0 && t >= p.prof_t0 && t < p.prof_t0 + kUProf)
+      if (p.prof && tid == 0 && pt >= p.prof_t0 && pt < p.prof_t0 + kUProf)
         for (int i = 0; i < 9; ++i)
-          p.prof[(int64_t)256 * kUProf * 16 + ((int64_t)wg * kUProf + t - p.prof_t0) * 16 + i] = ro.ts[i];
+          p.prof[(int64_t)256 * kUProf * 16 + ((int64_t)wg * kUProf + pt - p.prof_t0) * 16 + i] = ro.ts[i];
 #endif
       const float uds_w = wave_sum_dpp(ro.uds);
       if (lane == 0) { red[16 + w] = active ? ro.lse : 0.f; red[32 + w] = uds_w; }
@@ -413,7 +473,7 @@
       const float s = granule_gather(loss_granules(p.gran, epoch), p.n_owner, tag + 3, lane, flagp);
       if (lane == 0) {
         const float l = -s / (float)B;
-        p.train_loss[step] = l;
+        p.train_loss[epoch - 1u] = l;
         if (!isfinite(l)) atomicOr(flagp, 1);
       }
     }
@@ -422,8 +482,8 @@
 
 
 #ifdef BSIG_ROW_PROF
-#define BSIG_FSTAMP(i) do { if (p.prof && threadIdx.x == 0 && t >= p.prof_t0 && t < p.prof_t0 + kUProf) \
-    p.prof[(int64_t)256 * kUProf * 16 + ((int64_t)wg * kUProf + t - p.prof_t0) * 16 + (i)] = wall_clock64(); } while (0)
+#define BSIG_FSTAMP(i) do { if (p.prof && threadIdx.x == 0 && pt >= p.prof_t0 && pt < p.prof_t0 + kUProf) \
+    p.prof[(int64_t)256 * kUProf * 16 + ((int64_t)wg * kUProf + pt - p.prof_t0) * 16 + (i)] = wall_clock64(); } while (0)
 #else
 #define BSIG_FSTAMP(i)
 #endif
@@ -435,8 +495,9 @@
   const bool exact = K == KP;
   const int B = p.B, Nh = p.Nh, NhP = p.NhP, D = p.D, DK = D * K, R = p.R;
   const int step = o.step0 + t;
-  const unsigned epoch = (unsigned)step + 1u;
+  const unsigned epoch = o.ubase + (unsigned)step + 1u;
   const uint32_t tag = epoch * 4u;
+  [[maybe_unused]] const int pt = t + (int)o.ubase;
   const int own = o.own, r0 = o.r0;
   float* red = o.red; float* part = o.part; float* XS = o.XS;
   int32_t* flagp = o.flagp;
@@ -462,7 +523,7 @@
     yd[i] = 0.f; eu[i] = 0.f;
   }
   if (active) {
-    const int64_t yrow = p.ids[(int64_t)step * B + row];
+    const int64_t yrow = p.ids[(int64_t)(epoch - 1u) * B + row];
 #pragma unroll
     for (int i = 0; i < NQH; ++i)
       if (valid[i]) yd[i] = p.y[yrow * p.ldy + d0 + (h + 2 * i) * GR];
@@ -630,17 +691,17 @@
     const float s = granule_gather(loss_granules(p.gran, epoch), p.n_owner * R, tag + 3, lane, flagp);
     if (lane == 0) {
       const float l = -s / (float)B;
-      p.train_loss[step] = l;
+      p.train_loss[epoch - 1u] = l;
       if (!isfinite(l)) atomicOr(flagp, 1);
     }
   }
   if (bad) atomicOr(flagp, 1);
 }
 
-#define BSIG_U_ROWID(step_)                                                                  \
+#define BSIG_U_ROWID(ids_, row0_, step_)                                                    \
   if (has_tile && w < p.MT) {                                                                \
     const int64_t r = (int64_t)(step_) * B + min(16 * w + c16_l, B - 1);                     \
-    pf_row = p.feat_ids ? (int64_t)p.feat_ids[r] : r;                                        \
+    pf_row = (ids_) ? (row0_) + (int64_t)(ids_)[r] : r;                                      \
   }
 #define BSIG_U_PREFETCH()                                                                    \
   if (has_tile && w < p.MT) {                                                                \
@@ -684,7 +745,10 @@
   constexpr int FP = kUFP;
   const int WP = p.WP;
   int32_t* flagp = p.state + 2;
-  const int step0 = p.state[0];
+  const int n_chunks = (DP || XR || p.chunks == nullptr) ? 1 : p.n_chunks;
+  UCk ck;
+  u_chunk_load(p, 0, ck);
+  const int step0 = ck.step0;
   if (p.prof && p.n_updates > 0 && tid == 0) p.prof[((int64_t)wg * kUProf) * 16 + 14] = wall_clock64();
   double b1t = reinterpret_cast<const double*>(p.state + 12)[0];
   double b2t = reinterpret_cast<const double*>(p.state + 12)[1];
@@ -824,9 +888,10 @@
 
   UOwn o;
   u_own_init(p, o, own, true, XS, red, Ft, lane0);
+  u_own_chunk(o, ck);
   const int eo = (own - p.n_owner + p.T) % p.T;
   const bool has_erow = p.do_eval && eo < p.NE;
-  int pending_eval = -1;
+  int pending_eval = -1, pending_chunk = 0;
 
   f32x4 Freg[kUSteps];
   {
@@ -837,16 +902,32 @@
   int64_t pf_row = 0;
   {
     const int c16_l = c16, g4_l = g4;
-    if (p.n_updates > 0) { BSIG_U_ROWID(step0) BSIG_U_PREFETCH() }
+    if (p.n_updates > 0) { BSIG_U_ROWID(p.feat_ids, 0, step0) BSIG_U_PREFETCH() }
   }
   __syncthreads();
 
+  for (int c = 0; c < n_chunks; ++c) {
+  if (c > 0) {
+    u_chunk_load(p, c, ck);
+    u_own_chunk(o, ck);
+#pragma unroll
+    for (int jj = 0; jj < MAXBLK; ++jj)
+#pragma unroll
+      for (int nt = 0; nt < NT; ++nt)
+#pragma unroll
+        for (int v = 0; v < 4; ++v) { Mr[jj][nt][v] = 0.f; Vr[jj][nt][v] = 0.f; }
+#pragma unroll
+    for (int nt = 0; nt < NT; ++nt) { bm[nt] = 0.f; bv[nt] = 0.f; }
+    b1t = 1.0; b2t = 1.0;
+  }
+  const int step0 = ck.step0;
   for (int t = 0; t < p.n_updates; ++t) {
     int tid_l = tid, c16_l = c16, g4_l = g4;
     asm volatile("" : "+v"(tid_l), "+v"(c16_l), "+v"(g4_l));
     const int step = step0 + t;
-    const unsigned epoch = (unsigned)step + 1u;
+    const unsigned epoch = ck.ubase + (unsigned)step + 1u;
     const uint32_t tag = epoch * 4u;
+    [[maybe_unused]] const int pt = t + (int)ck.ubase;
     if (red[63] != 0.f) break;
     BSIG_USTAMP(0);
     {
@@ -899,7 +980,7 @@
       __syncthreads();
       if (tid_l == 0) flag_raise(p.flag_fwd, slot, epoch);
       BSIG_USTAMP(3);
-      if (t + 1 < p.n_updates) { BSIG_U_ROWID(step + 1) }
+      if (t + 1 < p.n_updates || c + 1 < n_chunks) { BSIG_U_ROWID(p.feat_ids, 0, epoch) }
     }
     if (tid_l == 0)
       red[63] = (__hip_atomic_load(flagp, __ATOMIC_RELAXED, __HIP_MEMORY_SCOPE_AGENT) & 2) ? 1.f : 0.f;
@@ -910,20 +991,20 @@
     if (has_row) u_own_update(p, o, t, w, lane0, wg);
     if (__builtin_expect(pending_eval >= 0, 0)) {
       __syncthreads();
-      if (has_erow) u_owner_eval(p, XS, red, eo, pending_eval, u_eval_stream(p, o, pending_eval, false), o.a);
+      if (has_erow) u_owner_eval(p, XS, red, eo, u_eval_of(p, pending_chunk, pending_eval), o.a);
       pending_eval = -1;
     }
-    if (__builtin_expect(p.do_eval && step > 0 && (step - 1) % p.eval_every == 0, 0)) {
-      const int e = u_evals_before(step, p.eval_every) - 1;
-      u_tile_eval<NT>(p, Wl, biasl, slot, ks, n0, k0, e);
-      pending_eval = e;
+    if (__builtin_expect(p.do_eval && (step > 0 ? (step - 1) % p.eval_every == 0 : c > 0), 0)) {
+      pending_chunk = step > 0 ? c : c - 1;
+      pending_eval = step > 0 ? u_evals_before(step, p.eval_every) - 1 : u_last_eval(p.n_updates, p.eval_every);
+      u_tile_eval<NT>(p, Wl, biasl, slot, ks, n0, k0, u_eval_of(p, pending_chunk, pending_eval));
     }
 
     {
       int tid_l = tid, c16_l = c16, g4_l = g4;
       asm volatile("" : "+v"(tid_l), "+v"(c16_l), "+v"(g4_l));
       const int lane = tid_l & 63;
-      if (t + 1 < p.n_updates) { BSIG_U_PREFETCH() }
+      if (t + 1 < p.n_updates || c + 1 < n_chunks) { BSIG_U_PREFETCH() }
       BSIG_USTAMP(2);
       if (w == 0) {
         unsigned long long* sug = gran_rep(p, 1, wg & 7);
@@ -1134,6 +1215,7 @@
       BSIG_USTAMP(12);
     }
   }
+  }
   if constexpr (XR) {
     if (slot == 0 && tid == 0 &&
         (__hip_atomic_load(flagp, __ATOMIC_RELAXED, __HIP_MEMORY_SCOPE_AGENT) & 2))
@@ -1142,14 +1224,14 @@
 
   if (p.do_eval && !run_aborted(flagp, red, tid)) {
     if (pending_eval >= 0) {
-      if (has_erow) u_owner_eval(p, XS, red, eo, pending_eval, u_eval_stream(p, o, pending_eval, false), o.a);
+      if (has_erow) u_owner_eval(p, XS, red, eo, u_eval_of(p, pending_chunk, pending_eval), o.a);
       pending_eval = -1;
     }
-    if (step0 + p.n_updates == p.n_total && (!DP || p.n_updates == 0)) {
-      const int e = u_evals_before(p.n_total - 1, p.eval_every);
+    if (ck.step0 + p.n_updates == p.n_total && (!DP || p.n_updates == 0)) {
+      const UEval ev = u_eval_of(p, n_chunks - 1, u_evals_before(p.n_total - 1, p.eval_every));
       __syncthreads();
-      u_tile_eval<NT>(p, Wl, biasl, slot, ks, n0, k0, e);
-      if (has_erow) u_owner_eval(p, XS, red, eo, e, u_eval_stream(p, o, e, true), o.a);
+      u_tile_eval<NT>(p, Wl, biasl, slot, ks, n0, k0, ev);
+      if (has_erow) u_owner_eval(p, XS, red, eo, ev, o.a);
     }
   }
   if (!DP && has_tile) {
@@ -1180,18 +1262,21 @@
     p.prof[((int64_t)wg * kUProf) * 16 + 13] = wall_clock64();
   }
   if (wg == 0 && tid == 0 && p.n_updates > 0) {
+    u_chunk_load(p, n_chunks - 1, ck);
+    const int step0 = ck.step0;
     int32_t* st = p.state;
     reinterpret_cast<double*>(st + 12)[0] = b1t;
     reinterpret_cast<double*>(st + 12)[1] = b2t;
     reinterpret_cast<float*>(st)[4] = a0;
     reinterpret_cast<float*>(st)[5] = a1;
     int n_ev = 0;
-    if (p.do_eval) {
-      n_ev = u_evals_before(step0 + p.n_updates, p.eval_every) - u_evals_before(step0, p.eval_every);
-      if (!DP && step0 + p.n_updates == p.n_total && (p.n_total - 1) % p.eval_every != 0) ++n_ev;
-    }
-    reinterpret_cast<uint64_t*>(st + 8)[1] += (uint64_t)(p.n_updates + n_ev);
-    st[0] = step0 + p.n_updates;
+    if (ck.do_eval) {
+      n_ev = u_evals_before(step0 + ck.n_updates, ck.eval_every) - u_evals_before(step0, ck.eval_every);
+      if (!DP && step0 + ck.n_updates == ck.n_total && (ck.n_total - 1) % ck.eval_every != 0) ++n_ev;
+    }
+    reinterpret_cast<uint64_t*>(st + 8)[0] = ck.seed;
+    reinterpret_cast<uint64_t*>(st + 8)[1] = ck.rng_ctr0 + (uint64_t)(ck.n_updates + n_ev);
+    st[0] = step0 + ck.n_updates;
   }
 }
 
@@ -1202,15 +1287,25 @@
   const int w = __builtin_amdgcn_readfirstlane(tid >> 6);
   const int wg = blockIdx.x;
   int32_t* flagp = p.state + 2;
+  const int n_chunks = (dp || p.chunks == nullptr) ? 1 : p.n_chunks;
+  UCk ck;
+  u_chunk_load(p, 0, ck);
   UOwn o;
   u_own_init(p, o, role.owner, false, XS, red, smem, lane0);
+  u_own_chunk(o, ck);
   const bool has_row = role.owner < p.n_owner;
   const int eo = (role.owner - p.n_owner + p.T) % p.T;
   const bool has_erow = p.do_eval && eo < p.NE;
   const int fk = u_fast_kind(p);
-  int pending_eval = -1;
+  int pending_eval = -1, pending_chunk = 0;
+  for (int c = 0; c < n_chunks; ++c) {
+  if (c > 0) {
+    u_chunk_load(p, c, ck);
+    u_own_chunk(o, ck);
+  }
   for (int t = 0; t < p.n_updates; ++t) {
     const int step = o.step0 + t;
+    [[maybe_unused]] const int pt = t + (int)ck.ubase;
     if (run_aborted(flagp, red, tid)) break;
     BSIG_USTAMP(0);
     if (has_row) {
@@ -1229,20 +1324,23 @@
     }
     if (__builtin_expect(pending_eval >= 0, 0)) {
       __syncthreads();
-      if (has_erow) u_owner_eval(p, XS, red, eo, pending_eval, u_eval_stream(p, o, pending_eval, false), o.a);
+      if (has_erow) u_owner_eval(p, XS, red, eo, u_eval_of(p, pending_chunk, pending_eval), o.a);
       pending_eval = -1;
     }
-    if (__builtin_expect(p.do_eval && step > 0 && (step - 1) % p.eval_every == 0, 0))
-      pending_eval = u_evals_before(step, p.eval_every) - 1;
+    if (__builtin_expect(p.do_eval && (step > 0 ? (step - 1) % p.eval_every == 0 : c > 0), 0)) {
+      pending_chunk = step > 0 ? c : c - 1;
+      pending_eval = step > 0 ? u_evals_before(step, p.eval_every) - 1 : u_last_eval(p.n_updates, p.eval_every);
+    }
     __syncthreads();
+  }
   }
   if (p.do_eval && !run_aborted(flagp, red, tid)) {
     if (pending_eval >= 0 && has_erow)
-      u_owner_eval(p, XS, red, eo, pending_eval, u_eval_stream(p, o, pending_eval, false), o.a);
-    if (o.step0 + p.n_updates == p.n_total && (!dp || p.n_updates == 0)) {
-      const int e = u_evals_before(p.n_total - 1, p.eval_every);
+      u_owner_eval(p, XS, red, eo, u_eval_of(p, pending_chunk, pending_eval), o.a);
+    if (ck.step0 + p.n_updates == p.n_total && (!dp || p.n_updates == 0)) {
+      const UEval ev = u_eval_of(p, n_chunks - 1, u_evals_before(p.n_total - 1, p.eval_every));
       __syncthreads();
-      if (has_erow) u_owner_eval(p, XS, red, eo, e, u_eval_stream(p, o, e, true), o.a);
+      if (has_erow) u_owner_eval(p, XS, red, eo, ev, o.a);
     }
   }
 }
@@ -1404,6 +1502,7 @@
   *g = c;
   e->kind = 1; e->streams = false;
   e->eval_single = e->eval_dp = c.eval_passes > 0;
+  e->block_launch = false;
   e->workspace_bytes = u_data_bytes(c) + u_sync_bytes();
   return true;
 }
@@ -1444,6 +1543,9 @@
                                  (int64_t)g.Nh * s.feat_dim < ((int64_t)1 << 29))),
                "persistent updates: a resident data-parallel launch moves 16-byte gradient quads");
   if (n <= 0 && !b.adam_pending && !b.do_eval) return BSIG_OK;
+  BSIG_REQUIRE(!(b.chunks && !(b.n_chunks >= 1 && !b.grads && !b.xr_ready && b.do_eval && b.feat_ids == b.ids &&
+                               n >= 1 && b.n_total == n && (int64_t)b.n_chunks * n < (1 << 30))),
+               "persistent updates: a block of chunks runs on a single rank with the evaluations inside the launch");
   UArgs p{};
   p.B = s.batch; p.Bp = g.Bp; p.MT = g.MT;
   p.Fdim = s.feat_dim; p.KS = g.KS; p.ksteps = g.ksteps; p.KB = g.KB; p.WP = g.WP;
@@ -1487,6 +1589,7 @@
     p.eval_passes = ceil_div(b.n_test, s.batch); p.eval_row0 = b.eval_row0;
     p.y_test = b.y_test; p.ldy_test = b.ldy_test; p.test_loss = b.test_loss;
   }
+  if (b.chunks) { p.chunks = b.chunks; p.n_chunks = b.n_chunks; }
   p.prof = reinterpret_cast<long long*>(persist_profile_buffer());
   if (p.prof) {
     const char* t0 = getenv("BSIG_PROF_T0");
diff --git a/bayes_sim_ig_amd/csrc/persist.h b/bayes_sim_ig_amd/csrc/persist.h
--- a/bayes_sim_ig_amd/csrc/persist.h
+++ b/bayes_sim_ig_amd/csrc/persist.h
@@ -8,8 +8,13 @@
   bool streams = false;
   bool eval_single = false;
   bool eval_dp = false;
+  bool block_launch = false;
   size_t workspace_bytes = 0;
 };
+
+inline bool block_launch_resolved(int kind, bool eval_single, bool forced_single) {
+  return kind == 1 && eval_single && !forced_single;
+}
 
 struct PersistShape {
   int batch, feat_dim, out_dim, n_comp;
@@ -48,6 +53,7 @@
   const int32_t* feat_ids;
   int64_t w_off, b_off;
   int64_t eval_row0 = 0;
+  const bsig_fit_chunk* chunks = nullptr; int n_chunks = 1;
 };
 
 bool persist_resolve(const PersistShape& s, UGeom* g, PersistEngine* e);
diff --git a/bayes_sim_ig_amd/mdnn.py b/bayes_sim_ig_amd/mdnn.py
--- a/bayes_sim_ig_amd/mdnn.py
+++ b/bayes_sim_ig_amd/mdnn.py
@@ -231,7 +231,13 @@
     def _resident_calls(self):
         return self._dp.resident_calls() if self._dp is not None else 0
 
-    def _give_up_a_level(self, resident_calls_before):
+    def _give_up_a_level(self, resident_calls_before, block_launches_before=None):
+        if block_launches_before is not None and getattr(self, '_block_launches', 0) > block_launches_before:
+            import warnings
+            warnings.warn('bayes_sim_ig_amd: a persistent launch over a block of chunks timed out; this model '
+                          'continues with one launch per chunk', RuntimeWarning, stacklevel=3)
+            self._no_block_launch = True
+            return
         if self._dp is not None and self._dp.resident_calls() > resident_calls_before:
             import warnings
             warnings.warn('bayes_sim_ig_amd: a data-parallel launch that stays resident across the gradient '
@@ -406,23 +412,7 @@
                 self._restore(snap)
                 self._give_up_a_level(calls0)
 
-    def _may_time_out(self):
-        if getattr(self, '_no_persistent', False) or os.environ.get('BSIG_NO_PERSISTENT') == '1':
-            return False
-        return self._plan is None or bool(_lib.load().bsig_fit_is_persistent(self._plan))
-
-    @_on_model_device
-    def _run_training_once(self, x_data, y_data, n_updates, batch_size, test_frac=0.2,
-                           ids_table=None, _defer=False, _feats=None):
-        assert x_data.shape[0] == y_data.shape[0]
-        lib = self._gpu()
-        self.train()
-        cfg = self._cfg()
-        dev = self._flat.device
-        d, n_tot = self.output_dim, x_data.shape[0]
-        n_train = max(int(n_tot * (1.0 - test_frac)), 1)
-        n_test = n_tot - n_train
-        st = _lib.stream()
+    def _ensure_plan(self, lib, cfg, batch_size, n_train, n_test, n_updates):
         key = (batch_size, max(n_test, self._bufs.get('cap_test', 0)), n_updates,
                cfg.head.eps_noise, cfg.lr, cfg.head.min_weight, cfg.head.ll_limit,
                max(n_train, self._bufs.get('cap_train', 0)))
@@ -435,6 +425,119 @@
                                               n_updates, flags, C.byref(handle)))
             self._plan, self._plan_key = handle, key
             self._bufs['cap_test'], self._bufs['cap_train'] = key[1], key[7]
+
+    @staticmethod
+    def block_prefix(sizes, test_frac):
+        k = 0
+        for n_tot in sizes:
+            if n_tot - max(int(n_tot * (1.0 - test_frac)), 1) < 1:
+                break
+            k += 1
+        return k
+
+    @_on_model_device
+    def run_training_block(self, feats, y_data, sizes, n_updates, batch_size, test_frac=0.2):
+        if (self._dp is not None or not self._flat.is_cuda or getattr(self, '_no_block_launch', False)
+                or getattr(self, 'rff', None) is None or len(sizes) < 1):
+            return None
+        lib = self._gpu()
+        self.train()
+        cfg = self._cfg()
+        dev = self._flat.device
+        d, rows = self.output_dim, int(sum(sizes))
+        assert feats.shape[0] == rows == y_data.shape[0] and feats.is_cuda and feats.dtype == torch.float32
+        split = [(max(int(n * (1.0 - test_frac)), 1), n - max(int(n * (1.0 - test_frac)), 1)) for n in sizes]
+        n_train, n_test = max(a for a, _ in split), max(b for _, b in split)
+        self._ensure_plan(lib, cfg, batch_size, n_train, n_test, n_updates)
+        st = _lib.stream()
+        n_chunks, n_ids = len(sizes), len(sizes) * n_updates * batch_size
+        every = max(n_updates // 5, 1)
+        n_e = len([it for it in range(n_updates) if it % every == 0 or it + 1 == n_updates])
+        ldy = _lib.round_up(d, 4)
+        y_stage = self._buf('blk_y', rows * ldy)
+        stage = self._buf('blk_stage', 16 * n_chunks + n_ids, torch.int32)
+        train_loss, test_loss = self._buf('blk_train_loss', n_chunks * n_updates), self._buf('blk_test_loss', n_chunks * n_e)
+        state = self._buf('state', 16, torch.int32)
+        ws = self._buf('fit_ws', int(lib.bsig_fit_workspace_bytes(self._plan)) // 4 + 1)
+        ldx = _lib.round_up(self.input_dim, 4)
+        if sizes[0] > self._bufs.get('cap_rows', 0):
+            self._bufs.pop('x_stage', None), self._bufs.pop('y_stage', None)
+            self._bufs['cap_rows'] = sizes[0]
+        x_stage = self._buf('x_stage', self._bufs['cap_rows'] * ldx)
+        coeff, ldc, off = self._rff_args()
+        fb = _lib.FitBuffers()
+        fb.params, fb.grads = self._flat.data_ptr(), self._flat_grad.data_ptr()
+        fb.exp_avg, fb.exp_avg_sq = self._exp_avg.data_ptr(), self._exp_avg_sq.data_ptr()
+        fb.rff_coeff = None if coeff is None else coeff.data_ptr()
+        fb.ld_coeff = ldc
+        fb.rff_offset = None if off is None else off.data_ptr()
+        fb.x_train, fb.ldx_train, fb.n_train = x_stage.data_ptr(), ldx, split[0][0]
+        fb.y_train, fb.ldy_train = y_stage.data_ptr(), ldy
+        fb.x_test, fb.ldx_test, fb.n_test = x_stage.data_ptr() + 4 * split[0][0] * ldx, ldx, split[0][1]
+        fb.y_test, fb.ldy_test = y_stage.data_ptr() + 4 * split[0][0] * ldy, ldy
+        fb.ids_table = stage.data_ptr() + 64 * n_chunks
+        fb.train_loss, fb.test_loss = train_loss.data_ptr(), test_loss.data_ptr()
+        fb.state = state.data_ptr()
+        fb.workspace, fb.workspace_bytes = ws.data_ptr(), ws.numel() * 4
+        flags = _lib.FIT_GRAPH if type(self).USE_GRAPH else 0
+        _lib.check(lib.bsig_fit_bind(self._plan, C.byref(fb), flags))
+        if n_chunks > int(lib.bsig_fit_block_chunks(self._plan, n_train)):
+            return None
+        ys, ldy_src = _lib.as_f32_rows(y_data, dev)
+        assert ys.shape[1] == d
+        if self.output_lows is not None:
+            _lib.check(lib.bsig_normalize_rows(
+                _lib.ptr(ys), ldy_src, _lib.ptr(self.output_lows),
+                _lib.ptr(self.output_highs), _lib.ptr(y_stage), ldy, rows, d, st))
+        else:
+            _lib.check(lib.bsig_copy_rows(_lib.ptr(ys), ldy_src, None, _lib.ptr(y_stage), ldy, rows, d, st))
+        ring = self._bufs.setdefault('blk_ring', {'slots': [], 'next': 0})
+        if not ring['slots'] or ring['slots'][0][0].numel() < 16 * n_chunks + n_ids:
+            ring['slots'] = [[torch.empty(16 * n_chunks + n_ids, dtype=torch.int32, pin_memory=True), None]
+                             for _ in range(4)]
+        slot = ring['slots'][ring['next'] % 4]
+        ring['next'] += 1
+        if slot[1] is not None:
+            slot[1].synchronize()
+        host = slot[0].numpy()
+        seeds = []
+        for c, (n_tr, _) in enumerate(split):
+            lo = 16 * n_chunks + c * n_updates * batch_size
+            host[lo:lo + n_updates * batch_size] = np.random.randint(
+                0, n_tr, (n_updates, batch_size), dtype=np.int32).reshape(-1) + np.int32(sum(sizes[:c]))
+            seeds.append(self._seed())
+        table = _lib.fit_chunk_table(sizes, seeds, n_updates, batch_size, test_frac)
+        host[:16 * n_chunks] = table.view(np.int32)
+        stage[:16 * n_chunks + n_ids].copy_(slot[0][:16 * n_chunks + n_ids], non_blocking=True)
+        slot[1] = torch.cuda.Event()
+        slot[1].record()
+        packed = torch.empty(n_chunks, 2 * n_e + 1, dtype=torch.float32, device=dev)
+        _lib.check(lib.bsig_fit_run_block(
+            self._plan, _lib.ptr(feats), feats.stride(0), rows, _lib.ptr(y_stage), ldy,
+            C.c_void_p(stage.data_ptr() + 64 * n_chunks), n_ids, C.c_void_p(table.ctypes.data),
+            _lib.ptr(stage), n_chunks, _lib.ptr(train_loss), _lib.ptr(test_loss), _lib.ptr(packed),
+            batch_size, st))
+        self._block_launches = getattr(self, '_block_launches', 0) + 1
+        return [PendingLogs(packed[c], n_e, split[c][1], type(self).VERBOSE) for c in range(n_chunks)]
+
+    def _may_time_out(self):
+        if getattr(self, '_no_persistent', False) or os.environ.get('BSIG_NO_PERSISTENT') == '1':
+            return False
+        return self._plan is None or bool(_lib.load().bsig_fit_is_persistent(self._plan))
+
+    @_on_model_device
+    def _run_training_once(self, x_data, y_data, n_updates, batch_size, test_frac=0.2,
+                           ids_table=None, _defer=False, _feats=None):
+        assert x_data.shape[0] == y_data.shape[0]
+        lib = self._gpu()
+        self.train()
+        cfg = self._cfg()
+        dev = self._flat.device
+        d, n_tot = self.output_dim, x_data.shape[0]
+        n_train = max(int(n_tot * (1.0 - test_frac)), 1)
+        n_test = n_tot - n_train
+        st = _lib.stream()
+        self._ensure_plan(lib, cfg, batch_size, n_train, n_test, n_updates)
         factored = isinstance(x_data, CrossCorrFactors)
         if factored and not lib.bsig_fit_accepts_factor_rows(self._plan, x_data.s_dim, x_data.a_dim):
             x_data, factored = x_data.materialize(), False
diff --git a/include/bsig.h b/include/bsig.h
--- a/include/bsig.h
+++ b/include/bsig.h
@@ -198,6 +198,22 @@
 int bsig_fit_updates(bsig_fit_plan* plan, int64_t n_updates, bsig_stream_t stream);
 int bsig_fit_pack_logs(bsig_fit_plan* plan, int64_t n_updates, float* out,
                        bsig_stream_t stream);
+typedef struct bsig_fit_chunk {
+  int64_t row0;
+  int32_t n_train, n_test;
+  int64_t ids_off;
+  uint64_t seed, rng_ctr0;
+  int32_t n_updates, eval_every;
+  int32_t train_slot, test_slot;
+  int32_t upd_base, eval_base;
+} bsig_fit_chunk;
+int bsig_fit_block_chunks(const bsig_fit_plan* plan, int64_t n_train);
+int bsig_fit_run_block(bsig_fit_plan* plan, const float* feats, int64_t ld_feats, int64_t rows,
+                       const float* y, int64_t ldy, const int32_t* ids, int64_t n_ids,
+                       const bsig_fit_chunk* chunks_host, const bsig_fit_chunk* chunks_dev, int n_chunks,
+                       float* train_loss, float* test_loss, float* packed_logs, int64_t norm_batch,
+                       bsig_stream_t stream);
+int bsig_debug_block_launch(int engine_kind, int eval_in_launch, int forced_single);
 int bsig_fit_grad(bsig_fit_plan* plan, bsig_stream_t stream);
 int bsig_fit_apply(bsig_fit_plan* plan, bsig_stream_t stream);
 int bsig_fit_flush(bsig_fit_plan* plan, bsig_stream_t stream);
```
